# imjaegyun/super_resolution

Measured on AMD Instinct MI355X. Metric: SR output megapixels/sec, HAT-S x4, 1280x720 LR in, higher is better.
Workload: dtype bf16; 1 GPU; HAT-S x4, one 3x720x1280 LR frame per GPU, full-frame forward; upscale=4, parallelism=dp1

## Files before the change

include/hat_mi355x.h:

```cpp
#ifndef HAT_MI355X_H
#define HAT_MI355X_H

#include <stdint.h>

#ifdef __cplusplus
extern "C" {
#endif

#define HAT_ABI_VERSION 2

enum { HAT_F32 = 0, HAT_BF16 = 1 };
enum { HAT_EINVAL = -1, HAT_ELDS = -2, HAT_EUNSUPPORTED = -3 };

enum { HAT_ACT_NONE = 0, HAT_ACT_GELU = 1 , HAT_ACT_LRELU = 2 ,
       HAT_ACT_LRELU02 = 3  };
enum { HAT_X_NHWC_T = 0, HAT_X_NHWC_F32 = 1, HAT_X_NCHW_F32_MEAN = 2 };
enum { HAT_O_NHWC_T = 0, HAT_O_NHWC_F32 = 1, HAT_O_PIXSHUF_T = 2, HAT_O_NCHW_F32 = 3 };

typedef struct HatConvDesc {
    const void* x;
    const void* x0;
    const void* w;
    const float* bias;
    void* out;
    const float* r1;
    const void* r2;
    const float* r2scale;
    float* colsum;
    int32_t B, H, W;
    int32_t Cin, ldx, x_mode;
    int32_t c_split, ldx0;
    int32_t ksize, Kpad;
    int32_t nt, n_slices;
    int64_t w_bstride;
    int32_t n_store;
    int32_t ldo, out_mode, act;
    int32_t ldr1, ldr2, r2scale_bstride;
    int32_t ps_r;
    float in_scale, out_scale;
    float mean[4];
    int32_t dtype;
    int32_t ld_ln, ln_ones;
    const float* ln_g;
    const float* ln_b;
    void* ln_out;
    float* gap_out;
    void* n16_out;
    int32_t gap_c;
    int32_t reserved0;
} HatConvDesc;

int hat_conv_occupancy(const HatConvDesc* d, int32_t* wgs_per_cu);
int hat_conv_tiles(const HatConvDesc* d, int32_t* tiles_out);
int hat_conv_plan(const HatConvDesc* d, int32_t* waves, int32_t* rows_per_wave, int32_t* tiles, int64_t* lds_bytes);
int hat_conv(const HatConvDesc* d, void* stream);

int hat_linear(const HatConvDesc* d, void* stream);

int hat_conv3x3_small_groups(const HatConvDesc* d, int32_t* groups_out);
int hat_conv3x3_small(const HatConvDesc* d, void* stream);

typedef struct HatCabFoldDesc {
    const void* c1;
    const float* c1_colsum;
    const float* w2;
    const float* b2;
    const float* wk;
    const float* bias_in;
    float* scale;
    void* wf;
    float* bias_out;
    float* tmp;
    int32_t B, H, W, C, mid, ld1, tiles, ldcs, k, ld_scale, dtype;
    float conv_scale;
    const float* stats;
    const float* w2f;
} HatCabFoldDesc;
int hat_cab_fold(const HatCabFoldDesc* d, void* stream);

typedef struct HatAggrCabDesc {
    HatConvDesc lin;
    const void* c1;
    const void* wf;
    const float* bias_b;
} HatAggrCabDesc;
int hat_aggr_cab(const HatAggrCabDesc* d, void* stream);

int hat_layernorm_blocks(void);
int hat_layernorm(const float* x, void* y, const float* gamma, const float* beta, float* gap_partial,
                  int32_t B, int64_t npix, int32_t C, int32_t ldy, int32_t out_f32, int32_t gap_c,
                  int32_t dtype, void* stream);

int hat_add_f32(const float* a, const float* c, float* out, int32_t B, int64_t n, int64_t c_bstride, void* stream);

int hat_esc_weights(const float* gap_partial, int32_t nblk, int64_t npix, const float* w1, const float* b1,
                    const float* w2, const float* b2, const float* plk_packed, void* w_out, int32_t B,
                    int32_t pdim, int32_t ksize, int32_t Kpad, int32_t dtype, void* stream);

int hat_esc_conv13(const void* x, int32_t ldx, const void* wp, int32_t Kpad, void* y16, int32_t B, int32_t H, int32_t W,
                   int32_t dtype, void* stream);
// ... 5 lines not shown
                    int32_t W, int32_t hid, int32_t ldu, int32_t ldo, int32_t dtype, void* stream);

typedef struct HatMlpDesc {
    const void* x;
    const void* w1f;
    const float* b1;
    const void* w2f;
    const float* b2;
    const float* r1;
    void* out;
    int32_t B, H, W, C, hidden;
    int32_t ldx, ldr1, ldo;
    int32_t out_f32, dtype;
} HatMlpDesc;
int hat_ocab_mlp(const HatMlpDesc* d, void* stream);
int hat_ocab_qkv(const HatMlpDesc* d, void* stream);

int hat_ocab_keybias(const void* sal, int32_t ldsal, const void* kv, int32_t ldkv, float* kb, int32_t B, int32_t H, int32_t W,
                     int32_t C, int32_t ws, int32_t wse, int32_t pad, int32_t k_keep, int32_t dtype, void* stream);
int hat_ocab_attention_kb(const void* q, const void* kv, const float* bias_rot, const float* kb, void* out, int32_t B, int32_t H,
                          int32_t W, int32_t C, int32_t heads, int32_t ws, int32_t wse, int32_t pad, int32_t ldq, int32_t ldkv,
                          int32_t ldo, int32_t dtype, void* stream);

int hat_sgfn_gate(const void* u, const float* wdw, const float* bdw, void* out, int32_t B, int32_t H, int32_t W,
                  int32_t half, int32_t ldu, int32_t ldo, int32_t dtype, void* stream);

int hat_ocab_attention(const void* q, const void* kv, const float* bias_rot, void* out, int32_t B, int32_t H,
                       int32_t W, int32_t C, int32_t heads, int32_t ws, int32_t wse, int32_t ldq,
                       int32_t ldkv, int32_t ldo, int32_t dtype, void* stream);
int hat_ocab_attention_log2(const void* q, const void* kv, const float* bias_rot, void* out, int32_t B, int32_t H, int32_t W,
                            int32_t C, int32_t heads, int32_t ws, int32_t wse, int32_t ldq, int32_t ldkv, int32_t ldo,
                            int32_t dtype, void* stream);

int hat_cab_squeeze_units(int32_t H, int32_t W, int32_t* rows_per_band, int32_t* units);
int hat_cab_squeeze(const void* x, const void* wpk, const float* bias, void* out, float* colsum, int32_t B, int32_t H,
                    int32_t W, int32_t C, int32_t ldx, int32_t dtype, void* stream);

int hat_conv3x3_to_planes(const void* x, const void* wpk, const float* bias, float* out, int32_t B, int32_t H, int32_t W,
                          int32_t C, int32_t ldx, int32_t n_out, float out_scale, const float* mean4, int32_t dtype,
                          void* stream);

int hat_u8_to_planes(const uint8_t* src, int64_t src_pitch, int64_t src_bstride, float* dst, int32_t B, int32_t h, int32_t w,
                     int32_t Hp, int32_t Wp, int32_t bgr, void* stream);
int hat_planes_to_u8(const float* src, int32_t B, int32_t Hs, int32_t Ws, uint8_t* dst, int64_t dst_pitch, int64_t dst_bstride,
                     int32_t h_out, int32_t w_out, int32_t bgr, void* stream);
int hat_conv3x3_to_u8(const void* x, const void* wpk, const float* bias, uint8_t* dst, int64_t dst_pitch, int64_t dst_bstride,
                      int32_t B, int32_t H, int32_t W, int32_t C, int32_t ldx, int32_t h_out, int32_t w_out, float out_scale,
                      const float* mean4, int32_t bgr, int32_t dtype, void* stream);

int hat_yuv420_to_planes(const uint8_t* y, int64_t y_pitch, int64_t y_bstride, const uint8_t* cb, const uint8_t* cr, int64_t c_pitch,
                         int32_t c_step, int64_t c_bstride, float* dst, int32_t B, int32_t h, int32_t w, int32_t Hp, int32_t Wp,
                         const float* to_rgb12, void* stream);
int hat_planes_to_yuv420(const float* src, int32_t B, int32_t Hs, int32_t Ws, uint8_t* y, int64_t y_pitch, int64_t y_bstride,
                         uint8_t* cb, uint8_t* cr, int64_t c_pitch, int32_t c_step, int64_t c_bstride, int32_t h_out, int32_t w_out,
                         const float* from_rgb12, void* stream);
int hat_conv3x3_to_yuv420(const void* x, const void* wpk, const float* bias, uint8_t* y, int64_t y_pitch, int64_t y_bstride, uint8_t* cb,
                          uint8_t* cr, int64_t c_pitch, int32_t c_step, int64_t c_bstride, int32_t B, int32_t H, int32_t W, int32_t C,
                          int32_t ldx, int32_t h_out, int32_t w_out, float out_scale, const float* mean4, const float* from_rgb12,
                          int32_t dtype, void* stream);

int hat_yuv420p16_to_planes(const uint16_t* y, int64_t y_pitch, int64_t y_bstride, const uint16_t* cb, const uint16_t* cr, int64_t c_pitch,
                            int32_t c_step, int64_t c_bstride, float* dst, int32_t B, int32_t h, int32_t w, int32_t Hp, int32_t Wp,
                            const float* to_rgb12, int32_t depth, int32_t msb, void* stream);
int hat_planes_to_yuv420p16(const float* src, int32_t B, int32_t Hs, int32_t Ws, uint16_t* y, int64_t y_pitch, int64_t y_bstride,
                            uint16_t* cb, uint16_t* cr, int64_t c_pitch, int32_t c_step, int64_t c_bstride, int32_t h_out, int32_t w_out,
                            const float* from_rgb12, int32_t depth, int32_t msb, void* stream);
int hat_conv3x3_to_yuv420p16(const void* x, const void* wpk, const float* bias, uint16_t* y, int64_t y_pitch, int64_t y_bstride, uint16_t* cb,
                             uint16_t* cr, int64_t c_pitch, int32_t c_step, int64_t c_bstride, int32_t B, int32_t H, int32_t W, int32_t C,
                             int32_t ldx, int32_t h_out, int32_t w_out, float out_scale, const float* mean4, const float* from_rgb12,
                             int32_t dtype, int32_t depth, int32_t msb, void* stream);

typedef struct {
    void* y; int64_t y_pitch, y_bstride; void* cb; void* cr; int64_t c_pitch; int32_t c_step; int64_t c_bstride;
    int32_t sub_x, sub_y, depth, msb;
} HatYuvSurface;
int hat_yuv_to_planes(const HatYuvSurface* src, float* dst, int32_t B, int32_t h, int32_t w, int32_t Hp, int32_t Wp, const float* to_rgb12,
                      void* stream);
int hat_planes_to_yuv(const float* src, int32_t B, int32_t Hs, int32_t Ws, const HatYuvSurface* dst, int32_t h_out, int32_t w_out,
                      const float* from_rgb12, void* stream);
int hat_conv3x3_to_yuv(const void* x, const void* wpk, const float* bias, const HatYuvSurface* dst, int32_t B, int32_t H, int32_t W, int32_t C,
                       int32_t ldx, int32_t h_out, int32_t w_out, float out_scale, const float* mean4, const float* from_rgb12,
                       int32_t dtype, void* stream);

#define HAT_SITING_CENTER 0
#define HAT_SITING_LEFT 1
#define HAT_SITING_TOPLEFT 2
int hat_yuv_to_planes_sited(const HatYuvSurface* src, int32_t siting, float* dst, int32_t B, int32_t h, int32_t w, int32_t Hp, int32_t Wp,
                            const float* to_rgb12, void* stream);
int hat_planes_to_yuv_sited(const float* src, int32_t B, int32_t Hs, int32_t Ws, const HatYuvSurface* dst, int32_t siting, int32_t h_out,
                            int32_t w_out, const float* from_rgb12, void* stream);

int hat_imresize_rows(const void* src, int32_t src_u8, int64_t src_pitch, int64_t src_bstride, int32_t bgr, float* mid, int32_t B,
                      int32_t h, int32_t w, int32_t oh, const float* w_h, const int32_t* src_h, int32_t P_h, int64_t n_table,
                      void* stream);
int hat_imresize_cols_to_planes(const float* mid, int32_t B, int32_t oh, int32_t w, int32_t ow, const float* w_w, const int32_t* src_w,
                                int32_t P_w, int64_t n_table, float* dst, int32_t Hp, int32_t Wp, void* stream);
int hat_imresize_cols_to_u8(const float* mid, int32_t B, int32_t oh, int32_t w, int32_t ow, const float* w_w, const int32_t* src_w,
                            int32_t P_w, int64_t n_table, uint8_t* dst, int64_t dst_pitch, int64_t dst_bstride, int32_t bgr,
                            void* stream);


enum { HAT_METRICS_Y = 1, HAT_METRICS_BGR = 2, HAT_METRICS_PSNR = 4, HAT_METRICS_SSIM = 8 };
int hat_u8_metrics_workspace_bytes(int32_t B, int32_t h, int32_t w, int32_t crop_border, int32_t flags, int64_t* bytes);
int hat_u8_metrics(const uint8_t* a, int64_t a_pitch, int64_t a_bstride, const uint8_t* b, int64_t b_pitch, int64_t b_bstride,
                   int32_t B, int32_t h, int32_t w, int32_t crop_border, int32_t flags, double* sums, void* workspace, void* stream);

int hat_pil_resize_u8(const uint8_t* src, int64_t src_pitch, int32_t h, int32_t w, uint8_t* mid, uint8_t* dst, int64_t dst_pitch, int32_t oh,
                      int32_t ow, const int32_t* coef_w, const int32_t* bounds_w, int32_t K_w, const int32_t* coef_h,
                      const int32_t* bounds_h, int32_t K_h, void* stream);
int hat_arb_psnr_workspace_bytes(int32_t h, int32_t w, int32_t shave, int64_t* bytes);
int hat_arb_psnr(const float* pred, int32_t ph, int32_t pw, const uint8_t* gt, int64_t gt_pitch, int32_t h, int32_t w, int32_t gray,
                 int32_t shave, double* sums, void* workspace, void* stream);

int hat_window_attention(const void* q, const void* kv, const float* bias_flip, void* out, int32_t B, int32_t H,
                         int32_t W, int32_t C, int32_t heads, int32_t ws, int32_t shift, int32_t ldq, int32_t ldkv,
                         int32_t ldo, int32_t dtype, void* stream);

typedef struct HatFfnDesc {
    const float* t_in;
    float* t_out;
    const float* ln_g;
    const float* ln_b;
    const void* w1f;
    const float* b1;
    const void* dww;
    const float* dwb;
    const void* w2f;
    const float* b2;
    const float* ln1_g;
    const float* ln1_b;
    void* n_out;
    float* gap_out;
    int32_t B, H, W, C;
    int32_t chunks;
    int32_t ldn, gap_c;
    int32_t dtype;
    int32_t ldm_in;
    const void* m_in;
    void* n16_out;
} HatFfnDesc;

int hat_ffn_tiles(const HatFfnDesc* d, int32_t* tiles_out);
int hat_ffn(const HatFfnDesc* d, void* stream);

int hat_ffn2(const HatFfnDesc* d, void* stream);

typedef struct HatHabTailDesc {
    HatFfnDesc ffn;
    const void* n;
    const void* y16;
    const void* c1;
    const void* w_aggr;
    const void* wf;
    const float* bias_b;
    int32_t ldn_in;
    int32_t ldr2;
    const void* r2;
    const float* r2scale;
    int32_t r2scale_bstride;
    int32_t reserved1;
} HatHabTailDesc;
int hat_hab_tail(const HatHabTailDesc* d, void* stream);

int hat_hab_tail3(const HatHabTailDesc* d, void* stream);

typedef struct hat_plan hat_plan;
// ... 144 lines not shown
```

super_resolution_amd/_lib.py:

```python
from __future__ import annotations

import ctypes as C
import os
import threading

_HERE = os.path.dirname(os.path.abspath(__file__))
LIB_PATH = os.environ.get("HAT_MI355X_LIB") or os.path.join(_HERE, "libhat_mi355x.so")

ABI_VERSION = 2
HAT_F32, HAT_BF16 = 0, 1
ACT_NONE, ACT_GELU, ACT_LRELU, ACT_LRELU02 = 0, 1, 2, 3
X_NHWC_T, X_NHWC_F32, X_NCHW_F32_MEAN = 0, 1, 2
O_NHWC_T, O_NHWC_F32, O_PIXSHUF_T, O_NCHW_F32 = 0, 1, 2, 3
METRICS_Y, METRICS_BGR, METRICS_PSNR, METRICS_SSIM = 1, 2, 4, 8

_ERRORS = {-1: "HAT_EINVAL (bad argument)", -2: "HAT_ELDS (tile does not fit in 160 KiB LDS)",
           -3: "HAT_EUNSUPPORTED (shape not instantiated)"}


class HatConvDesc(C.Structure):
    _fields_ = [
        ("x", C.c_void_p), ("x0", C.c_void_p), ("w", C.c_void_p), ("bias", C.c_void_p),
        ("out", C.c_void_p), ("r1", C.c_void_p), ("r2", C.c_void_p), ("r2scale", C.c_void_p), ("colsum", C.c_void_p),
        ("B", C.c_int32), ("H", C.c_int32), ("W", C.c_int32),
        ("Cin", C.c_int32), ("ldx", C.c_int32), ("x_mode", C.c_int32),
        ("c_split", C.c_int32), ("ldx0", C.c_int32),
        ("ksize", C.c_int32), ("Kpad", C.c_int32),
        ("nt", C.c_int32), ("n_slices", C.c_int32),
        ("w_bstride", C.c_int64),
        ("n_store", C.c_int32),
        ("ldo", C.c_int32), ("out_mode", C.c_int32), ("act", C.c_int32),
        ("ldr1", C.c_int32), ("ldr2", C.c_int32), ("r2scale_bstride", C.c_int32),
        ("ps_r", C.c_int32),
        ("in_scale", C.c_float), ("out_scale", C.c_float),
        ("mean", C.c_float * 4),
        ("dtype", C.c_int32),
        ("ld_ln", C.c_int32), ("ln_ones", C.c_int32),
        ("ln_g", C.c_void_p), ("ln_b", C.c_void_p), ("ln_out", C.c_void_p),
        ("gap_out", C.c_void_p), ("n16_out", C.c_void_p), ("gap_c", C.c_int32), ("reserved0", C.c_int32),
    ]


class HatMlpDesc(C.Structure):
    _fields_ = [
        ("x", C.c_void_p), ("w1f", C.c_void_p), ("b1", C.c_void_p), ("w2f", C.c_void_p), ("b2", C.c_void_p),
        ("r1", C.c_void_p), ("out", C.c_void_p),
        ("B", C.c_int32), ("H", C.c_int32), ("W", C.c_int32), ("C", C.c_int32), ("hidden", C.c_int32),
        ("ldx", C.c_int32), ("ldr1", C.c_int32), ("ldo", C.c_int32),
        ("out_f32", C.c_int32), ("dtype", C.c_int32),
    ]


class HatFfnDesc(C.Structure):
    _fields_ = [
        ("t_in", C.c_void_p), ("t_out", C.c_void_p), ("ln_g", C.c_void_p), ("ln_b", C.c_void_p),
        ("w1f", C.c_void_p), ("b1", C.c_void_p), ("dww", C.c_void_p), ("dwb", C.c_void_p),
        ("w2f", C.c_void_p), ("b2", C.c_void_p), ("ln1_g", C.c_void_p), ("ln1_b", C.c_void_p),
        ("n_out", C.c_void_p), ("gap_out", C.c_void_p),
        ("B", C.c_int32), ("H", C.c_int32), ("W", C.c_int32), ("C", C.c_int32),
        ("chunks", C.c_int32), ("ldn", C.c_int32), ("gap_c", C.c_int32), ("dtype", C.c_int32),
        ("ldm_in", C.c_int32), ("m_in", C.c_void_p), ("n16_out", C.c_void_p),
    ]


class HatHabTailDesc(C.Structure):
    _fields_ = [("ffn", HatFfnDesc), ("n", C.c_void_p), ("y16", C.c_void_p), ("c1", C.c_void_p), ("w_aggr", C.c_void_p),
                ("wf", C.c_void_p), ("bias_b", C.c_void_p), ("ldn_in", C.c_int32), ("ldr2", C.c_int32), ("r2", C.c_void_p),
                ("r2scale", C.c_void_p), ("r2scale_bstride", C.c_int32), ("reserved1", C.c_int32)]


class HatCabFoldDesc(C.Structure):
    _fields_ = [
        ("c1", C.c_void_p), ("c1_colsum", C.c_void_p), ("w2", C.c_void_p), ("b2", C.c_void_p), ("wk", C.c_void_p),
        ("bias_in", C.c_void_p), ("scale", C.c_void_p), ("wf", C.c_void_p), ("bias_out", C.c_void_p), ("tmp", C.c_void_p),
        ("B", C.c_int32), ("H", C.c_int32), ("W", C.c_int32), ("C", C.c_int32), ("mid", C.c_int32), ("ld1", C.c_int32),
        ("tiles", C.c_int32), ("ldcs", C.c_int32), ("k", C.c_int32), ("ld_scale", C.c_int32), ("dtype", C.c_int32),
        ("conv_scale", C.c_float), ("stats", C.c_void_p), ("w2f", C.c_void_p),
    ]


class HatAggrCabDesc(C.Structure):
    _fields_ = [("lin", HatConvDesc), ("c1", C.c_void_p), ("wf", C.c_void_p), ("bias_b", C.c_void_p)]


class HatYuvSurface(C.Structure):
    _fields_ = [("y", C.c_void_p), ("y_pitch", C.c_int64), ("y_bstride", C.c_int64), ("cb", C.c_void_p), ("cr", C.c_void_p),
                ("c_pitch", C.c_int64), ("c_step", C.c_int32), ("c_bstride", C.c_int64),
                ("sub_x", C.c_int32), ("sub_y", C.c_int32), ("depth", C.c_int32), ("msb", C.c_int32)]


class HatNafHalfDesc(C.Structure):
    _fields_ = [("r_in", C.c_void_p), ("gprev", C.c_void_p), ("wf", C.c_void_p), ("bf", C.c_void_p), ("r_out", C.c_void_p),
                ("w1", C.c_void_p), ("b1", C.c_void_p), ("dww", C.c_void_p), ("dwb", C.c_void_p), ("g_out", C.c_void_p),
                ("partials", C.c_void_p), ("wf_bstride", C.c_int64), ("bf_bstride", C.c_int32),
                ("B", C.c_int32), ("H", C.c_int32), ("W", C.c_int32), ("C", C.c_int32), ("ldr", C.c_int32), ("ldg", C.c_int32),
                ("ldo", C.c_int32), ("dtype", C.c_int32), ("reserved0", C.c_int32)]
# ... 13 lines not shown
                ("ldo", C.c_int32), ("out_f32", C.c_int32), ("dtype", C.c_int32), ("reserved0", C.c_int32)]


_YUV_BLOCK = [C.c_void_p, C.c_int64, C.c_int64, C.c_void_p, C.c_void_p, C.c_int64, C.c_int32, C.c_int64]

SIGNATURES = {
    "hat_abi_version": (C.c_int, []),
    "hat_target_arch": (C.c_char_p, []),
    "hat_conv_tiles": (C.c_int, [C.POINTER(HatConvDesc), C.POINTER(C.c_int32)]),
    "hat_ocab_mlp": (C.c_int, [C.POINTER(HatMlpDesc), C.c_void_p]),
    "hat_ocab_qkv": (C.c_int, [C.POINTER(HatMlpDesc), C.c_void_p]),
    "hat_conv_occupancy": (C.c_int, [C.POINTER(HatConvDesc), C.POINTER(C.c_int32)]),
    "hat_conv_plan": (C.c_int, [C.POINTER(HatConvDesc), C.POINTER(C.c_int32), C.POINTER(C.c_int32), C.POINTER(C.c_int32),
                                C.POINTER(C.c_int64)]),
    "hat_conv": (C.c_int, [C.POINTER(HatConvDesc), C.c_void_p]),
    "hat_linear": (C.c_int, [C.POINTER(HatConvDesc), C.c_void_p]),
    "hat_conv3x3_small_groups": (C.c_int, [C.POINTER(HatConvDesc), C.POINTER(C.c_int32)]),
    "hat_conv3x3_small": (C.c_int, [C.POINTER(HatConvDesc), C.c_void_p]),
    "hat_cab_fold": (C.c_int, [C.POINTER(HatCabFoldDesc), C.c_void_p]),
    "hat_aggr_cab": (C.c_int, [C.POINTER(HatAggrCabDesc), C.c_void_p]),
    "hat_ffn_tiles": (C.c_int, [C.POINTER(HatFfnDesc), C.POINTER(C.c_int32)]),
    "hat_ffn": (C.c_int, [C.POINTER(HatFfnDesc), C.c_void_p]),
    "hat_ffn2": (C.c_int, [C.POINTER(HatFfnDesc), C.c_void_p]),
    "hat_hab_tail": (C.c_int, [C.POINTER(HatHabTailDesc), C.c_void_p]),
    "hat_hab_tail3": (C.c_int, [C.POINTER(HatHabTailDesc), C.c_void_p]),
    "hat_plan_load": (C.c_int, [C.c_char_p, C.POINTER(C.c_void_p)]),
    "hat_plan_info": (C.c_int, [C.c_void_p, C.POINTER(C.c_int32), C.POINTER(C.c_int64), C.POINTER(C.c_int64)]),
    "hat_plan_forward": (C.c_int, [C.c_void_p, C.c_void_p, C.c_void_p, C.c_void_p]),
    "hat_plan_free": (None, [C.c_void_p]),
    "hat_layernorm_blocks": (C.c_int, []),
    "hat_layernorm": (C.c_int, [C.c_void_p, C.c_void_p, C.c_void_p, C.c_void_p, C.c_void_p, C.c_int32, C.c_int64,
                                C.c_int32, C.c_int32, C.c_int32, C.c_int32, C.c_int32, C.c_void_p]),
    "hat_rect_sum": (C.c_int, [C.c_void_p, C.c_int32, C.c_int32, C.c_int32, C.c_int32, C.c_int32, C.c_int32, C.c_int32, C.c_int32,
                               C.c_int64, C.c_int32, C.c_void_p, C.c_int32, C.c_void_p, C.c_void_p, C.c_void_p]),
    "hat_add_f32": (C.c_int, [C.c_void_p, C.c_void_p, C.c_void_p, C.c_int32, C.c_int64, C.c_int64, C.c_void_p]),
    "hat_esc_weights": (C.c_int, [C.c_void_p, C.c_int32, C.c_int64, C.c_void_p, C.c_void_p, C.c_void_p, C.c_void_p,
                                  C.c_void_p, C.c_void_p, C.c_int32, C.c_int32, C.c_int32, C.c_int32, C.c_int32, C.c_void_p]),
    "hat_esc_conv13": (C.c_int, [C.c_void_p, C.c_int32, C.c_void_p, C.c_int32, C.c_void_p, C.c_int32, C.c_int32, C.c_int32, C.c_int32, C.c_void_p]),
    "hat_eca_scale": (C.c_int, [C.c_void_p, C.c_int32, C.c_int32, C.c_int64, C.c_void_p, C.c_int32, C.c_float,
                                C.c_void_p, C.c_void_p, C.c_int32, C.c_int32, C.c_void_p]),
    "hat_dwconv_gate": (C.c_int, [C.c_void_p, C.c_void_p, C.c_void_p, C.c_void_p, C.c_int32, C.c_int32, C.c_int32,
                                  C.c_int32, C.c_int32, C.c_int32, C.c_int32, C.c_void_p]),
    "hat_ocab_keybias": (C.c_int, [C.c_void_p, C.c_int32, C.c_void_p, C.c_int32, C.c_void_p] + [C.c_int32] * 9 + [C.c_void_p]),
    "hat_ocab_attention_kb": (C.c_int, [C.c_void_p] * 5 + [C.c_int32] * 12 + [C.c_void_p]),
    "hat_sgfn_gate": (C.c_int, [C.c_void_p, C.c_void_p, C.c_void_p, C.c_void_p, C.c_int32, C.c_int32, C.c_int32,
                                C.c_int32, C.c_int32, C.c_int32, C.c_int32, C.c_void_p]),
    "hat_ocab_attention": (C.c_int, [C.c_void_p, C.c_void_p, C.c_void_p, C.c_void_p, C.c_int32, C.c_int32, C.c_int32,
                                     C.c_int32, C.c_int32, C.c_int32, C.c_int32, C.c_int32, C.c_int32, C.c_int32,
                                     C.c_int32, C.c_void_p]),
    "hat_ocab_attention_log2": (C.c_int, [C.c_void_p, C.c_void_p, C.c_void_p, C.c_void_p, C.c_int32, C.c_int32, C.c_int32,
                                     C.c_int32, C.c_int32, C.c_int32, C.c_int32, C.c_int32, C.c_int32, C.c_int32,
                                     C.c_int32, C.c_void_p]),
    "hat_cab_squeeze_units": (C.c_int, [C.c_int32, C.c_int32, C.c_void_p, C.c_void_p]),
    "hat_cab_squeeze": (C.c_int, [C.c_void_p, C.c_void_p, C.c_void_p, C.c_void_p, C.c_void_p, C.c_int32, C.c_int32, C.c_int32,
                                  C.c_int32, C.c_int32, C.c_int32, C.c_void_p]),
    "hat_conv3x3_to_planes": (C.c_int, [C.c_void_p, C.c_void_p, C.c_void_p, C.c_void_p, C.c_int32, C.c_int32, C.c_int32, C.c_int32,
                                        C.c_int32, C.c_int32, C.c_float, C.c_void_p, C.c_int32, C.c_void_p]),
    "hat_u8_to_planes": (C.c_int, [C.c_void_p, C.c_int64, C.c_int64, C.c_void_p, C.c_int32, C.c_int32, C.c_int32, C.c_int32, C.c_int32,
                                   C.c_int32, C.c_void_p]),
    "hat_planes_to_u8": (C.c_int, [C.c_void_p, C.c_int32, C.c_int32, C.c_int32, C.c_void_p, C.c_int64, C.c_int64, C.c_int32, C.c_int32,
                                   C.c_int32, C.c_void_p]),
    "hat_conv3x3_to_u8": (C.c_int, [C.c_void_p, C.c_void_p, C.c_void_p, C.c_void_p, C.c_int64, C.c_int64, C.c_int32, C.c_int32, C.c_int32,
                                    C.c_int32, C.c_int32, C.c_int32, C.c_int32, C.c_float, C.c_void_p, C.c_int32, C.c_int32, C.c_void_p]),
    "hat_plan_forward_u8": (C.c_int, [C.c_void_p, C.c_void_p, C.c_int64, C.c_int32, C.c_int32, C.c_void_p, C.c_int64, C.c_int32,
                                      C.c_void_p]),
    "hat_yuv420_to_planes": (C.c_int, _YUV_BLOCK + [C.c_void_p, C.c_int32, C.c_int32, C.c_int32, C.c_int32, C.c_int32, C.c_void_p, C.c_void_p]),
    "hat_planes_to_yuv420": (C.c_int, [C.c_void_p, C.c_int32, C.c_int32, C.c_int32] + _YUV_BLOCK + [C.c_int32, C.c_int32, C.c_void_p, C.c_void_p]),
    "hat_conv3x3_to_yuv420": (C.c_int, [C.c_void_p, C.c_void_p, C.c_void_p] + _YUV_BLOCK + [C.c_int32] * 7 + [C.c_float, C.c_void_p, C.c_void_p,
                                                                                                      C.c_int32, C.c_void_p]),
    "hat_plan_forward_yuv420": (C.c_int, [C.c_void_p] + _YUV_BLOCK + [C.c_int32, C.c_int32] + _YUV_BLOCK + [C.c_void_p, C.c_void_p, C.c_void_p]),
    "hat_yuv420p16_to_planes": (C.c_int, _YUV_BLOCK + [C.c_void_p, C.c_int32, C.c_int32, C.c_int32, C.c_int32, C.c_int32, C.c_void_p, C.c_int32,
                                                       C.c_int32, C.c_void_p]),
    "hat_planes_to_yuv420p16": (C.c_int, [C.c_void_p, C.c_int32, C.c_int32, C.c_int32] + _YUV_BLOCK + [C.c_int32, C.c_int32, C.c_void_p, C.c_int32,
                                                                                                     C.c_int32, C.c_void_p]),
    "hat_conv3x3_to_yuv420p16": (C.c_int, [C.c_void_p, C.c_void_p, C.c_void_p] + _YUV_BLOCK + [C.c_int32] * 7 + [C.c_float, C.c_void_p, C.c_void_p,
                                                                                                         C.c_int32, C.c_int32, C.c_int32, C.c_void_p]),
    "hat_plan_forward_yuv420_deep": (C.c_int, [C.c_void_p] + _YUV_BLOCK + [C.c_int32] * 4 + _YUV_BLOCK + [C.c_int32, C.c_int32, C.c_void_p, C.c_void_p,
                                                                                                     C.c_void_p]),
    "hat_yuv_to_planes": (C.c_int, [C.POINTER(HatYuvSurface), C.c_void_p] + [C.c_int32] * 5 + [C.c_void_p, C.c_void_p]),
    "hat_planes_to_yuv": (C.c_int, [C.c_void_p, C.c_int32, C.c_int32, C.c_int32, C.POINTER(HatYuvSurface), C.c_int32, C.c_int32, C.c_void_p,
                                    C.c_void_p]),
    "hat_conv3x3_to_yuv": (C.c_int, [C.c_void_p, C.c_void_p, C.c_void_p, C.POINTER(HatYuvSurface)] + [C.c_int32] * 7 + [C.c_float, C.c_void_p,
                                                                                                        C.c_void_p, C.c_int32, C.c_void_p]),
    "hat_plan_forward_yuv": (C.c_int, [C.c_void_p, C.POINTER(HatYuvSurface), C.POINTER(HatYuvSurface), C.c_int32, C.c_int32, C.c_void_p,
                                       C.c_void_p, C.c_void_p]),
    "hat_yuv_to_planes_sited": (C.c_int, [C.POINTER(HatYuvSurface), C.c_int32, C.c_void_p] + [C.c_int32] * 5 + [C.c_void_p, C.c_void_p]),
    "hat_planes_to_yuv_sited": (C.c_int, [C.c_void_p, C.c_int32, C.c_int32, C.c_int32, C.POINTER(HatYuvSurface), C.c_int32, C.c_int32, C.c_int32,
                                          C.c_void_p, C.c_void_p]),
    "hat_plan_forward_yuv_sited": (C.c_int, [C.c_void_p, C.POINTER(HatYuvSurface), C.c_int32, C.POINTER(HatYuvSurface), C.c_int32, C.c_int32,
                                             C.c_int32, C.c_void_p, C.c_void_p, C.c_void_p]),
    "hat_imresize_rows": (C.c_int, [C.c_void_p, C.c_int32, C.c_int64, C.c_int64, C.c_int32, C.c_void_p, C.c_int32, C.c_int32, C.c_int32,
                                    C.c_int32, C.c_void_p, C.c_void_p, C.c_int32, C.c_int64, C.c_void_p]),
    "hat_imresize_cols_to_planes": (C.c_int, [C.c_void_p, C.c_int32, C.c_int32, C.c_int32, C.c_int32, C.c_void_p, C.c_void_p, C.c_int32,
                                              C.c_int64, C.c_void_p, C.c_int32, C.c_int32, C.c_void_p]),
    "hat_imresize_cols_to_u8": (C.c_int, [C.c_void_p, C.c_int32, C.c_int32, C.c_int32, C.c_int32, C.c_void_p, C.c_void_p, C.c_int32,
                                          C.c_int64, C.c_void_p, C.c_int64, C.c_int64, C.c_int32, C.c_void_p]),
    "hat_u8_metrics_workspace_bytes": (C.c_int, [C.c_int32, C.c_int32, C.c_int32, C.c_int32, C.c_int32, C.POINTER(C.c_int64)]),
    "hat_u8_metrics": (C.c_int, [C.c_void_p, C.c_int64, C.c_int64, C.c_void_p, C.c_int64, C.c_int64, C.c_int32, C.c_int32, C.c_int32,
                                 C.c_int32, C.c_int32, C.c_void_p, C.c_void_p, C.c_void_p]),
    "hat_pil_resize_u8": (C.c_int, [C.c_void_p, C.c_int64, C.c_int32, C.c_int32, C.c_void_p, C.c_void_p, C.c_int64, C.c_int32, C.c_int32,
                                    C.c_void_p, C.c_void_p, C.c_int32, C.c_void_p, C.c_void_p, C.c_int32, C.c_void_p]),
    "hat_arb_psnr_workspace_bytes": (C.c_int, [C.c_int32, C.c_int32, C.c_int32, C.POINTER(C.c_int64)]),
    "hat_arb_psnr": (C.c_int, [C.c_void_p, C.c_int32, C.c_int32, C.c_void_p, C.c_int64, C.c_int32, C.c_int32, C.c_int32, C.c_int32,
                               C.c_void_p, C.c_void_p, C.c_void_p]),
    "hat_dihedral_f32": (C.c_int, [C.c_void_p, C.c_void_p, C.c_int32, C.c_int32, C.c_int32, C.c_int32, C.c_int32, C.c_float, C.c_int32,
                                   C.c_void_p]),
    "hat_window_attention": (C.c_int, [C.c_void_p, C.c_void_p, C.c_void_p, C.c_void_p, C.c_int32, C.c_int32, C.c_int32,
                                       C.c_int32, C.c_int32, C.c_int32, C.c_int32, C.c_int32, C.c_int32, C.c_int32,
                                       C.c_int32, C.c_void_p]),
    "hat_niqe_workspace_bytes": (C.c_int, [C.c_int32, C.c_int32, C.c_int32, C.c_int32, C.POINTER(C.c_int32), C.POINTER(C.c_int32),
                                           C.POINTER(C.c_int64)]),
    "hat_niqe_y_u8": (C.c_int, [C.c_void_p, C.c_int64, C.c_int64, C.c_int32, C.c_int32, C.c_int32, C.c_int32, C.c_int32, C.c_void_p,
                                C.c_void_p, C.c_void_p]),
    "hat_imresize_plane_rows": (C.c_int, [C.c_void_p, C.c_void_p, C.c_int32, C.c_int32, C.c_int32, C.c_int32, C.c_void_p, C.c_void_p,
                                          C.c_int32, C.c_int64, C.c_void_p]),
    "hat_imresize_plane_cols": (C.c_int, [C.c_void_p, C.c_int32, C.c_int32, C.c_int32, C.c_int32, C.c_void_p, C.c_void_p, C.c_int32,
                                          C.c_int64, C.c_float, C.c_void_p, C.c_void_p]),
    "hat_niqe_block_stats": (C.c_int, [C.c_void_p, C.c_int32, C.c_int32, C.c_int32, C.c_int32, C.POINTER(C.c_double), C.c_void_p,
                                       C.c_void_p]),
    "hat_naf_half_tiles": (C.c_int, [C.c_int32, C.c_int32]),
    "hat_naf_half": (C.c_int, [C.POINTER(HatNafHalfDesc), C.c_void_p]),
    "hat_naf_fold": (C.c_int, [C.POINTER(HatNafFoldDesc), C.c_void_p]),
    "hat_esc_convffn_tiles": (C.c_int, [C.c_int32, C.c_int32]),
    "hat_esc_convffn": (C.c_int, [C.POINTER(HatEscConvFfnDesc), C.c_void_p]),
    "hat_window_attention_r": (C.c_int, [C.c_void_p] * 4 + [C.c_int32] * 10 + [C.c_void_p]),
    "hat_esc_layernorm": (C.c_int, [C.c_void_p] * 4 + [C.c_float, C.c_int64, C.c_int32, C.c_int32, C.c_int32, C.c_void_p]),
    "hat_esc_shuffle_add": (C.c_int, [C.c_void_p] * 3 + [C.c_int32] * 5 + [C.c_void_p]),
    "hat_escreal_skip": (C.c_int, [C.c_void_p] * 7 + [C.c_int32] * 6 + [C.c_void_p]),
    "hat_dysample": (C.c_int, [C.c_void_p] * 4 + [C.c_int32] * 5 + [C.c_void_p]),
    "hat_unshuffle_pad": (C.c_int, [C.c_void_p] * 2 + [C.c_int32] * 5 + [C.c_void_p]),
    "hat_escrealm_skip": (C.c_int, [C.c_void_p] * 9 + [C.c_int32] * 8 + [C.c_void_p]),
    "hat_shuffle_planes": (C.c_int, [C.c_void_p] * 2 + [C.c_int32] * 5 + [C.c_void_p]),
    "hat_escfp_convffn": (C.c_int, [C.POINTER(HatEscConvFfnDesc), C.c_void_p]),
    "hat_escfp_layernorm": (C.c_int, [C.c_void_p] * 4 + [C.c_float, C.c_int64, C.c_int32, C.c_int32, C.c_int32, C.c_void_p]),
    "hat_escfp_weights": (C.c_int, [C.c_void_p, C.c_int32, C.c_int64] + [C.c_void_p] * 7 + [C.c_int32] * 3 + [C.c_void_p]),
    "hat_escfp_shuffle_bicubic": (C.c_int, [C.c_void_p] * 4 + [C.c_int32] * 5 + [C.c_void_p]),
    "hat_lte_query": (C.c_int, [C.c_void_p, C.c_void_p, C.c_int32, C.c_int32, C.c_void_p, C.c_int32, C.c_int32] + [C.c_void_p] * 11
                      + [C.c_int64, C.c_int32, C.c_int32] + [C.c_float] * 4 + [C.c_void_p, C.c_int32, C.c_void_p]),
    "hat_lte_query_u8": (C.c_int, [C.c_void_p, C.c_void_p, C.c_int32, C.c_int32, C.c_void_p, C.c_int32, C.c_int32] + [C.c_void_p] * 9
                         + [C.c_int32, C.c_int32] + [C.c_float] * 4 + [C.c_void_p, C.c_int64, C.c_int32, C.c_int32, C.c_void_p]),
    "hat_lte_query_yuv": (C.c_int, [C.c_void_p, C.c_void_p, C.c_int32, C.c_int32, C.c_void_p, C.c_int32, C.c_int32] + [C.c_void_p] * 9
                          + [C.c_int32, C.c_int32] + [C.c_float] * 4 + [C.POINTER(HatYuvSurface), C.c_void_p, C.c_int32, C.c_void_p]),
    "hat_shuffle_to_u8": (C.c_int, [C.c_void_p, C.c_int32, C.c_void_p] + [C.c_int32] * 4 + [C.c_void_p, C.c_int64, C.c_int64] + [C.c_int32] * 3
                          + [C.c_void_p]),
    "hat_shuffle_to_yuv": (C.c_int, [C.c_void_p, C.c_int32, C.c_void_p] + [C.c_int32] * 4 + [C.POINTER(HatYuvSurface), C.c_int32, C.c_int32,
                                                                                              C.c_void_p, C.c_void_p]),
}

_lib = None
_lock = threading.Lock()


def load():
    global _lib
    if _lib is not None:
        return _lib
    with _lock:
        if _lib is not None:
            return _lib
        if not os.path.exists(LIB_PATH):
            raise RuntimeError(
                f"{LIB_PATH} not found: the HIP kernels are not built. Run `python -m super_resolution_amd.build` "
                "(needs hipcc). There is no CPU fallback for the HAT forward pass.")
        import torch
        lib = C.CDLL(LIB_PATH)
        for name, (res, args) in SIGNATURES.items():
# ... 17 lines not shown
```

super_resolution_amd/build.py:

```python
from __future__ import annotations

import os
import subprocess
import sys
from concurrent.futures import ThreadPoolExecutor

HERE = os.path.dirname(os.path.abspath(__file__))
CSRC = os.path.join(HERE, "csrc")
LIB = os.path.join(HERE, "libhat_mi355x.so")
SOURCES = ["hat_conv.hip", "hat_conv64r.hip", "hat_attn.hip", "hat_misc.hip", "hat_ffn.hip", "hat_ffn2.hip", "hat_tail3.hip", "hat_tail3l.hip", "hat_pw.hip", "hat_mlp.hip", "hat_cabsq.hip", "hat_esc13.hip", "hat_u8.hip", "hat_yuv.hip", "hat_resize.hip", "hat_pil_resize.hip", "hat_metrics.hip", "hat_dihedral.hip", "hat_niqe.hip", "hat_naf.hip", "hat_esc.hip", "hat_escreal.hip", "hat_escrealm.hip", "hat_escfp.hip", "hat_lte.hip", "hat_esc_sink.hip", "hat_plan.cpp"]
HEADERS = [os.path.join(CSRC, "hat_common.h"), os.path.join(CSRC, "hat_yuv_check.h"), os.path.join(CSRC, "hat_yuv_sample.h"), os.path.join(CSRC, "hat_frame_sink.h"), os.path.join(CSRC, "hat_esc_ffn.h"), os.path.join(CSRC, "hat_plan_parse.h"), os.path.join(os.path.dirname(HERE), "include", "hat_mi355x.h")]
FLAGS = ["-O3", "--offload-arch=gfx950", "-fPIC", "-std=c++17", "-Wall", "-Wno-unused-function"]


def _hipcc() -> str:
    for c in (os.environ.get("HIPCC"), "/opt/rocm/bin/hipcc", "hipcc"):
        if c and (os.path.isabs(c) and os.path.exists(c) or not os.path.isabs(c)):
            return c
    raise RuntimeError("hipcc not found")


def _stale(target: str, deps) -> bool:
    if not os.path.exists(target):
        return True
    t = os.path.getmtime(target)
    return any(os.path.getmtime(d) > t for d in deps)


def build(force: bool = False, verbose: bool = True) -> str:
    hipcc = _hipcc()
    objs, jobs = [], []
    for src in SOURCES:
        s = os.path.join(CSRC, src)
        o = os.path.join(CSRC, os.path.splitext(src)[0] + ".o")
        objs.append(o)
        if force or _stale(o, [s] + HEADERS):
            jobs.append([hipcc, *FLAGS, "-c", s, "-o", o])

    def run(cmd):
        if verbose:
            print(" ".join(cmd), flush=True)
        r = subprocess.run(cmd, capture_output=True, text=True)
        if r.returncode != 0:
            raise RuntimeError(f"hipcc failed:\n{' '.join(cmd)}\n{r.stdout}\n{r.stderr}")
        if verbose and r.stderr.strip():
            print(r.stderr, file=sys.stderr)

    with ThreadPoolExecutor(max_workers=4) as ex:
        list(ex.map(run, jobs))
    if force or jobs or _stale(LIB, objs):
        run([hipcc, "--offload-arch=gfx950", "-shared", "-fPIC", "-o", LIB, *objs])
    return LIB


if __name__ == "__main__":
    print(build(force="--force" in sys.argv))
```

super_resolution_amd/csrc/hat_conv.hip:

```cpp
#include <type_traits>

#include "hat_common.h"

bool hat_conv64r_can_launch(const HatConvDesc& d);
int hat_conv64r_launch(const HatConvDesc& d, hipStream_t s);

#ifndef HAT_CONV_PIPE
#define HAT_CONV_PIPE 1
#endif

namespace {

struct TileCfg { int waves, pt; };

__host__ inline size_t conv_lds_bytes(const HatConvDesc& d, int waves, int pt, int es, int kc) {
    const int hl = d.ksize / 2;
    const int cin_p = (d.Cin + 7) & ~7;
    const size_t xs = (size_t)(waves * pt + 2 * hl) * (16 + 2 * hl) * lds_row_elems(cin_p, es) * es;
    const size_t ws = (size_t)d.nt * 16 * lds_row_elems(kc, es) * es;
    const size_t koff = ((size_t)(d.Kpad / 32) * 16 + 15) & ~(size_t)15;
    return xs + ws + koff;
}

__host__ inline bool conv_pick(const HatConvDesc& d, TileCfg* out, size_t* lds) {
    const int es = d.dtype == HAT_BF16 ? 2 : 4;
    const int kc = (d.dtype == HAT_BF16 ? 64 : 32) * (d.nt == 1 ? 3 : (d.nt <= 4 ? 2 : 1));
    const TileCfg cands[3] = {{8, 2}, {4, 2}, {4, 1}};
    const size_t wbytes = (size_t)d.nt * 16 * d.ksize * d.ksize * ((d.Cin + 7) & ~7) * es;
    for (int pass = (wbytes <= 180000 ? 0 : 1); pass < 2; ++pass) {
        const size_t limit = pass == 0 ? HAT_LDS_MAX / 2 : HAT_LDS_MAX;
        for (int i = 0; i < 3; ++i) {
            const int rows = cands[i].waves * cands[i].pt;
            if (i < 2 && d.H * 2 <= rows) continue;
            if (pass == 0 && i == 2) continue;
            const size_t b = conv_lds_bytes(d, cands[i].waves, cands[i].pt, es, kc);
            if (b <= limit) { *out = cands[i]; *lds = b; return true; }
        }
    }
    return false;
}

template <typename T, int WAVES, int PT, int NT, int TH = 0>
__global__ __launch_bounds__(WAVES * 64) void conv_kernel(const HatConvDesc d) {
    using M = MT<T>;
    constexpr int NTHR = WAVES * 64;
    constexpr int TROWS = WAVES * PT;
    constexpr int KC = M::KC * (NT == 1 ? 3 : (NT <= 4 ? 2 : 1));
    constexpr int KS = KC / 32;
    constexpr int PPR = KC * (int)sizeof(T) / 16;
    constexpr int VEC = M::VEC;
    constexpr int WPIECES = NT * 16 * PPR;
    constexpr int WPT = (WPIECES + NTHR - 1) / NTHR;

    extern __shared__ __attribute__((aligned(16))) char smem[];
#ifdef HAT_CONV_STAMPS
    const long long st0 = (long long)__builtin_amdgcn_s_memtime();
#endif
    const int tid = threadIdx.x;
    const int lane = tid & 63, wave = tid >> 6, g = lane >> 4, c16 = lane & 15;
    if (d.reserved0 > 0) {
        const unsigned lin = (blockIdx.z * gridDim.y + blockIdx.y) * gridDim.x + blockIdx.x;
        if (lin < 256u) {
            const int n = (int)((lin >> 3) & 3u) * d.reserved0;
            for (int i = 0; i < n; ++i) __builtin_amdgcn_s_sleep(127);
        }
    }
    const int ks_ = d.ksize;
    const int hl = ks_ >> 1, TWH = 16 + 2 * hl, THH = TROWS + 2 * hl;
    const int Cin = d.Cin, Cin_p = (Cin + 7) & ~7;
    const int ldxs = lds_row_elems(Cin_p, sizeof(T));
    const int ldws = lds_row_elems(KC, sizeof(T));
    T* Xs = reinterpret_cast<T*>(smem);
    T* Ws = Xs + (size_t)THH * TWH * ldxs;
    int* koff = reinterpret_cast<int*>(Ws + NT * 16 * ldws);
    float* cs = reinterpret_cast<float*>(Ws);

    const int b = blockIdx.z;
    const int x0 = blockIdx.x * 16, y0 = blockIdx.y * TROWS;
    const int H = d.H, W = d.W;
    const int ntaps = ks_ * ks_;

    for (int i = tid; i < (d.Kpad / 32) * 4; i += NTHR) {
        const int k = 32 * (i >> 2) + 8 * (i & 3);
        int tp = k / Cin_p;
        const int cc = k - tp * Cin_p;
        tp = tp < ntaps ? tp : ntaps - 1;
        koff[i] = ((tp / ks_) * TWH + (tp % ks_)) * ldxs + cc;
    }
// ... 427 lines not shown
    if (!d.x || !d.w || !d.bias || !d.out) return HAT_EINVAL;
    if (d.reserved0 & ~3) return HAT_EINVAL;
    if (d.reserved0) {
        if (d.dtype != HAT_BF16 || d.nt != 9 || d.n_slices != 1 || d.n_store != 144 || d.colsum || d.ksize == 1) return HAT_EINVAL;
        if ((d.reserved0 & 1) && (!d.r1 || reinterpret_cast<uintptr_t>(d.r1) % 8)) return HAT_EINVAL;
        if ((d.reserved0 & 2) && (d.out_mode != HAT_O_NHWC_F32 || d.ldo % 8 || reinterpret_cast<uintptr_t>(d.out) % 16)) return HAT_EINVAL;
    }
    if (d.B < 1 || d.H < 1 || d.W < 1 || d.Cin < 1) return HAT_EINVAL;
    if (d.act < HAT_ACT_NONE || d.act > HAT_ACT_LRELU02) return HAT_EINVAL;
    if (d.ksize < 1 || (d.ksize & 1) == 0 || d.ksize > 17) return HAT_EINVAL;
    if (d.dtype != HAT_F32 && d.dtype != HAT_BF16) return HAT_EINVAL;
    const int kc = (d.dtype == HAT_BF16 ? 64 : 32) * (d.nt == 1 ? 3 : (d.nt <= 4 ? 2 : 1)), vec = d.dtype == HAT_BF16 ? 8 : 4;
    const int cin_p = (d.Cin + 7) & ~7;
    if (d.Kpad % kc || d.Kpad < d.ksize * d.ksize * cin_p) return HAT_EINVAL;
    if (d.n_slices < 1 || d.n_store < 1 || d.n_store > d.n_slices * d.nt * 16) return HAT_EINVAL;
    if (d.x_mode == HAT_X_NHWC_T) {
        if (d.ldx % vec || d.ldx < cin_p) return HAT_EINVAL;
        if (d.x0 && (d.ldx0 % vec || d.c_split % vec || d.c_split > d.Cin)) return HAT_EINVAL;
    } else if (d.x_mode == HAT_X_NHWC_F32) {
        if (d.ldx % 4 || d.Cin % 4 || d.x0) return HAT_EINVAL;
    } else if (d.x_mode == HAT_X_NCHW_F32_MEAN) {
        if (d.Cin > 4 || d.x0) return HAT_EINVAL;
    } else {
        return HAT_EINVAL;
    }
    if (d.out_mode == HAT_O_NCHW_F32) {
        if (d.n_store > 4 || d.r1 || d.r2) return HAT_EINVAL;
    } else {
        if (d.n_store % 4 || d.ldo % 4) return HAT_EINVAL;
        if (d.out_mode == HAT_O_PIXSHUF_T) {
            if (d.ps_r < 2 || d.n_store % (d.ps_r * d.ps_r) || (d.n_store / (d.ps_r * d.ps_r)) % 4 || d.r1 || d.r2) return HAT_EINVAL;
        } else if (d.out_mode != HAT_O_NHWC_T && d.out_mode != HAT_O_NHWC_F32) {
            return HAT_EINVAL;
        }
    }
    if (d.r1 && d.ldr1 % 4) return HAT_EINVAL;
    if (d.r2 && (d.ldr2 % 4 || !d.r2scale)) return HAT_EINVAL;
    if (d.ln_out) {
        if (!d.ln_g || !d.ln_b || d.ln_ones || d.n_slices != 1 || d.n_store != d.nt * 16 || d.ld_ln % 4 || d.ld_ln < d.n_store) return HAT_EINVAL;
        if (d.out_mode != HAT_O_NHWC_T && d.out_mode != HAT_O_NHWC_F32) return HAT_EINVAL;
        if (d.colsum || d.gap_c < 0 || d.gap_c > 16 || d.gap_c % 4) return HAT_EINVAL;
    } else if (d.gap_out || d.n16_out) {
#ifndef HAT_CONV_STAMPS
        return HAT_EINVAL;
#endif
    }
    return 0;
}

}

extern "C" int hat_conv_tiles(const HatConvDesc* d, int32_t* tiles_out) {
    if (!d || !tiles_out) return HAT_EINVAL;
    TileCfg tc; size_t lds;
    if (!conv_pick(*d, &tc, &lds)) return HAT_ELDS;
    *tiles_out = ((d->W + 15) / 16) * ((d->H + tc.waves * tc.pt - 1) / (tc.waves * tc.pt));
    return 0;
}

extern "C" int hat_conv_plan(const HatConvDesc* d, int32_t* waves, int32_t* rows_per_wave, int32_t* tiles, int64_t* lds_bytes) {
    if (!d || !waves || !rows_per_wave || !tiles || !lds_bytes) return HAT_EINVAL;
    TileCfg tc; size_t lds;
    if (!conv_pick(*d, &tc, &lds)) return HAT_ELDS;
    *waves = tc.waves; *rows_per_wave = tc.pt; *lds_bytes = (int64_t)lds;
    *tiles = ((d->W + 15) / 16) * ((d->H + tc.waves * tc.pt - 1) / (tc.waves * tc.pt));
    return 0;
}

extern "C" int hat_conv_occupancy(const HatConvDesc* dp, int32_t* wgs_per_cu) {
    if (!dp || !wgs_per_cu) return HAT_EINVAL;
    TileCfg tc; size_t lds;
    if (!conv_pick(*dp, &tc, &lds)) return HAT_ELDS;
    int v = 0;
    g_occ_query = &v;
    const int rc = dp->dtype == HAT_BF16 ? dispatch_tile<bf16_t>(*dp, tc, lds, nullptr) : dispatch_tile<float>(*dp, tc, lds, nullptr);
    g_occ_query = nullptr;
    *wgs_per_cu = v;
    return rc;
}

extern "C" int hat_conv(const HatConvDesc* dp, void* stream) {
    if (!dp) return HAT_EINVAL;
    const HatConvDesc& d = *dp;
    int rc = conv_validate(d);
    if (rc) return rc;
    TileCfg tc; size_t lds;
    hipStream_t s = reinterpret_cast<hipStream_t>(stream);
    if (hat_conv64r_can_launch(d)) return hat_conv64r_launch(d, s);
    if (!conv_pick(d, &tc, &lds)) return HAT_ELDS;
    if (d.dtype == HAT_BF16) return dispatch_tile<bf16_t>(d, tc, lds, s);
    return dispatch_tile<float>(d, tc, lds, s);
}
```

super_resolution_amd/csrc/hat_plan.cpp:

```cpp
#include <hip/hip_runtime.h>
#include <stdint.h>
#include <stdio.h>
#include <string.h>

#include <string>
#include <utility>
#include <vector>

#include "../../include/hat_mi355x.h"
#include "hat_plan_parse.h"
#include "hat_yuv_check.h"

using namespace hat_plan_host;

struct hat_plan {
    int32_t dims[8];
    std::vector<Buf> bufs;
    std::vector<Call> calls;
    int device = -1;
    mutable float* stage_in = nullptr;
    mutable float* stage_out = nullptr;
};

namespace {

struct Resolved {
    const hat_plan* p;
    const Call* c;
    const void* x;
    void* y;
    void* stream;
    std::vector<std::vector<unsigned char>> tmp;
    void* ptr(uint32_t buf, uint64_t off) const {
        if (buf == NULL_BUF) return nullptr;
        const Buf& b = p->bufs[buf];
        char* base = b.kind == BUF_INPUT ? (char*)const_cast<void*>(x) : (b.kind == BUF_OUTPUT ? (char*)y : (char*)b.dev);
        return base + off;
    }
    int32_t I(size_t k) const { return (int32_t)c->args[k].i; }
    int64_t L(size_t k) const { return c->args[k].i; }
    float F(size_t k) const { return (float)c->args[k].f; }
    void* P(size_t k) {
        const Arg& a = c->args[k];
        if (a.tag == ARG_PTR) return ptr(a.buf, a.off);
        if (a.tag == ARG_STREAM) return stream;
        if (a.tag == ARG_STRUCT || a.tag == ARG_HOST) {
            tmp.emplace_back(a.blob);
            for (const Fix& fx : a.fix) {
                void* v = ptr(fx.buf, fx.off);
                memcpy(tmp.back().data() + fx.field_off, &v, sizeof(void*));
            }
            return tmp.back().data();
        }
        return nullptr;
    }
};

template <class T> T arg_as(Resolved& r, size_t k) {
    if constexpr (std::is_same_v<T, int32_t>) return r.I(k);
    else if constexpr (std::is_same_v<T, int64_t>) return r.L(k);
    else if constexpr (std::is_same_v<T, float>) return r.F(k);
    else return (T)r.P(k);
}
template <class... A, size_t... K> int replay(int (*fn)(A...), Resolved& r, std::index_sequence<K...>) { return fn(arg_as<A>(r, K)...); }
template <class... A> int replay(int (*fn)(A...), Resolved& r) {
    return r.c->args.size() == sizeof...(A) ? replay(fn, r, std::index_sequence_for<A...>{}) : HAT_EINVAL;
}

int dispatch(Resolved& r) {
    switch (r.c->fn) {
#define HAT_PLAN_CASE(f) case FN_##f: return replay(&f, r);
        HAT_PLAN_FUNCTIONS(HAT_PLAN_CASE)
#undef HAT_PLAN_CASE
        default: return HAT_EUNSUPPORTED;
    }
}

}

extern "C" void hat_plan_free(hat_plan* p) {
    if (!p) return;
    for (Buf& b : p->bufs)
        if (b.dev) (void)hipFree(b.dev);
    if (p->stage_in) (void)hipFree(p->stage_in);
    if (p->stage_out) (void)hipFree(p->stage_out);
// ... 8 lines not shown
    try {
        return plan_load_impl(path, out);
    } catch (...) {
        return HAT_EINVAL;
    }
}

namespace {
struct PlanGuard {
    hat_plan* p;
    ~PlanGuard() { if (p) hat_plan_free(p); }
};
}

static int plan_load_impl(const char* path, hat_plan** out) {
    FILE* f = fopen(path, "rb");
    if (!f) return HAT_EINVAL;
    struct FileGuard { FILE* f; ~FileGuard() { fclose(f); } } fguard{f};
    hat_plan* p = new hat_plan();
    PlanGuard guard{p};
    {
        Parsed parsed;
        if (const int rc = hat_plan_parse(f, &parsed)) return rc;
        memcpy(p->dims, parsed.dims, sizeof(p->dims));
        p->bufs = std::move(parsed.bufs);
        p->calls = std::move(parsed.calls);
    }
    if (hipGetDevice(&p->device) != hipSuccess) return HAT_EINVAL;
    std::vector<unsigned char> host;
    for (Buf& b : p->bufs) {
        if (b.kind != BUF_CONST && b.kind != BUF_SCRATCH) continue;
        hipError_t e = hipMalloc(&b.dev, b.nbytes ? b.nbytes : 16);
        if (e != hipSuccess) { b.dev = nullptr; return (int)e; }
        if (b.kind == BUF_CONST) {
            host.resize(b.nbytes);
            if (fseeko(f, (off_t)b.file_off, SEEK_SET) != 0 || (b.nbytes && fread(host.data(), 1, b.nbytes, f) != b.nbytes)) return HAT_EINVAL;
            e = hipMemcpy(b.dev, host.data(), b.nbytes, hipMemcpyHostToDevice);
        } else {
            e = hipMemset(b.dev, 0, b.nbytes ? b.nbytes : 16);
        }
        if (e != hipSuccess) return (int)e;
    }
    if (const hipError_t e = hipDeviceSynchronize()) return (int)e;
    guard.p = nullptr;
    *out = p;
    return 0;
}

extern "C" int hat_plan_info(const hat_plan* p, int32_t* dims8, int64_t* n_calls, int64_t* device_bytes) {
    if (!p) return HAT_EINVAL;
    if (dims8) memcpy(dims8, p->dims, sizeof(p->dims));
    if (n_calls) *n_calls = (int64_t)p->calls.size();
    if (device_bytes) {
        int64_t s = 0;
        for (const Buf& b : p->bufs)
            if (b.dev) s += (int64_t)b.nbytes;
        *device_bytes = s;
    }
    return 0;
}

extern "C" int hat_plan_forward(const hat_plan* p, const float* x, float* y, void* stream) {
    if (!p || !x || !y) return HAT_EINVAL;
    int dev = -1;
    if (hipGetDevice(&dev) != hipSuccess || dev != p->device) return HAT_EINVAL;
    for (const Call& c : p->calls) {
        Resolved r{p, &c, x, y, stream, {}};
        const int rc = dispatch(r);
        if (rc) return rc;
    }
    return 0;
}

namespace {
bool addresses_output(const hat_plan* p, const Call& c) {
    for (const Arg& a : c.args) {
        if (a.tag == ARG_PTR && a.buf != NULL_BUF && p->bufs[a.buf].kind == BUF_OUTPUT) return true;
        for (const Fix& fx : a.fix)
            if (fx.buf != NULL_BUF && p->bufs[fx.buf].kind == BUF_OUTPUT) return true;
    }
    return false;
}

bool ends_in_planes(const hat_plan* p) {
    if (p->calls.empty()) return false;
    const Call& c = p->calls.back();
    if (c.fn != FN_hat_conv3x3_to_planes || c.args.size() != 14 || c.args[3].tag != ARG_PTR || c.args[3].buf >= p->bufs.size()) return false;
    if (p->bufs[c.args[3].buf].kind != BUF_OUTPUT || c.args[3].off != 0 || c.args[9].i != 3) return false;
    for (size_t k = 0; k + 1 < p->calls.size(); ++k)
        if (addresses_output(p, p->calls[k])) return false;
    return true;
}

template <typename Source, typename Fused, typename Planes>
int forward_frames(const hat_plan* p, void* stream, Source source, Fused fused_sink, Planes planes_sink, bool may_fuse = true) {
    const int32_t B = p->dims[0], H = p->dims[2], W = p->dims[3], s = p->dims[4];
    int dev = -1;
    if (hipGetDevice(&dev) != hipSuccess || dev != p->device) return HAT_EINVAL;
    const bool fused = may_fuse && ends_in_planes(p);
    if (!p->stage_in) {
        const hipError_t e = hipMalloc((void**)&p->stage_in, (size_t)B * 3 * H * W * sizeof(float));
        if (e != hipSuccess) { p->stage_in = nullptr; return (int)e; }
    }
    if (!fused && !p->stage_out) {
        const hipError_t e = hipMalloc((void**)&p->stage_out, (size_t)B * 3 * s * H * s * W * sizeof(float));
        if (e != hipSuccess) { p->stage_out = nullptr; return (int)e; }
    }
    int rc = source(p->stage_in);
    if (rc) return rc;
    const size_t n = p->calls.size() - (fused ? 1 : 0);
    for (size_t k = 0; k < n; ++k) {
        Resolved r{p, &p->calls[k], p->stage_in, p->stage_out, stream, {}};
        rc = dispatch(r);
        if (rc) return rc;
    }
    if (!fused) return planes_sink(p->stage_out, s * H, s * W);
    Resolved r{p, &p->calls.back(), p->stage_in, nullptr, stream, {}};
    return fused_sink(r);
}

int frame_fits(const hat_plan* p, int32_t h, int32_t w) {
    const int32_t H = p->dims[2], W = p->dims[3];
    if (p->dims[1] != 3 || p->dims[5] != 3) return HAT_EUNSUPPORTED;
    return h > H || w > W || H - h >= h || W - w >= w ? HAT_EINVAL : 0;
}

int forward_yuv(const hat_plan* p, const HatYuvSurface* src, const HatYuvSurface* dst, int32_t h, int32_t w, const float* to_rgb12,
                const float* from_rgb12, void* stream, bool planes420, int32_t src_siting = HAT_SITING_CENTER,
                int32_t dst_siting = HAT_SITING_CENTER) {
    if (!hat_yuv_surface_ok(src, 1, h, w)) return HAT_EINVAL;
    if (const int rc = frame_fits(p, h, w)) return rc;
    const int32_t B = p->dims[0], H = p->dims[2], W = p->dims[3], s = p->dims[4], ho = s * h, wo = s * w;
    if (!hat_yuv_surface_ok(src, B, h, w) || !hat_yuv_surface_ok(dst, B, (int64_t)s * h, (int64_t)s * w)) return HAT_EINVAL;
    const bool sited_out = hat_siting_of(dst, dst_siting) != HAT_SITING_CENTER;
    return forward_frames(
        p, stream,
        [&](float* in) {
            if (hat_siting_of(src, src_siting) == HAT_SITING_CENTER) return hat_yuv_to_planes(src, in, B, h, w, H, W, to_rgb12, stream);
            return hat_yuv_to_planes_sited(src, src_siting, in, B, h, w, H, W, to_rgb12, stream);
        },
        [&](Resolved& r) {
            return hat_conv3x3_to_yuv(r.P(0), r.P(1), (const float*)r.P(2), dst, r.I(4), r.I(5), r.I(6), r.I(7), r.I(8), ho, wo, r.F(10),
                                      (const float*)r.P(11), from_rgb12, r.I(12), stream);
        },
        [&](const float* out, int32_t Hs, int32_t Ws) {
            const HatYuvSurface& d = *dst;
            if (sited_out) return hat_planes_to_yuv_sited(out, B, Hs, Ws, dst, dst_siting, ho, wo, from_rgb12, stream);
            if (!planes420) return hat_planes_to_yuv(out, B, Hs, Ws, dst, ho, wo, from_rgb12, stream);
            if (d.depth == 8)
                return hat_planes_to_yuv420(out, B, Hs, Ws, (uint8_t*)d.y, d.y_pitch, d.y_bstride, (uint8_t*)d.cb, (uint8_t*)d.cr, d.c_pitch, d.c_step,
                                            d.c_bstride, ho, wo, from_rgb12, stream);
            return hat_planes_to_yuv420p16(out, B, Hs, Ws, (uint16_t*)d.y, d.y_pitch, d.y_bstride, (uint16_t*)d.cb, (uint16_t*)d.cr, d.c_pitch, d.c_step,
                                           d.c_bstride, ho, wo, from_rgb12, d.depth, d.msb, stream);
        },
        !sited_out);
}
}

extern "C" int hat_plan_forward_u8(const hat_plan* p, const uint8_t* src, int64_t src_pitch, int32_t h, int32_t w, uint8_t* dst,
                                   int64_t dst_pitch, int32_t flags, void* stream) {
    if (!p || !src || !dst || h < 1 || w < 1 || src_pitch < 3 * (int64_t)w) return HAT_EINVAL;
    if (const int rc = frame_fits(p, h, w)) return rc;
    const int32_t B = p->dims[0], H = p->dims[2], W = p->dims[3], s = p->dims[4];
    if (dst_pitch < 3 * (int64_t)s * w) return HAT_EINVAL;
    const int bgr = flags & 1, ho = s * h, wo = s * w;
    return forward_frames(
        p, stream, [&](float* in) { return hat_u8_to_planes(src, src_pitch, src_pitch * h, in, B, h, w, H, W, bgr, stream); },
        [&](Resolved& r) {
            return hat_conv3x3_to_u8(r.P(0), r.P(1), (const float*)r.P(2), dst, dst_pitch, dst_pitch * ho, r.I(4), r.I(5), r.I(6), r.I(7), r.I(8),
                                     ho, wo, r.F(10), (const float*)r.P(11), bgr, r.I(12), stream);
        },
        [&](const float* out, int32_t Hs, int32_t Ws) { return hat_planes_to_u8(out, B, Hs, Ws, dst, dst_pitch, dst_pitch * ho, ho, wo, bgr, stream); });
}

extern "C" int hat_plan_forward_yuv420(const hat_plan* p, const uint8_t* sy, int64_t sy_pitch, int64_t sy_bstride, const uint8_t* scb,
                                       const uint8_t* scr, int64_t sc_pitch, int32_t sc_step, int64_t sc_bstride, int32_t h, int32_t w,
                                       uint8_t* dy, int64_t dy_pitch, int64_t dy_bstride, uint8_t* dcb, uint8_t* dcr, int64_t dc_pitch,
                                       int32_t dc_step, int64_t dc_bstride, const float* to_rgb12, const float* from_rgb12, void* stream) {
    if (!p || !sy || !scb || !scr || !dy || !dcb || !dcr || !to_rgb12 || !from_rgb12 || h < 2 || w < 2 || (h & 1) || (w & 1)) return HAT_EINVAL;
    if ((sc_step != 1 && sc_step != 2) || (dc_step != 1 && dc_step != 2) || sy_pitch < w || sc_pitch < (int64_t)sc_step * (w / 2)) return HAT_EINVAL;
    const HatYuvSurface src = hat_yuv420_surface(sy, sy_pitch, sy_bstride, scb, scr, sc_pitch, sc_step, sc_bstride, 8, 0);
    const HatYuvSurface dst = hat_yuv420_surface(dy, dy_pitch, dy_bstride, dcb, dcr, dc_pitch, dc_step, dc_bstride, 8, 0);
    return forward_yuv(p, &src, &dst, h, w, to_rgb12, from_rgb12, stream, true);
}

extern "C" int hat_plan_forward_yuv420_deep(const hat_plan* p, const void* sy, int64_t sy_pitch, int64_t sy_bstride, const void* scb,
                                            const void* scr, int64_t sc_pitch, int32_t sc_step, int64_t sc_bstride, int32_t src_depth,
                                            int32_t src_msb, int32_t h, int32_t w, void* dy, int64_t dy_pitch, int64_t dy_bstride, void* dcb,
                                            void* dcr, int64_t dc_pitch, int32_t dc_step, int64_t dc_bstride, int32_t dst_depth, int32_t dst_msb,
                                            const float* to_rgb12, const float* from_rgb12, void* stream) {
    if (!p || !sy || !scb || !scr || !dy || !dcb || !dcr || !to_rgb12 || !from_rgb12 || h < 2 || w < 2 || (h & 1) || (w & 1)) return HAT_EINVAL;
    if ((src_depth != 8 && !hat_yuv_depth_ok(src_depth, 0)) || (dst_depth != 8 && !hat_yuv_depth_ok(dst_depth, 0))) return HAT_EINVAL;
    if ((src_msb != 0 && src_msb != 1) || (dst_msb != 0 && dst_msb != 1)) return HAT_EINVAL;
    const int32_t db = dst_depth == 8 ? 1 : 2;
    if ((db == 2 && (((uintptr_t)dy | (uintptr_t)dcb | (uintptr_t)dcr) & 1)) || (dc_step != db && dc_step != 2 * db)) return HAT_EINVAL;
    const HatYuvSurface src = hat_yuv420_surface(sy, sy_pitch, sy_bstride, scb, scr, sc_pitch, sc_step, sc_bstride, src_depth, src_msb);
    const HatYuvSurface dst = hat_yuv420_surface(dy, dy_pitch, dy_bstride, dcb, dcr, dc_pitch, dc_step, dc_bstride, dst_depth, dst_msb);
    return forward_yuv(p, &src, &dst, h, w, to_rgb12, from_rgb12, stream, true);
}

extern "C" int hat_plan_forward_yuv(const hat_plan* p, const HatYuvSurface* src, const HatYuvSurface* dst, int32_t h, int32_t w,
                                    const float* to_rgb12, const float* from_rgb12, void* stream) {
    if (!p || !src || !dst || !to_rgb12 || !from_rgb12 || h < 1 || w < 1) return HAT_EINVAL;
    return forward_yuv(p, src, dst, h, w, to_rgb12, from_rgb12, stream, false);
}

extern "C" int hat_plan_forward_yuv_sited(const hat_plan* p, const HatYuvSurface* src, int32_t src_siting, const HatYuvSurface* dst,
                                          int32_t dst_siting, int32_t h, int32_t w, const float* to_rgb12, const float* from_rgb12,
                                          void* stream) {
    if (!p || !src || !dst || !to_rgb12 || !from_rgb12 || h < 1 || w < 1 || !hat_siting_ok(src_siting) || !hat_siting_ok(dst_siting))
        return HAT_EINVAL;
    return forward_yuv(p, src, dst, h, w, to_rgb12, from_rgb12, stream, false, src_siting, dst_siting);
}
```

super_resolution_amd/engine.py:

```python
from __future__ import annotations

import dataclasses
import math
import os
from typing import Dict

import torch

from . import ops
from .engine_base import EngineBase
from .frame_boundary import FrameBoundary
from .ops import (ACT_GELU, ACT_LRELU, ACT_NONE, O_NCHW_F32, O_NHWC_F32, O_NHWC_T, O_PIXSHUF_T, X_NCHW_F32_MEAN, X_NHWC_F32, X_NHWC_T)
from .packing import _ESC

RGB_MEAN = (0.4488, 0.4371, 0.4040)


def _r8(x: int) -> int:
    return (x + 7) // 8 * 8


def _r4(x: int) -> int:
    return (x + 3) // 4 * 4


@dataclasses.dataclass(frozen=True)
class Options:
    no_n16: bool = False
    no_t16: bool = False
    no_fused_ffn: bool = False
    ffn_v1: bool = False
    no_hab_tail: bool = False
    no_cab_fold: bool = False
    no_cab_sweep: bool = False
    no_esc13: bool = False
    esc_side: bool = False
    one_stream: bool = False
    no_attn_log2: bool = False
    no_ocab_mlp: bool = False
    no_ocab_qkv: bool = False
    no_bf16_conv_in: bool = False
    no_conv_ln: bool = False

    @classmethod
    def from_env(cls, env=None) -> "Options":
        env = os.environ if env is None else env
        get = lambda name: env.get("HAT_" + name.upper(), "")
        any_value = ("no_cab_fold", "no_cab_sweep", "no_ocab_mlp", "no_ocab_qkv", "no_bf16_conv_in", "no_conv_ln")
        return cls(**{k.name: (get(k.name) != "" if k.name in any_value else get(k.name) == "1") for k in dataclasses.fields(cls)})


class _Packed:

    def __getitem__(self, key):
        try:
            return getattr(self, key)
        except AttributeError:
            raise KeyError(key) from None


class _Hab(_Packed):
    fold = ffn = ffn3 = fc1 = fc2 = bias256 = None
    tail = "aggr"
    next_ln = None
    out16 = False


class _Ocab(_Packed):
    qkvf = mlpf = esc = fh0 = fh2 = None


class _Naf(_Packed):

    def __init__(self, c, head, blocks, tail):
        self.c, self.head, self.blocks, self.tail = c, head, blocks, tail


class _Group(_Packed):
    to_conv = ocab16 = out16 = False
    conv_ln = None

    def __init__(self, heads, habs, ocab, conv):
        self.heads, self.habs, self.ocab, self.conv = heads, habs, ocab, conv


class _Fwd:

    def __init__(self, eng, w, B, H, W, band, one_stream):
        self.B, self.H, self.W, self.N = B, H, W, H * W
        self.C, self.dt, self.ldc = eng.C, eng.dtype, _r8(eng.C)
        self.geo = dict(B=B, H=H, W=W, dtype=eng.dtype)
        self.w, self.band, self.one_stream = w, band, one_stream
        self.t = self.gin = w["tA"]
        self.have_n = self.have_n16 = False
        self.nblk = ops.layernorm_blocks()

    def ln(self, src, dst, gb, out_f32=False, gap_c=0):
        ops.layernorm(src, dst, gb[0], gb[1], B=self.B, npix=self.N, C_=self.C, ldy=(self.C if out_f32 else self.ldc),
                      out_f32=out_f32, dtype=self.dt, gap=(self.w["gap"] if gap_c else None), gap_c=gap_c)

    def pooled(self, src, ld, C_, dst, off=0, r0=None, r1=None, c0=0, c1=None):
        bd, w = self.band, self.w
        ops.rect_sum(src, dst, w["rs_tmp"], w["rs_cnt"], B=self.B, W=self.W, ld=ld, C_=C_, r0=(bd.lo if r0 is None else r0),
                     r1=(bd.lo + bd.own if r1 is None else r1), c0=c0, c1=c1, out_off=off)

    def gstat(self, esc):
        gs = 32 if esc.pdim > 16 else 16
        return tuple(self.w[k].view(-1)[:self.B * gs].view(self.B, gs) for k in ("gstat_l", "gstat_g"))


class HATEngine(FrameBoundary, EngineBase):
    def __init__(self, cfg: dict, state_dict: Dict[str, torch.Tensor], device, dtype: str = "bf16"):
        if cfg.get("upsampler") != "pixelshuffle":
            raise NotImplementedError("only upsampler='pixelshuffle' is on the hot path (all shipped test YAMLs)")
        if cfg.get("resi_connection", "1conv") not in ("1conv", "identity"):
            raise ValueError(f"Unknown resi_connection: {cfg.get('resi_connection')}")
        self.cfg = cfg
        self.opt = Options.from_env()
        self.identity = cfg.get("resi_connection", "1conv") == "identity"
        if torch.device(device).type != "cuda":
            raise RuntimeError("HATEngine needs a GPU device: there is no CPU path")
        super().__init__(device, dtype, int(os.environ.get("HAT_WS_CACHE", "12")))
        self.C = cfg["embed_dim"]
        self.ws = cfg["window_size"]
        self.wse = self.ws + int(cfg["overlap_ratio"] * self.ws)
        self.scale = cfg["upscale"]
        self.fp16_fallbacks = 0
        self.u8_fused_calls = self.u8_planes_calls = 0
        self.yuv_fused_calls = self.yuv_planes_calls = 0
        self.use_n16 = not self.opt.no_n16
        self.t16 = not self.opt.no_t16 and self.dtype == ops.HAT_BF16 and self.C == 144
        self._s1 = None
        ops._lib.load()
        self.hatx = cfg.get("variant", "hat") == "hatx"
        self.topk = float(cfg.get("kv_topk_ratio", 1.0)) if self.hatx else 1.0
        self.focus = bool(cfg.get("use_focus_bias", False)) if self.hatx else False
        self.fuse_ffn = not self.hatx and ops.ffn_supported(self.C) and not self.opt.no_fused_ffn
        self._pack(state_dict)
        self._resolve()

    def _lin(self, sd, wkey, bkey, scale=1.0):
        w = sd[wkey]
        b = sd.get(bkey) if bkey else None
        o, i = w.shape[0], w.reshape(w.shape[0], -1).shape[1]

        pack = lambda wm, bias: ops.pack_pointwise(wm, bias, self.dtype, self.dev, scale=scale)
        w2 = w.reshape(o, -1)
        if w2.shape[1] == i and i > 512 and i % 16 == 0 and not ops.linear_supported(o, i, self.dtype):
            h1, h2 = pack(w2[:, :i // 2].contiguous(), b), pack(w2[:, i // 2:].contiguous(), None)
            h1.ksplit = h2
            return h1
        return pack(w, b)

    def _c3(self, sd, wkey, bkey):
        w = sd[wkey]
        if w.shape[0] > 16 and ops.conv3x3_small_supported(w.shape[0], w.shape[1], self.dtype):
            return ops.pack_linear_weight(w, sd[bkey], self.dtype, self.dev)
        return ops.pack_conv_weight(w, sd[bkey], self.dtype, self.dev)

    def _esc(self, sd, core, plk_key, pdim, ksize):
        esc = _ESC(sd, core, plk_key, pdim, ksize, self.C, self.dtype, self.dev)
        esc.aggr = self._lin(sd, *esc.aggr_keys)
        esc.conv13 = ops.esc_conv13_supported(pdim, ksize, self.dtype) and not self.opt.no_esc13
        return esc

    def _run_lin(self, pw, x, out, **kw):
        h2 = getattr(pw, "ksplit", None)
        if h2 is not None:
            if kw.get("out_mode") != O_NHWC_F32 or kw.get("act", ACT_NONE) != ACT_NONE:
                raise NotImplementedError("a K-split linear accumulates through its fp32 output")
            (ops.linear if pw.frag else ops.conv)(pw, x, out, **kw)
            (ops.linear if h2.frag else ops.conv)(h2, x.reshape(-1)[pw.cin:], out, **dict(kw, r1=out, ldr1=kw["ldo"]))
            return
        (ops.linear if pw.frag else ops.conv)(pw, x, out, **kw)

    def _pack(self, sd):
        cfg, dev = self.cfg, self.dev
        f32 = dict(dtype=torch.float32, device=dev)
        P = lambda w, b=None, **kw: ops.pack_conv_weight(sd[w], None if b is None else sd[b], self.dtype, dev, **kw)
        vec = lambda k: sd[k].detach().to(**f32).contiguous()
        self.naf = self._pack_naf(sd) if cfg.get("naf") else None
        self.conv_first = P("conv_first.weight", "conv_first.bias")
        self.pe_norm = (vec("patch_embed.norm.weight"), vec("patch_embed.norm.bias")) if cfg.get("patch_norm", True) else None
        self.ape = vec("absolute_pos_embed").reshape(-1) if cfg.get("ape", False) else None
        self.layers = []
        for g, (depth, heads) in enumerate(zip(cfg["depths"], cfg["num_heads"])):
            habs = [self._pack_hab(sd, f"layers.{g}.residual_group.blocks.{i}") for i in range(depth)]
            ocab = self._pack_ocab(sd, f"layers.{g}.residual_group.overlap_attn", heads)
            self.layers.append(_Group(heads, habs, ocab, None if self.identity else P(f"layers.{g}.conv.weight", f"layers.{g}.conv.bias")))
        self.norm = (vec("norm.weight"), vec("norm.bias"))
        self.conv_after_body = None if self.identity else P("conv_after_body.weight", "conv_after_body.bias")
        self.conv_before_up = P("conv_before_upsample.0.weight", "conv_before_upsample.0.bias")
        self.ups = []
        s = self.scale
        if s & (s - 1) == 0:
            for i in range(int(math.log2(s))):
                self.ups.append((self._pack_ps(sd, f"upsample.{2 * i}", 2), 2))
        elif s == 3:
            self.ups.append((self._pack_ps(sd, "upsample.0", 3), 3))
        else:
            raise ValueError(f"scale {s} is not supported. Supported scales: 2^n and 3.")
        self.conv_last = P("conv_last.weight", "conv_last.bias")
        wl = sd["conv_last.weight"]
        self.conv_last_sweep = None
        if ops.conv3x3_to_planes_supported(wl.shape[0], wl.shape[1], 16, self.dtype) and not self.opt.no_cab_sweep:
            self.conv_last_sweep = ops.pack_cab_squeeze(wl, sd["conv_last.bias"], dev) + (wl.shape[0],)

    def _pack_naf(self, sd):
        c, nb = int(self.cfg["naf"]["width"]), int(self.cfg["naf"]["blocks"])
        if c not in ops.NAF_WIDTHS:
            raise ValueError(f"naf_width {c} is not supported: hat_naf_half is built for {' and '.join(map(str, ops.NAF_WIDTHS))} channels")
        if self.cfg["in_chans"] != 3:
            raise ValueError(f"the NAF stem's head and tail convs are packed for in_chans 3, got {self.cfg['in_chans']}")
        P = lambda k: ops.pack_conv_weight(sd[f"naf.{k}.weight"], sd[f"naf.{k}.bias"], self.dtype, self.dev)
        return _Naf(c, P("head"), [ops.pack_naf_block(sd, f"naf.body.{i}", self.dtype, self.dev) for i in range(nb)], P("tail"))

    def _pack_hab(self, sd, p):
        cfg, dt, dev, C, opt = self.cfg, self.dtype, self.dev, self.C, self.opt
        f32 = dict(dtype=torch.float32, device=dev)
        vec = lambda k: sd[k].detach().to(**f32).contiguous()
        hb = _Hab()
        hb.n1 = (vec(p + ".norm1.weight"), vec(p + ".norm1.bias"))
        hb.n2 = (vec(p + ".norm2.weight"), vec(p + ".norm2.bias"))
        hb.esc = self._esc(sd, p + ".esc_attn.core", p + ".esc_attn.plk_filter", cfg["esc_pdim"], cfg["esc_kernel"])
        hb.cab0 = self._c3(sd, p + ".conv_block.cab.0.weight", p + ".conv_block.cab.0.bias")
        hb.cab2 = self._c3(sd, p + ".conv_block.cab.2.weight", p + ".conv_block.cab.2.bias")
        hb.eca_w = vec(p + ".conv_block.cab.3.conv.weight").reshape(-1)
        w2raw = sd[p + ".conv_block.cab.2.weight"]
        if hb.esc.aggr.frag and not hb.cab0.frag and ops.aggr_cab_supported(C, w2raw.shape[1], dt) and not opt.no_cab_fold:
            hb.fold = {"w2": w2raw.detach().to(**f32).contiguous(), "b2": vec(p + ".conv_block.cab.2.bias"),
                       "ba": vec(hb.esc.aggr_keys[1]), "w2f": ops.pack_cab_w2f(w2raw, dev)}
            if ops.cab_squeeze_supported(C, w2raw.shape[1], 16, dt) and not opt.no_cab_sweep:
                hb.fold["sq"] = ops.pack_cab_squeeze(sd[p + ".conv_block.cab.0.weight"], sd[p + ".conv_block.cab.0.bias"], dev)
        if not self.fuse_ffn:
            hb.fc1 = self._lin(sd, p + ".mlp.fc1.weight", p + ".mlp.fc1.bias")
            hb.fc2 = self._lin(sd, p + ".mlp.fc2.weight", p + ".mlp.fc2.bias")
        hid2 = sd[p + ".mlp.dw.weight"].shape[0]
        hb.dw_w = sd[p + ".mlp.dw.weight"].detach().to(**f32).reshape(hid2, 9).t().contiguous()
        hb.dw_b = vec(p + ".mlp.dw.bias")
        hb.tail144_ok = hb.tail180_ok = False
        if not self.fuse_ffn:
            return hb
        fw = [sd[p + k] for k in (".mlp.fc1.weight", ".mlp.fc1.bias", ".mlp.dw.weight", ".mlp.dw.bias", ".mlp.fc2.weight", ".mlp.fc2.bias")]
        fp16_ok = ops.ffn_fp16_range_bound(fw[0], fw[1], fw[2], fw[3], *hb.n2) < ops.FP16_SAFE
        if not fp16_ok:
            self.fp16_fallbacks += 1
        if ops.ffn2_supported(C, hid2 // 2, dt) and not opt.ffn_v1 and fp16_ok:
            hb.ffn = ops.pack_ffn2(*fw, dev)
        else:
            hb.ffn = ops.pack_ffn(*fw, dt, dev)
        hb.tail144_ok = (hb.fold is not None and hb.esc.pdim == 16 and ops.hab_tail_supported(hb.ffn, hb.esc.aggr, w2raw.shape[1], dt)
                         and not opt.no_hab_tail)
        if hb.tail144_ok:
            hb.ffn3 = ops.pack_ffn3(*fw, *hb.n2, dev)
        if (hb.fold is None and C == 180 and fp16_ok and ops.tail3_supported(C, hid2 // 2, dt) and hb.esc.pdim == 16
                and hb.esc.aggr.frag and not opt.no_hab_tail):
            f3 = ops.pack_ffn3(*fw, *hb.n2, dev)
            if ops.hab_tail_supported(f3, hb.esc.aggr, w2raw.shape[1], dt):
                hb.ffn3, hb.tail180_ok = f3, True
                hb.bias256 = torch.zeros(256, **f32)
                hb.bias256[:C] = vec(hb.esc.aggr_keys[1])
        return hb

    def _pack_ocab(self, sd, p, heads):
        cfg, dt, dev, C = self.cfg, self.dtype, self.dev, self.C
        vec = lambda k: sd[k].detach().to(dtype=torch.float32, device=dev).contiguous()
        ws, wse = self.ws, self.wse
        M = ws + wse - 1
        shift = (ws - wse + 1 - (ws - 1)) * (M + 1)
        rot = (torch.arange(M * M) + shift) % (M * M)
        d = C // heads
        qscale = cfg.get("qk_scale") or d ** -0.5
        qlog2 = (ops.ocab_attention_log2_supported(C, heads, ws, wse, dt) and not (self.focus or self.topk < 1.0)
                 and not self.opt.no_attn_log2 and d % 2 == 0 and _r8(C) == C)
        if qlog2:
            qscale = qscale * ops.LOG2E
        table = sd[p + ".relative_position_bias_table"].detach().to(torch.float32).cpu()
        oc = _Ocab()
        oc.n1 = (vec(p + ".norm1.weight"), vec(p + ".norm1.bias"))
        oc.n2 = (vec(p + ".norm2.weight"), vec(p + ".norm2.bias"))
        oc.q = self._lin(sd, p + ".q_proj.weight", p + ".q_proj.bias", scale=qscale)
        oc.kv = self._lin(sd, p + ".kv_proj.weight", p + ".kv_proj.bias")
        oc.proj = self._lin(sd, p + ".proj.weight", p + ".proj.bias")
        oc.mlp0 = self._lin(sd, p + ".mlp.0.weight", p + ".mlp.0.bias")
        oc.mlp2 = self._lin(sd, p + ".mlp.2.weight", p + ".mlp.2.bias")
        if ops.ocab_mlp_supported(C, sd[p + ".mlp.0.weight"].shape[0], dt) and _r8(C) == C and not self.opt.no_ocab_mlp:
            oc.mlpf = ops.pack_ocab_mlp(sd[p + ".mlp.0.weight"], sd[p + ".mlp.0.bias"], sd[p + ".mlp.2.weight"], sd[p + ".mlp.2.bias"], dev)
        oc.bias_rot = table[rot].t().contiguous().to(dev)
        oc.qlog2 = qlog2
# ... 37 lines not shown
                else:
                    nxt, gap_c = (self.norm, 0) if self.conv_after_body is not None else (None, 0)
                G.conv_ln = (nxt, gap_c) if nxt is not None and gap_c in (0, 4, 8, 12, 16) else None
        self._resolve_stream16()
        self.u8_fused = self.conv_last_sweep is not None and self.conv_last_sweep[2] == 3
        hab0 = layers[0].habs[0] if layers and layers[0].habs else None
        self._hab0 = hab0
        self._yw = max([16] + [e.npad for e in escs])
        self._kpad = max([hab0.esc.kpad if hab0 else 0] + [G.ocab.esc.kpad for G in layers if G.ocab.esc is not None])

    def _resolve_stream16(self):
        if not self.t16:
            return
        layers = self.layers
        tail16 = lambda hb: hb.tail == "fused144" and hb.ffn3.C == 144
        conv16 = lambda G: bool(G.conv is not None and not G.conv.frag and G.conv.ksize > 1 and G.conv.nt == 9
                                and G.conv.n_slices == 1 and G.conv.nout == 144)
        for G in layers:
            oc = G.ocab
            G.ocab16 = bool(G.habs and tail16(G.habs[-1]) and G.to_conv and oc.mlpf is not None and oc.proj.frag
                            and oc.proj.nt == 9 and getattr(oc.proj, "ksplit", None) is None and oc.esc is None)
            for i, hb in enumerate(G.habs):
                hb.out16 = tail16(hb) and (G.ocab16 if i + 1 == len(G.habs) else tail16(G.habs[i + 1]))
        for gi, G in enumerate(layers):
            if not conv16(G) or G.conv_ln is None:
                continue
            if gi + 1 < len(layers):
                nG = layers[gi + 1]
                G.out16 = bool(nG.habs and tail16(nG.habs[0]) and conv16(nG))
            else:
                G.out16 = self.conv_after_body is not None

    def _alloc_workspace(self, B, H, W, tag):
        C, dev, T, hab0, yw = self.C, self.dev, self.tdt, self._hab0, self._yw
        N = H * W
        mid = hab0.cab0.nout if hab0 is not None else 8
        hid2 = 2 * int(C * self.cfg["mlp_ratio"])
        z = lambda *shape, dtype=T: torch.zeros(*shape, dtype=dtype, device=dev)
        f = torch.float32
        w = {
            "f0": z(B, N, C, dtype=f), "tA": z(B, N, C, dtype=f), "tB": z(B, N, C, dtype=f), "tC": z(B, N, C, dtype=f),
            "hA": (z(B, N, C, dtype=torch.float16) if self.t16 else None),
            "hB": (z(B, N, C, dtype=torch.float16) if self.t16 else None), "hC": (z(B, N, C, dtype=torch.float16) if self.t16 else None),
            "n": z(B, N, _r8(C)), "n2b": z(B, N, _r8(C)), "c1": z(B, N, _r8(mid)), "c2": z(B, N, _r8(C)), "m2": z(B, N, ops.ffn_m_ld(C)),
            "y16": z(B, N, yw), "n16": z(B, N, 16), "u": z(B, N, _r8(max(hid2, 2 * C))), "g": z(B, N, _r8(max(hid2 // 2, 2 * C))),
            "q": z(B, N, _r8(C)), "kv": z(B, N, _r8(2 * C)), "ao": z(B, N, _r8(C)),
            "fb": z(B, N, 64),
            "gap": z(B, max(ops.layernorm_blocks(), -(-H // 4) * -(-W // 16)), yw, dtype=f),
            "scale": z(B, 256, dtype=f), "eca_tmp": z(B, 32, 256, dtype=f),
        }
        if any(G.ocab.qkvf is not None for G in self.layers):
            w["qkv"] = z(B, N, 432)
        w["weff"] = z(B, yw, max(self._kpad, 64))
        if any(G.ocab.esc is not None for G in self.layers):
            w["yesc"] = z(B, N, _r8(C))
        if self.focus:
            w["fh"], w["sal"] = z(B, N, _r8(C // 4)), z(B, N, 8, dtype=f)
        if self.focus or self.topk < 1.0:
            w["kb"] = z(B, (H // self.ws) * (W // self.ws), -(-(self.wse * self.wse) // 16) * 16, dtype=f)
        if hab0 is not None:
            cab2 = hab0.cab2
            tiles = ops.conv3x3_small_groups(cab2, B, H, W, self.dtype) if cab2.frag else ops.conv_tiles(cab2, H, W, self.dtype)
            w["tiles"] = tiles
            w["colsum"] = z(B, tiles, cab2.npad, dtype=f)
        if hab0 is not None and hab0.fold is not None:
            cab0 = hab0.cab0
            w["sweep"] = "sq" in hab0.fold and W % 16 == 0 and cab0.npad == 16
            w["tiles1"] = ops.cab_squeeze_units(H, W) if w["sweep"] else ops.conv_tiles(cab0, H, W, self.dtype)
            w["colsum1"] = z(B, w["tiles1"], cab0.npad, dtype=f)
            w["wf"] = z(B, hab0.esc.aggr.nt * 3 * 512)
            w["bias_b"] = z(B, hab0.esc.aggr.npad, dtype=f)
        if tag is not None:
            w["gstat_l"], w["gstat_g"] = z(B, yw, dtype=f), z(B, yw, dtype=f)
            w["cstat_l"], w["cstat_g"] = z(B, 72, dtype=f), z(B, 72, dtype=f)
            w["estat_l"], w["estat_g"] = z(B, 256, dtype=f), z(B, 256, dtype=f)
            w["rs_tmp"], w["rs_cnt"] = z(B, 64, 256, dtype=f), torch.zeros(B, dtype=torch.int32, device=dev)
        if self.naf is not None:
            c = self.naf.c
            w["naf_sA"], w["naf_sB"], w["naf_gA"], w["naf_gB"] = z(B, N, c, dtype=f), z(B, N, c, dtype=f), z(B, N, c), z(B, N, c)
            w["naf_part"], w["naf_wf"], w["naf_bf"] = z(B, ops.naf_tiles(H, W), c, dtype=f), z(B, c * c), z(B, c, dtype=f)
            w["x_naf"] = z(B, self.cfg["in_chans"], H, W, dtype=f)
        h, wd = H, W
        w["ups"] = []
        for _, r in self.ups:
            h, wd = h * r, wd * r
            w["ups"].append(z(B, h * wd, 64))
        return w

    def _esc_w(self, esc: _ESC, w, B, H, W, nblk, gap=None):
        ops.esc_weights(w["gap"] if gap is None else gap, nblk, H * W, esc.w1, esc.b1, esc.w2, esc.b2, esc.plk, w["weff"], B=B,
                        pdim=esc.pdim, ksize=esc.ksize, kpad=esc.kpad, dtype=self.dtype)

    def _esc_conv(self, esc: _ESC, w, n, B, H, W, n16=None):
        if esc.conv13:
            src, ldx = (n16, 16) if n16 is not None else (n, _r8(self.C))
            ops.esc_conv13(src, w["weff"], w["y16"], B=B, H=H, W=W, ldx=ldx, kpad=esc.kpad, dtype=self.dtype)
            return
        pw = ops.PackedConv(w["weff"], esc.zero_bias, esc.ksize, esc.pdim, esc.kpad, 1, esc.npad // 16, esc.pdim,
                            w_bstride=esc.npad * esc.kpad)
        ops.conv(pw, n, w["y16"], B=B, H=H, W=W, dtype=self.dtype, ldx=_r8(self.C), ldo=w["y16"].shape[2], n_store=_r4(esc.pdim))

    def _esc_lk(self, esc: _ESC, w, n, B, H, W, nblk):
        self._esc_w(esc, w, B, H, W, nblk)
        self._esc_conv(esc, w, n, B, H, W)

    @staticmethod
    def _hab_halo(esc: _ESC) -> int:
        return max(3, esc.ksize // 2 + 1)

    def _ocab_halo(self, oc: _Ocab) -> int:
        pad = (self.wse - self.ws + 1) // 2
        return pad + (oc.esc.ksize // 2 if oc.esc is not None else 0)

    def band_halo(self) -> int:
        d = 8
        for G in self.layers:
            d = max([d, self._ocab_halo(G.ocab)] + [self._hab_halo(hb.esc) for hb in G.habs])
        return d

    def _side_stream(self, f: _Fwd):
        if f.band is not None or f.one_stream:
            return torch.cuda.current_stream(self.dev)
        if self._s1 is None:
            self._s1 = torch.cuda.Stream(device=self.dev)
        return self._s1

    def _check_input(self, x):
        if x.dim() != 4 or x.shape[1] != self.cfg["in_chans"]:
            raise RuntimeError(f"expected (B,{self.cfg['in_chans']},H,W), got {tuple(x.shape)}")
        if x.shape[2] % self.ws or x.shape[3] % self.ws:
            raise RuntimeError(f"input size ({x.shape[2]},{x.shape[3]}) is not a multiple of window_size {self.ws}")

    def ocab_only(self, t: torch.Tensor, group: int, H: int, W: int) -> torch.Tensor:
        x = torch.zeros(t.shape[0], self.cfg["in_chans"], H, W, device=self.dev)
        with self._lock, torch.cuda.device(self.dev):
            return self._forward(x, only_ocab=(t.to(self.dev, torch.float32).contiguous(), group))

    def _forward(self, x: torch.Tensor, only_ocab=None, one_stream=None, sink=None) -> torch.Tensor:
        gen = self._forward_gen(x, only_ocab=only_ocab, one_stream=one_stream, sink=sink)
        try:
            req = next(gen)
        except StopIteration as done:
            return done.value
        raise RuntimeError(f"the unsharded forward must not reach an exchange point (got {req[0]!r})")

    def _forward_gen(self, x: torch.Tensor, only_ocab=None, band=None, one_stream=None, sink=None):
        self._check_input(x)
        if band is not None and self.naf is not None:
            raise NotImplementedError("a row band of a HybridHATNAF frame is not implemented: the stem's SCA pool needs one more "
                                      "reduce exchange and two more halo rows per NAF block")
        B, _, H, W = x.shape
        x = x.to(torch.float32).contiguous()
        w = dict(self._workspace(B, H, W, tag=(None if band is None else ("band", band.idx, band.n))))
        if band is not None and band.e1 - band.e0 != H:
            raise RuntimeError(f"band {band.idx} holds frame rows [{band.e0}, {band.e1}) but the input has {H} rows")
        f = _Fwd(self, w, B, H, W, band, self.opt.one_stream if one_stream is None else one_stream)
        if only_ocab is not None:
            t_in, gidx = only_ocab
            w["tB"].copy_(t_in.reshape(B, H * W, self.C))
            f.t = w["tB"]
            return (yield from self._ocab(f, self.layers[gidx], as_conv_input=False)).clone()
        if sink is None:
            y = torch.empty(B, self.cfg["in_chans"], H * self.scale, W * self.scale, dtype=torch.float32, device=self.dev)
        elif band is not None:
            raise RuntimeError(sink.band_refusal)
        else:
            y = sink.out
        if self.naf is not None:
            x = self._naf_stem(f, x)
        self._head(f, x)
# ... 244 lines not shown
            with torch.cuda.stream(s1):
                self._run_lin(oc.q, w["n"], w["q"], **geo, ldx=ldc, ldo=ldc)
            self._run_lin(oc.kv, kv_src, w["kv"], **geo, ldx=ldc, ldo=w["kv"].shape[2])
            s0.wait_stream(s1)
        self._ocab_attention(f, G, kv_src, qbuf, kvbuf, ldq, ldkv)
        tout = w["tB"] if t is w["tA"] else t
        if oc.proj.frag:
            self._run_lin(oc.proj, w["ao"], tout, **geo, ldx=ldc, ldo=C, out_mode=O_NHWC_F32, r1=t, ldr1=C,
                          ln=oc.n2, ln_out=w["n"], ld_ln=ldc)
        else:
            self._run_lin(oc.proj, w["ao"], tout, **geo, ldx=ldc, ldo=C, out_mode=O_NHWC_F32, r1=t, ldr1=C)
            f.ln(tout, w["n"], oc.n2)
        if oc.mlpf is not None:
            dst = w["ao"] if as_conv_input else tout
            ops.ocab_mlp(oc.mlpf, w["n"], tout, dst, B=f.B, H=f.H, W=f.W, ldx=ldc, ldr1=C, ldo=(ldc if as_conv_input else C),
                         out_f32=not as_conv_input, dtype=f.dt)
            return dst
        self._run_lin(oc.mlp0, w["n"], w["g"], **geo, ldx=ldc, ldo=w["g"].shape[2], act=ACT_GELU)
        if as_conv_input:
            self._run_lin(oc.mlp2, w["g"], w["ao"], **geo, ldx=w["g"].shape[2], ldo=ldc, out_mode=O_NHWC_T, r1=tout, ldr1=C)
            return w["ao"]
        self._run_lin(oc.mlp2, w["g"], tout, **geo, ldx=w["g"].shape[2], ldo=C, out_mode=O_NHWC_F32, r1=tout, ldr1=C)
        return tout

    def _ocab_attention(self, f: _Fwd, G: _Group, kv_src, qbuf, kvbuf, ldq, ldkv):
        w, oc, C, ldc, ws, wse = f.w, G.ocab, self.C, f.ldc, self.ws, self.wse
        if not (self.focus or self.topk < 1.0):
            ops.ocab_attention(qbuf, kvbuf, oc.bias_rot, w["ao"], B=f.B, H=f.H, W=f.W, C_=C, heads=G.heads, ws=ws, wse=wse,
                               ldq=ldq, ldkv=ldkv, ldo=ldc, dtype=f.dt, q_log2=oc.qlog2)
            return
        nk, pad = wse * wse, (wse - ws + 1) // 2
        if self.focus:
            ops.conv(oc.fh0, kv_src, w["fh"], **f.geo, ldx=ldc, ldo=w["fh"].shape[2], act=ACT_GELU, n_store=_r4(C // 4))
            ops.conv(oc.fh2, w["fh"], w["sal"], **f.geo, ldx=w["fh"].shape[2], ldo=8, n_store=4, out_mode=O_NHWC_F32)
        k_keep = max(1, int(self.topk * nk)) if self.topk < 1.0 else nk
        ops.ocab_keybias(w["sal"] if self.focus else None, kvbuf, w["kb"], B=f.B, H=f.H, W=f.W, C_=C, ws=ws, wse=wse, pad=pad,
                         k_keep=k_keep, ldsal=(-8 if f.dt == ops.HAT_BF16 else 8), ldkv=ldkv, dtype=f.dt)
        ops.ocab_attention_kb(qbuf, kvbuf, oc.bias_rot, w["kb"], w["ao"], B=f.B, H=f.H, W=f.W, C_=C, heads=G.heads, ws=ws,
                              wse=wse, pad=pad, ldq=ldq, ldkv=ldkv, ldo=ldc, dtype=f.dt)

    def _group_end(self, f: _Fwd, G: _Group, tout):
        w, tA, C = f.w, f.w["tA"], self.C
        if f.band is not None and G.conv is not None:
            yield ("halo", [(tout, 1)])
        if G.conv is None:
            ops.add_f32(tout, tA, tA, B=f.B, n=f.N * C)
            f.t = f.gin = tA
            f.have_n = f.have_n16 = False
            return
        lnkw = {}
        if G.conv_ln is not None:
            nxt, gap_c = G.conv_ln
            lnkw = dict(ln=nxt, ln_out=w["n"], ld_ln=f.ldc, gap_out=w["gap"], gap_c=gap_c, n16_out=(w["n16"] if self.use_n16 and gap_c else None))
            f.nblk = ops.conv_tiles(G.conv, f.H, f.W, f.dt)
        f.have_n = G.conv_ln is not None
        f.have_n16 = bool(f.have_n and self.use_n16 and G.conv_ln[1])
        gout = w["hA"] if G.out16 else tA
        if G.to_conv:
            ops.conv(G.conv, tout, gout, **f.geo, ldx=f.ldc, ldo=C, x_mode=X_NHWC_T, out_mode=O_NHWC_F32, r1=f.gin, ldr1=C, **lnkw)
        else:
            ops.conv(G.conv, tout, gout, **f.geo, ldx=C, ldo=C, x_mode=X_NHWC_F32, out_mode=O_NHWC_F32, r1=f.gin, ldr1=C, **lnkw)
        f.t = f.gin = gout

    def _body_end(self, f: _Fwd):
        w, tA, C, ldc = f.w, f.w["tA"], self.C, f.ldc
        if f.gin is not tA and not (f.have_n and self.conv_after_body is not None):
            raise RuntimeError("the FP16 residual stream reached a reader that takes fp32 only")
        if self.conv_after_body is None:
            if f.band is not None:
                yield ("halo", [(tA, 8)])
            f.ln(tA, w["tB"], self.norm, out_f32=True)
            ops.add_f32(w["tB"], w["f0"], w["tB"], B=f.B, n=f.N * C)
            ops.conv(self.conv_before_up, w["tB"], w["fb"], **f.geo, ldx=C, ldo=64, x_mode=X_NHWC_F32, act=ACT_LRELU)
            return
        if f.band is not None:
            yield ("halo", [((w["n"] if f.have_n else tA), 8)])
        if not f.have_n:
            f.ln(tA, w["n"], self.norm)
        ops.conv(self.conv_after_body, w["n"], w["c2"], **f.geo, ldx=ldc, ldo=ldc, r1=w["f0"], ldr1=C)
        ops.conv(self.conv_before_up, w["c2"], w["fb"], **f.geo, ldx=ldc, ldo=64, act=ACT_LRELU)

    def _upsample(self, f: _Fwd, y, sink=None):
        src, h, wd, dt = f.w["fb"], f.H, f.W, f.dt
        for (pw, rr), dst in zip(self.ups, f.w["ups"]):
            ops.conv(pw, src, dst, B=f.B, H=h, W=wd, dtype=dt, ldx=64, ldo=64, out_mode=O_PIXSHUF_T, ps_r=rr)
            src, h, wd = dst, h * rr, wd * rr
        r = float(self.cfg.get("img_range", 1.0))
        if sink is not None:
            if self.u8_fused and wd % 16 == 0 and sink.fusable:
                wpk, b8, _ = self.conv_last_sweep
                sink.fused(src, wpk, b8, B=f.B, H=h, W=wd, C_=64, ldx=64, out_scale=1.0 / r, mean=self._mean(), dtype=dt)
                return
            y = torch.empty(f.B, 3, h, wd, dtype=torch.float32, device=self.dev)
        if self.conv_last_sweep is not None and wd % 16 == 0:
            wpk, b8, nout = self.conv_last_sweep
            ops.conv3x3_to_planes(src, wpk, b8, y, B=f.B, H=h, W=wd, C_=64, ldx=64, n_out=nout, out_scale=1.0 / r, mean=self._mean(),
                                  dtype=dt)
        else:
            ops.conv(self.conv_last, src, y, B=f.B, H=h, W=wd, dtype=dt, ldx=64, ldo=0, out_mode=O_NCHW_F32,
                     out_scale=1.0 / r, mean=self._mean())
        if sink is not None:
            sink.from_planes(y)
```

super_resolution_amd/frame_boundary.py:

```python
from __future__ import annotations

from typing import Optional

import torch

from . import ops


class _Sink:
    kind = band_refusal = None
    fusable = True

    def __init__(self, eng, out, size):
        self.eng, self.out, self.size = eng, out, size

    def _count(self, how):
        name = f"{self.kind}_{how}_calls"
        setattr(self.eng, name, getattr(self.eng, name) + 1)


class _U8Sink(_Sink):
    kind, band_refusal = "u8", "a row band hands its rows over as fp32: the 8-bit output is the unsharded forward's"

    def __init__(self, eng, out, bgr):
        super().__init__(eng, out, tuple(out.shape[1:3]))
        self.bgr = bool(bgr)

    def fused(self, src, wpk, b8, **conv):
        ops.conv3x3_to_u8(src, wpk, b8, self.out, h_out=self.size[0], w_out=self.size[1], bgr=self.bgr, **conv)
        self._count("fused")

    def shuffled(self, rows, base, **geo):
        ops.shuffle_to_u8(rows, base, self.out, bgr=self.bgr, **geo)
        self._count("fused")

    def from_planes(self, y):
        ops.planes_to_u8(y, self.out, bgr=self.bgr)
        self._count("planes")


class _YuvSink(_Sink):
    kind, band_refusal = "yuv", "the 4:2:0 output is the unsharded forward's, and it is one target of three"

    def __init__(self, eng, out, views, from_rgb, *, sub, depth, msb, siting="center"):
        super().__init__(eng, out, tuple(views[0].shape[1:3]))
        self.views, self.from_rgb, self.surface = views, from_rgb, dict(sub=sub, depth=depth, msb=msb)
        self.siting = ops._siting(sub, siting)[0]
        self.fusable = self.siting == "center"

    def fused(self, src, wpk, b8, **conv):
        ops.conv3x3_to_yuv(src, wpk, b8, *self.views, from_rgb=self.from_rgb, **self.surface, **conv)
        self._count("fused")

    def shuffled(self, rows, base, **geo):
        ops.shuffle_to_yuv(rows, base, *self.views, self.from_rgb, **self.surface, **geo)
        self._count("fused")

    def from_planes(self, y):
        ops.planes_to_yuv(y, *self.views, self.from_rgb, siting=self.siting, **self.surface)
        self._count("planes")


class FrameBoundary:

    def _pad_multiple(self) -> int:
        return self.ws

    def _out_factor(self) -> int:
        return self.scale

    def forward_ensemble(self, x: torch.Tensor, n: int = 8, *, one_stream: Optional[bool] = None) -> torch.Tensor:
        n = ops.ensemble_members(n)
        if not x.is_cuda:
            raise RuntimeError("HAT forward needs a device tensor: the HIP path is the only path")
        if x.device != self.dev:
            raise RuntimeError(f"input is on {x.device} but this engine's weights and workspace live on {self.dev}")
        with self._lock, torch.cuda.device(self.dev):
            if n == 1:
                return self._forward(x, one_stream=one_stream)
            self._check_input(x)
            s = self._out_factor()
            acc = torch.empty(x.shape[0], x.shape[1], x.shape[2] * s, x.shape[3] * s, dtype=torch.float32, device=self.dev)
            return self._ensemble(x, n, acc, one_stream=one_stream)

    def _ws_buffer(self, ws, key, shape):
        t = ws.get(key)
        if t is None or tuple(t.shape) != tuple(shape):
            t = ws[key] = torch.zeros(shape, dtype=torch.float32, device=self.dev)
            ws["bytes"] += t.numel() * 4
        return t

    def _ens_acc(self, ws, B, Hp, Wp):
        return self._ws_buffer(ws, "ens_acc", (B, 3, Hp * self._out_factor(), Wp * self._out_factor()))

    def _ensemble(self, x, n, acc, one_stream=None):
        x = x.to(torch.float32).contiguous()
        B, C_, H, W = x.shape
        for i in range(n):
            if i == 0:
                xi = x
            else:
                Hi, Wi = (W, H) if i & 4 else (H, W)
                xi = self._ws_buffer(self._workspace(B, Hi, Wi), "ens_x", (B, C_, Hi, Wi))
                ops.dihedral(x, xi, op=i)
            y = self._forward(xi, one_stream=one_stream)
            if not y.is_contiguous():
                Hi, Wi = xi.shape[2:]
                y = self._ws_buffer(self._workspace(B, Hi, Wi), "ens_y", tuple(y.shape)).copy_(y)
            ops.dihedral(y, acc, op=i, inverse=True, alpha=1.0 / n, accumulate=i > 0)
        return acc

    def _check_u8(self):
        if self.cfg["in_chans"] != 3:
            raise RuntimeError(f"8-bit frames are three-channel images: in_chans={self.cfg['in_chans']} has no uint8 path "
                               f"(use forward() and convert the planes yourself)")

    def _u8_out(self, out, shape):
        if out is None:
            return torch.empty(shape, dtype=torch.uint8, device=self.dev)
        if out.dtype != torch.uint8 or tuple(out.shape) != tuple(shape) or out.device != self.dev or out.stride(3) != 1 or out.stride(2) != 3:
            raise RuntimeError(f"out must be a {tuple(shape)} uint8 tensor on {self.dev} with interleaved pixels, got "
                               f"{tuple(out.shape)} {out.dtype} on {out.device}")
        return out

    def _to_sink(self, x, sink, ensemble, one_stream=None):
        if ensemble > 1:
            B, _, Hp, Wp = x.shape
            sink.from_planes(self._ensemble(x, ensemble, self._ens_acc(self._workspace(B, Hp, Wp), B, Hp, Wp), one_stream=one_stream))
            return sink.out
        return self._forward(x, one_stream=one_stream, sink=sink)

    def _frame_forward(self, B, h, w, fill, make_sink, ensemble, what=None, of="frame"):
        m = self._pad_multiple()
        Hp, Wp = -(-h // m) * m, -(-w // m) * m
# ... 118 lines not shown
```

super_resolution_amd/ops.py:

```python
from __future__ import annotations

import collections
import ctypes as C
from typing import Optional

import torch

from . import _lib
from ._lib import (ACT_GELU, ACT_LRELU, ACT_LRELU02, ACT_NONE, HAT_BF16, HAT_F32, O_NCHW_F32, O_NHWC_F32, O_NHWC_T, O_PIXSHUF_T,
                   X_NCHW_F32_MEAN, X_NHWC_F32, X_NHWC_T, HatAggrCabDesc, HatCabFoldDesc, HatConvDesc, HatFfnDesc, HatHabTailDesc, HatMlpDesc, HatNafFoldDesc,
                   HatNafHalfDesc, HatEscConvFfnDesc)
from .packing import (ESC_HID_PAD, FP16_SAFE, KC, NAF_WIDTHS, TORCH_DTYPE, PackedConv, PackedEscFfn, PackedFFN, PackedMlp, PackedNafBlock, choose_nt,
                      esc_geo_ensemble, pack_esc_convffn, PackedEscRealSkip, ESCFP_HID_PAD, PackedEscFpLk, bicubic_phase_table, escfp_rank1_fold,
                      pack_escfp_convffn, pack_escfp_lk, dysample_fold, pack_escreal_skip, pack_nearest_conv,
                      LTE_HIDDEN, PackedLte, pack_lte,
                      UNI_UPSAMPLERS, PackedEscRealMSkip, conv_nearest_fold, pack_conv_nearest, pack_escrealm_skip, pack_pixshuf_conv, pixshuf_perm,
                      choose_nt_linear, naf_ffn_fold, naf_frags, pack_naf_block,
                      ffn_fp16_range_bound, pack_cab_squeeze, pack_cab_w2f, pack_conv_weight, pack_ffn, pack_ffn2, pack_ffn3,
                      pack_linear_weight, pack_ocab_mlp, pack_ocab_qkv, pack_pointwise)

DTYPE_CODE = {"f32": HAT_F32, "fp32": HAT_F32, "float32": HAT_F32, "bf16": HAT_BF16, "bfloat16": HAT_BF16}


def _ptr(t: Optional[torch.Tensor]) -> Optional[int]:
    if t is None:
        return None
    if not t.is_cuda:
        raise RuntimeError("HAT HIP ops need device tensors (no CPU path exists)")
    if not t.is_contiguous():
        raise RuntimeError("HAT HIP ops need contiguous tensors")
    return t.data_ptr()


def _stream() -> int:
    return torch.cuda.current_stream().cuda_stream


_prof = None


class profile:

    def __enter__(self):
        global _prof
        _prof = []
        return _prof

    def __exit__(self, *exc):
        global _prof
        _prof = None
        return False


def profiling() -> bool:
    return _prof is not None


def _timed(name, flops, fn, tag="", nbytes=0.0):
    if _prof is None:
        return fn()
    s, e = torch.cuda.Event(enable_timing=True), torch.cuda.Event(enable_timing=True)
    s.record()
    r = fn()
    e.record()
    _prof.append((name, float(flops), s, e, tag, float(nbytes)))
    return r


_TNAME = {HAT_F32: "float", HAT_BF16: "__bf16"}


def _mean4(mean):
    return (C.c_float * 4)(*[float(mean[i]) if i < len(mean) else 0.0 for i in range(4)])


def _stream16(r1, out, out_mode: int) -> int:
    h = 1 if r1 is not None and r1.dtype == torch.float16 else 0
    if out_mode == O_NHWC_F32 and out.dtype == torch.float16:
        h |= 2
    return h


def conv(pw: PackedConv, x: torch.Tensor, out: torch.Tensor, *, B: int, H: int, W: int, dtype: int, ldx: int, ldo: int,
         x_mode: int = X_NHWC_T, out_mode: int = O_NHWC_T, act: int = ACT_NONE, n_store: Optional[int] = None,
         x0: Optional[torch.Tensor] = None, c_split: int = 0, ldx0: int = 0,
         r1: Optional[torch.Tensor] = None, ldr1: int = 0, r2: Optional[torch.Tensor] = None, ldr2: int = 0,
         r2scale: Optional[torch.Tensor] = None, r2scale_bstride: int = 0, colsum: Optional[torch.Tensor] = None,
         ps_r: int = 0, in_scale: float = 1.0, out_scale: float = 1.0, mean=(0.0, 0.0, 0.0, 0.0), cin: Optional[int] = None,
         ln=None, ln_out: Optional[torch.Tensor] = None, ld_ln: int = 0, gap_out: Optional[torch.Tensor] = None, gap_c: int = 0,
         n16_out: Optional[torch.Tensor] = None):
    lib = _lib.load()
    d = HatConvDesc()
    if ln is not None:
        d.ln_g, d.ln_b, d.ln_out, d.ld_ln = _ptr(ln[0]), _ptr(ln[1]), _ptr(ln_out), ld_ln
    if gap_out is not None and gap_c:
        d.gap_out, d.gap_c = _ptr(gap_out), gap_c
    d.n16_out = _ptr(n16_out)
    d.x, d.x0, d.w, d.bias, d.out = _ptr(x), _ptr(x0), _ptr(pw.w), _ptr(pw.bias), _ptr(out)
    d.r1, d.r2, d.r2scale, d.colsum = _ptr(r1), _ptr(r2), _ptr(r2scale), _ptr(colsum)
    d.B, d.H, d.W = B, H, W
    d.Cin, d.ldx, d.x_mode = (pw.cin if cin is None else cin), ldx, x_mode
# ... 355 lines not shown
def _lte_grid_args(what: str, pl: PackedLte, coef, freq, inp, H: int, W: int, ldc: int, ldf: int, grid, cell_yx, out_affine):
    gh, gw = int(grid[0]), int(grid[1])
    if coef.dtype != torch.float32 or freq.dtype != torch.float32 or inp.dtype != torch.float32:
        raise ValueError(f"{what} expects fp32 coef / freq rows and fp32 input planes")
    if coef.numel() < (H * W - 1) * ldc + LTE_HIDDEN or freq.numel() < (H * W - 1) * ldf + LTE_HIDDEN or inp.numel() != 3 * H * W:
        raise ValueError(f"{what}: coef / freq / inp do not hold a {H}x{W} map")
    Q, hd = gh * gw, float(LTE_HIDDEN)
    flops = Q * (4.0 * (2.0 * hd * hd * 3 + 2.0 * hd * 3 + 5.0 * hd) + 30.0)
    nbytes = 4.0 * (min(4 * Q, H * W) * 2 * hd + 3 * H * W) + 3 * hd * hd * (2 if pl.w[0].element_size() == 2 else 4)
    args = (_ptr(coef), _ptr(freq), ldc, ldf, _ptr(inp), H, W, _ptr(pl.phase), _ptr(pl.w[0]), _ptr(pl.b[0]), _ptr(pl.w[1]), _ptr(pl.b[1]),
            _ptr(pl.w[2]), _ptr(pl.b[2]), _ptr(pl.w4), _ptr(pl.b4), gh, gw, float(cell_yx[0]), float(cell_yx[1]), float(out_affine[0]),
            float(out_affine[1]))
    return args, flops, nbytes


def lte_query_u8(pl: PackedLte, coef, freq, inp, out, *, H: int, W: int, ldc: int, ldf: int, dtype: int, grid, cell_yx=(0.0, 0.0),
                 out_affine=(1.0, 0.0), bgr: bool = False):
    lib = _lib.load()
    gh, gw = int(grid[0]), int(grid[1])
    o = out[0] if out.dim() == 4 and out.shape[0] == 1 else out
    if o.dtype != torch.uint8 or not o.is_cuda or tuple(o.shape) != (gh, gw, 3) or o.stride(2) != 1 or o.stride(1) != 3:
        raise RuntimeError(f"lte_query_u8 needs a ({gh},{gw},3) uint8 device destination with interleaved pixels, got {tuple(out.shape)} {out.dtype}")
    args, flops, nbytes = _lte_grid_args("lte_query_u8", pl, coef, freq, inp, H, W, ldc, ldf, grid, cell_yx, out_affine)
    _timed(f"lte_query_kernel<{_TNAME[dtype]}, u8>", flops, lambda: _lib.check(
        lib.hat_lte_query_u8(*args, o.data_ptr(), o.stride(0), int(bool(bgr)), dtype, _stream()), "hat_lte_query_u8"),
        tag=f"lte grid {gh}x{gw} on {H}x{W} -> u8", nbytes=nbytes + 3.0 * gh * gw)


def lte_query_yuv(pl: PackedLte, coef, freq, inp, y, cb, cr, from_rgb, *, H: int, W: int, ldc: int, ldf: int, dtype: int, grid,
                  cell_yx=(0.0, 0.0), out_affine=(1.0, 0.0), sub, depth: int = 8, msb=False):
    lib = _lib.load()
    gh, gw = int(grid[0]), int(grid[1])
    surf = yuv_surface(y, cb, cr, sub=sub, depth=depth, msb=msb, what="lte_query_yuv")
    if tuple(y.shape) != (1, gh, gw):
        raise RuntimeError(f"lte_query_yuv: a {gh}x{gw} grid needs a (1,{gh},{gw}) Y view, got {tuple(y.shape)}")
    args, flops, nbytes = _lte_grid_args("lte_query_yuv", pl, coef, freq, inp, H, W, ldc, ldf, grid, cell_yx, out_affine)
    m, name = _f12(from_rgb), _sub_name(sub, depth)
    _timed(f"lte_query_kernel<{_TNAME[dtype]}, {name}>", flops, lambda: _lib.check(
        lib.hat_lte_query_yuv(*args, C.byref(surf), m, dtype, _stream()), "hat_lte_query_yuv"),
        tag=f"lte grid {gh}x{gw} on {H}x{W} -> {name}", nbytes=nbytes + 3.0 * gh * gw)


LOG2E = 1.4426950408889634


def ocab_attention_log2_supported(C_: int, heads: int, ws: int, wse: int, dtype: int) -> bool:
    return dtype == HAT_BF16 and C_ % heads == 0 and C_ // heads == 24 and ws == 16 and wse == 24 and C_ % 8 == 0


def ocab_attention(q, kv, bias_rot, out, *, B: int, H: int, W: int, C_: int, heads: int, ws: int, wse: int, ldq: int,
                   ldkv: int, ldo: int, dtype: int, q_log2: bool = False):
    lib = _lib.load()
    fn, nm = (lib.hat_ocab_attention_log2, "hat_ocab_attention_log2") if q_log2 else (lib.hat_ocab_attention, "hat_ocab_attention")
    _timed(f"ocab_attn_kernel<{_TNAME[dtype]}>", 2.0 * 2 * wse * wse * C_ * B * H * W, lambda: _lib.check(
        fn(_ptr(q), _ptr(kv), _ptr(bias_rot), _ptr(out), B, H, W, C_, heads, ws, wse, ldq, ldkv, ldo, dtype, _stream()), nm))


def cab_squeeze_supported(C_: int, mid: int, W: int, dtype: int) -> bool:
    return dtype == HAT_BF16 and 128 < C_ <= 160 and C_ % 8 == 0 and mid <= 8 and W % 16 == 0


def conv3x3_to_planes_supported(nout: int, cin: int, W: int, dtype: int) -> bool:
    return dtype == HAT_BF16 and cin == 64 and nout <= 8 and W % 16 == 0


def conv3x3_to_planes(x, wpk, bias8, out, *, B: int, H: int, W: int, C_: int, ldx: int, n_out: int, out_scale: float, mean,
                      dtype: int):
    lib = _lib.load()
    m4 = _mean4(mean)
    _timed("cab_squeeze_kernel<2, planes>", 2.0 * B * H * W * 9 * C_ * n_out, lambda: _lib.check(
        lib.hat_conv3x3_to_planes(_ptr(x), _ptr(wpk), _ptr(bias8), _ptr(out), B, H, W, C_, ldx, n_out, out_scale, m4, dtype,
                                  _stream()), "hat_conv3x3_to_planes"), tag=f"k3 {C_}->{n_out} {H}x{W} row sweep planes")


def conv3x3_to_u8(x, wpk, bias8, out, *, B: int, H: int, W: int, C_: int, ldx: int, h_out: int, w_out: int, out_scale: float, mean,
                  bgr: bool, dtype: int):
    lib = _lib.load()
    m4 = _mean4(mean)
    if out.dtype != torch.uint8 or not out.is_cuda or tuple(out.shape) != (B, h_out, w_out, 3) or out.stride(-1) != 1 or out.stride(-2) != 3:
        raise RuntimeError("conv3x3_to_u8 needs a (B,h_out,w_out,3) uint8 device destination with interleaved pixels")
    _timed("cab_squeeze_kernel<2, u8>", 2.0 * B * H * W * 9 * C_ * 3, lambda: _lib.check(
        lib.hat_conv3x3_to_u8(_ptr(x), _ptr(wpk), _ptr(bias8), out.data_ptr(), out.stride(1), out.stride(0), B, H, W, C_, ldx, h_out, w_out,
                              out_scale, m4, int(bgr), dtype, _stream()), "hat_conv3x3_to_u8"), tag=f"k3 {C_}->3 {H}x{W} row sweep u8")


def u8_to_planes(src, dst, *, bgr: bool = False):
    lib = _lib.load()
    B, h, w, c = src.shape
    if c != 3 or src.dtype != torch.uint8 or src.stride(-1) != 1 or src.stride(-2) != 3 or dst.dtype != torch.float32:
        raise RuntimeError("u8_to_planes needs (B,h,w,3) uint8 with interleaved pixels and an fp32 destination")
    if not src.is_cuda:
        raise RuntimeError("HAT HIP ops need device tensors (no CPU path exists)")
    if dst.dim() != 4 or dst.shape[0] != B or dst.shape[1] != 3 or dst.shape[2] < h or dst.shape[3] < w or dst.device != src.device:
        raise RuntimeError(f"u8_to_planes needs a (B,3,Hp>=h,Wp>=w) destination on {src.device}, got {tuple(dst.shape)} on {dst.device} "
                           f"for frames {tuple(src.shape)}")
    _timed("u8_to_planes_kernel", 0.0, lambda: _lib.check(
        lib.hat_u8_to_planes(src.data_ptr(), src.stride(1), src.stride(0), _ptr(dst), B, h, w, dst.shape[2], dst.shape[3], int(bgr),
                             _stream()), "hat_u8_to_planes"), tag=f"u8 {h}x{w} -> planes {dst.shape[2]}x{dst.shape[3]}")


def planes_to_u8(src, dst, *, bgr: bool = False):
    lib = _lib.load()
    B, c, Hs, Ws = src.shape
    if c != 3 or src.dtype != torch.float32 or dst.dtype != torch.uint8 or dst.shape[0] != B or dst.shape[3] != 3 or dst.stride(-1) != 1 \
            or dst.stride(-2) != 3 or not dst.is_cuda:
        raise RuntimeError("planes_to_u8 needs (B,3,Hs,Ws) fp32 planes and a (B,h,w,3) uint8 device destination with interleaved pixels")
    _timed("planes_to_u8_kernel", 0.0, lambda: _lib.check(
        lib.hat_planes_to_u8(_ptr(src), B, Hs, Ws, dst.data_ptr(), dst.stride(1), dst.stride(0), dst.shape[1], dst.shape[2], int(bgr),
                             _stream()), "hat_planes_to_u8"), tag=f"planes {Hs}x{Ws} -> u8 {dst.shape[1]}x{dst.shape[2]}")


ENSEMBLE_SIZES = (1, 2, 4, 8)


def ensemble_members(n) -> int:
    if isinstance(n, bool) or not isinstance(n, int) or n not in ENSEMBLE_SIZES:
        raise ValueError(f"the self-ensemble runs the first 1, 2, 4 or 8 of the eight flips / transposes, got {n!r}")
    return n


def dihedral(src, dst, *, op: int, inverse: bool = False, alpha: float = 1.0, accumulate: bool = False):
    lib = _lib.load()
    if src.dtype != torch.float32 or dst.dtype != torch.float32 or src.dim() < 2 or src.device != dst.device:
        raise RuntimeError(f"dihedral needs fp32 planes on one device, got {src.dtype} on {src.device} and {dst.dtype} on {dst.device}")
    if not 0 <= int(op) <= 7:
        raise RuntimeError(f"dihedral: op is one of the eight members 0..7, got {op}")
    H, W = src.shape[-2:]
    want = tuple(src.shape[:-2]) + ((W, H) if op & 4 else (H, W))
    if tuple(dst.shape) != want:
        raise RuntimeError(f"dihedral: member {op} of {tuple(src.shape)} planes needs a {want} destination, got {tuple(dst.shape)}")
    planes = src.numel() // (H * W)
    _timed("dihedral_transpose_kernel" if op & 4 else "dihedral_flip_kernel", 0.0, lambda: _lib.check(
        lib.hat_dihedral_f32(_ptr(src), _ptr(dst), planes, H, W, int(op), int(bool(inverse)), float(alpha), int(bool(accumulate)), _stream()),
        "hat_dihedral_f32"), tag=f"dihedral op {op}{' inv' if inverse else ''} {planes}x{H}x{W}", nbytes=4.0 * src.numel() * (3 if accumulate else 2))


resize_calls = 0
_RESIZE_TABLES_KEPT = 32
_resize_tables = collections.OrderedDict()
_resize_mid = {}


def _resize_workspace(dev, B: int, oh: int, w: int):
    key, n = (str(dev), _stream()), B * 3 * oh * w
    buf = _resize_mid.get(key)
    if buf is None or buf.numel() < n:
        _resize_mid.pop(key, None)
        buf = _resize_mid[key] = torch.empty(n, dtype=torch.float32, device=dev)
    return buf[:n].view(B, 3, oh, w)


def _resize_axis(dev, in_len: int, scale: float, antialiasing: bool) -> dict:
    import numpy as np

    from . import resize as _rz
    out_len = _rz.out_length(in_len, scale)
    key = (str(dev), int(in_len), out_len, float(scale), bool(antialiasing))
    t = _resize_tables.get(key)
    if t is not None:
        _resize_tables.move_to_end(key)
    else:
        try:
            w, s, _, _ = _rz.tables(in_len, out_len, scale, antialiasing)
        except ValueError as e:
            raise RuntimeError(str(e)) from e
        t = {"w": torch.from_numpy(w).to(dev).contiguous(), "src": torch.from_numpy(_rz.mirror(s, in_len).astype(np.int32)).to(dev).contiguous(),
# ... 262 lines not shown
        st, o_cb, o_cr = (frame.stride(0), 2 * cw, 2), off + (kind == "semi_vu"), off + (kind == "semi")
    return frame[:, :h], frame.as_strided((B, ch, cw), st, o_cb), frame.as_strided((B, ch, cw), st, o_cr)


def yuv_surface(y, cb, cr, *, sub, depth: int = 8, msb=False, what: str = "yuv_surface"):
    if y.dim() != 3 or y.dtype not in (torch.uint8, torch.uint16):
        raise TypeError(f"{what} needs uint8 (or uint16) (B,h,w) views, got {y.dtype} {tuple(y.shape)}")
    if (y.dtype == torch.uint8) != (depth == 8) or depth not in (8, 10, 12, 16):
        raise TypeError(f"{what}: depth {depth} does not go with {y.dtype} views (uint8 holds 8-bit samples, uint16 10, 12 or 16 bits)")
    if (cb is None) != (cr is None) or (cb is None) != (sub is None):
        raise RuntimeError(f"{what}: a grey surface has neither Cb nor Cr nor a subsampling; every other one has all three")
    if not y.is_cuda or y.stride(2) != 1:
        raise RuntimeError("HAT HIP ops need device tensors with unit-step rows (no CPU path exists)")
    n, (B, h, w) = y.element_size(), y.shape
    s = _lib.HatYuvSurface(y=y.data_ptr(), y_pitch=n * y.stride(1), y_bstride=n * y.stride(0), depth=int(depth), msb=int(bool(msb)))
    if cb is not None:
        sx, sy = int(sub[0]), int(sub[1])
        if (sx, sy) not in ((1, 1), (1, 0), (0, 0)) or (sx and w % 2) or (sy and h % 2):
            raise RuntimeError(f"{what}: a {h}x{w} frame has no chroma subsampling {(sx, sy)} (w even where sub_x = 1, h where sub_y = 1)")
        if cb.dtype != y.dtype or cr.dtype != y.dtype or not (cb.is_cuda and cr.is_cuda) or tuple(cb.shape) != (B, h >> sy, w >> sx) \
                or tuple(cr.shape) != tuple(cb.shape) or cb.stride() != cr.stride() or cb.stride(2) not in (1, 2):
            raise RuntimeError(f"{what} needs Cb, Cr ({B},{h >> sy},{w >> sx}) views of Y's dtype and one pitch with a step of 1 or 2 samples")
        s.cb, s.cr, s.c_pitch, s.c_step, s.c_bstride, s.sub_x, s.sub_y = cb.data_ptr(), cr.data_ptr(), n * cb.stride(1), n * cb.stride(2), \
            n * cb.stride(0), sx, sy
    return s


def _sub_name(sub, depth):
    return ("gray" if sub is None else {(1, 1): "yuv420", (1, 0): "yuv422", (0, 0): "yuv444"}[tuple(sub)]) + ("" if depth == 8 else f"p{depth}")


def _siting(sub, siting):
    from . import yuv as _yuv
    eff = _yuv.effective_siting(sub, siting)
    return eff, _yuv.SITINGS.index(eff)


def yuv_to_planes(y, cb, cr, dst, to_rgb, *, sub, depth: int = 8, msb=False, siting: str = "center"):
    lib = _lib.load()
    eff, code = _siting(sub, siting)
    surf = yuv_surface(y, cb, cr, sub=sub, depth=depth, msb=msb, what="yuv_to_planes")
    B, h, w = y.shape
    _planes_dst("yuv_to_planes", dst, y, contiguous=True)
    m, name = _f12(to_rgb), _sub_name(sub, depth)
    if code:
        _timed(f"yuv_to_planes_sited_kernel<{name}, {eff}>", 0.0, lambda: _lib.check(
            lib.hat_yuv_to_planes_sited(C.byref(surf), code, _ptr(dst), B, h, w, dst.shape[2], dst.shape[3], m, _stream()),
            "hat_yuv_to_planes_sited"), tag=f"{name} {eff} {h}x{w} -> planes {dst.shape[2]}x{dst.shape[3]}")
        return
    _timed(f"yuv_to_planes_kernel<{name}>", 0.0, lambda: _lib.check(
        lib.hat_yuv_to_planes(C.byref(surf), _ptr(dst), B, h, w, dst.shape[2], dst.shape[3], m, _stream()), "hat_yuv_to_planes"),
        tag=f"{name} {h}x{w} -> planes {dst.shape[2]}x{dst.shape[3]}")


def planes_to_yuv(src, y, cb, cr, from_rgb, *, sub, depth: int = 8, msb=False, siting: str = "center"):
    lib = _lib.load()
    eff, code = _siting(sub, siting)
    surf = yuv_surface(y, cb, cr, sub=sub, depth=depth, msb=msb, what="planes_to_yuv")
    B, h, w = y.shape
    _planes_src("planes_to_yuv", src, y, contiguous=True)
    m, name = _f12(from_rgb), _sub_name(sub, depth)
    if code:
        _timed(f"planes_to_yuv_sited_kernel<{name}, {eff}>", 0.0, lambda: _lib.check(
            lib.hat_planes_to_yuv_sited(_ptr(src), B, src.shape[2], src.shape[3], C.byref(surf), code, h, w, m, _stream()),
            "hat_planes_to_yuv_sited"), tag=f"planes {src.shape[2]}x{src.shape[3]} -> {name} {eff} {h}x{w}")
        return
    _timed(f"planes_to_yuv_kernel<{name}>", 0.0, lambda: _lib.check(
        lib.hat_planes_to_yuv(_ptr(src), B, src.shape[2], src.shape[3], C.byref(surf), h, w, m, _stream()), "hat_planes_to_yuv"),
        tag=f"planes {src.shape[2]}x{src.shape[3]} -> {name} {h}x{w}")


def conv3x3_to_yuv(x, wpk, bias8, y, cb, cr, *, sub, B: int, H: int, W: int, C_: int, ldx: int, out_scale: float, mean, from_rgb, dtype: int,
                   depth: int = 8, msb=False):
    lib = _lib.load()
    surf = yuv_surface(y, cb, cr, sub=sub, depth=depth, msb=msb, what="conv3x3_to_yuv")
    if y.shape[0] != B:
        raise RuntimeError(f"conv3x3_to_yuv: destination batch {y.shape[0]} != {B}")
    m4, m, name = _mean4(mean), _f12(from_rgb), _sub_name(sub, depth)
    _timed(f"cab_squeeze_kernel<2, {name}>", 2.0 * B * H * W * 9 * C_ * 3, lambda: _lib.check(
        lib.hat_conv3x3_to_yuv(_ptr(x), _ptr(wpk), _ptr(bias8), C.byref(surf), B, H, W, C_, ldx, y.shape[1], y.shape[2], out_scale, m4, m, dtype,
                               _stream()), "hat_conv3x3_to_yuv"), tag=f"k3 {C_}->3 {H}x{W} row sweep {name}")


def u8_metrics_flags(*, y_channel: bool, bgr: bool, psnr: bool, ssim: bool) -> int:
    return (_lib.METRICS_Y if y_channel else 0) | (_lib.METRICS_BGR if bgr else 0) | (_lib.METRICS_PSNR if psnr else 0) \
        | (_lib.METRICS_SSIM if ssim else 0)


def u8_metrics_workspace_bytes(B: int, h: int, w: int, *, crop_border: int, y_channel: bool, bgr: bool = False, psnr: bool = True,
                               ssim: bool = True) -> int:
    lib = _lib.load()
    n = C.c_int64(0)
    _lib.check(lib.hat_u8_metrics_workspace_bytes(B, h, w, crop_border, u8_metrics_flags(y_channel=y_channel, bgr=bgr, psnr=psnr, ssim=ssim),
                                                  C.byref(n)), "hat_u8_metrics_workspace_bytes")
    return n.value


def u8_metrics(a, b, sums, workspace, *, crop_border: int, y_channel: bool, bgr: bool = False, psnr: bool = True, ssim: bool = True):
    lib = _lib.load()
    for t in (a, b):
        if t.dim() != 4 or t.shape[3] != 3 or t.dtype != torch.uint8 or t.stride(-1) != 1 or t.stride(-2) != 3:
            raise RuntimeError("u8_metrics needs (B,h,w,3) uint8 frames with interleaved pixels")
        if not t.is_cuda:
            raise RuntimeError("HAT HIP ops need device tensors (no CPU path exists)")
    if a.shape != b.shape or a.device != b.device:
        raise RuntimeError(f"u8_metrics needs two frames of one shape on one device, got {tuple(a.shape)} on {a.device} and "
                           f"{tuple(b.shape)} on {b.device}")
    B, h, w, _ = a.shape
    if sums.dtype != torch.float64 or tuple(sums.shape) != (B, 4) or sums.device != a.device or workspace.device != a.device:
        raise RuntimeError(f"u8_metrics needs a (B,4) float64 destination and a workspace on {a.device}")
    need = u8_metrics_workspace_bytes(B, h, w, crop_border=crop_border, y_channel=y_channel, bgr=bgr, psnr=psnr, ssim=ssim)
    if workspace.dtype != torch.uint8 or workspace.numel() < need or workspace.data_ptr() % 8:
        raise RuntimeError(f"u8_metrics needs an 8-byte aligned uint8 workspace of at least {need} bytes")
    flags = u8_metrics_flags(y_channel=y_channel, bgr=bgr, psnr=psnr, ssim=ssim)
    nch = 1 if y_channel else 3
    hc, wc = h - 2 * crop_border, w - 2 * crop_border
    flops = 2.0 * B * nch * (hc - 10) * (wc - 10) * 5 * 22 if ssim else 0.0
    _timed(f"u8_metrics_kernel<{'y' if y_channel else 'rgb'}>", flops, lambda: _lib.check(
        lib.hat_u8_metrics(a.data_ptr(), a.stride(1), a.stride(0), b.data_ptr(), b.stride(1), b.stride(0), B, h, w, crop_border, flags,
                           _ptr(sums), _ptr(workspace), _stream()), "hat_u8_metrics"),
        tag=f"u8 metrics {h}x{w} crop {crop_border}{' psnr' if psnr else ''}{' ssim' if ssim else ''}", nbytes=2.0 * B * h * w * 3)


_niqe_buffers = {}


def niqe_workspace(B: int, h: int, w: int, *, crop_border: int):
    lib = _lib.load()
    H, W, n = C.c_int32(0), C.c_int32(0), C.c_int64(0)
    _lib.check(lib.hat_niqe_workspace_bytes(B, h, w, crop_border, C.byref(H), C.byref(W), C.byref(n)), "hat_niqe_workspace_bytes")
    return H.value, W.value, n.value


def _niqe_buffers_for(dev, B, h, w, crop_border):
    import numpy as np

    from . import niqe as _nq
    key = (str(dev), B, h, w, crop_border)
    buf = _niqe_buffers.get(key)
    if buf is None:
        H, W, nbytes = niqe_workspace(B, h, w, crop_border=crop_border)
        ws = torch.empty(nbytes // 4, dtype=torch.float32, device=dev)
        px, views, o = B * H * W, [], 0
        for shape in ((B, H, W), (B, H, W), (B, H // 2, W), (B, H // 2, W // 2)):
            n = shape[0] * shape[1] * shape[2]
            views.append(ws[o:o + n].view(shape))
            o += n
        assert o * 4 == nbytes and px == views[0].numel()
        win = np.ascontiguousarray(_nq.gaussian_window(), dtype=np.float64)
        buf = _niqe_buffers[key] = {"plane": views[0], "unit": views[1], "mid": views[2], "half": views[3], "window": win,
                                    "stats96": torch.zeros(B, H // 96, W // 96, 25, dtype=torch.float64, device=dev),
                                    "stats48": torch.zeros(B, H // 96, W // 96, 25, dtype=torch.float64, device=dev)}
    return buf


def niqe_stats(frame_u8, *, crop_border: int, bgr: bool = False):
    lib = _lib.load()
    f = frame_u8
    if not isinstance(f, torch.Tensor) or not f.is_cuda:
        raise RuntimeError("niqe_stats needs a uint8 device tensor (no CPU path exists: niqe.stats_of is the host definition)")
    if f.dim() == 3:
        f = f.unsqueeze(0)
    if f.dim() != 4 or f.shape[3] != 3 or f.dtype != torch.uint8 or f.stride(3) != 1 or f.stride(2) != 3:
        raise RuntimeError(f"niqe_stats needs (B,h,w,3) uint8 frames with interleaved pixels, got {tuple(frame_u8.shape)} {frame_u8.dtype}")
    B, h, w, _ = f.shape
    crop_border = int(crop_border)
# ... 243 lines not shown
```

super_resolution_amd/packing.py:

```python
from __future__ import annotations

from typing import Optional

import torch

from ._lib import HAT_BF16, HAT_F32

TORCH_DTYPE = {HAT_F32: torch.float32, HAT_BF16: torch.bfloat16}
KC = {HAT_F32: 32, HAT_BF16: 64}


class PackedConv:
    __slots__ = ("w", "bias", "ksize", "cin", "kpad", "nt", "n_slices", "nout", "w_bstride", "frag", "ksplit")

    def __init__(self, w, bias, ksize, cin, kpad, nt, n_slices, nout, w_bstride=0, frag=False):
        self.w, self.bias, self.ksize, self.cin, self.kpad = w, bias, ksize, cin, kpad
        self.nt, self.n_slices, self.nout, self.w_bstride = nt, n_slices, nout, w_bstride
        self.frag = frag
        self.ksplit = None

    @property
    def npad(self):
        return self.nt * 16 * self.n_slices

# ... 423 lines not shown
    wf, bf = escreal_skip_fold(w0, _f32(sd[p + ".0.bias"]), dw, _f32(sd[p + ".1.bias"]))
    f = PackedEscRealSkip()
    f.w1 = frags(_pad(wf.permute(0, 2, 3, 1).reshape(128, 147), 128, 160)).to(TORCH_DTYPE[dtype]).contiguous().to(device)
    f.b1 = bf.contiguous().to(device)
    f.w3 = frags(w3.reshape(64, 128)).to(TORCH_DTYPE[dtype]).contiguous().to(device)
    f.b3 = _f32(sd[p + ".3.bias"]).contiguous().to(device)
    return f


def pack_nearest_conv(weight, bias, dtype: int, device) -> PackedConv:
    wf, bf = nearest_conv_fold(_f32(weight), _f32(bias))
    o = weight.shape[0]
    n = torch.arange(4 * o)
    return pack_conv_weight(wf, bf, dtype, device, out_perm=(n % o) * 4 + n // o)


UNI_UPSAMPLERS = ("conv", "pixelshuffledirect", "pixelshuffle", "nearest+conv", "dysample")


class PackedEscRealMSkip:
    __slots__ = ("cin", "w0", "b0", "dw", "bdw", "w3", "b3")


def pack_escrealm_skip(sd, p: str, dtype: int, device) -> PackedEscRealMSkip:
    w0, dw, w3 = _f32(sd[p + ".1.weight"]), _f32(sd[p + ".2.weight"]), _f32(sd[p + ".4.weight"])
    cin = w0.shape[1]
    if cin not in (12, 48) or tuple(w0.shape) != (128, cin, 1, 1) or tuple(dw.shape) != (128, 1, 7, 7) or tuple(w3.shape) != (64, 128, 1, 1):
        raise ValueError(f"skip branch {tuple(w0.shape)} / {tuple(dw.shape)} / {tuple(w3.shape)} is not supported: hat_escrealm_skip is "
                         "built for 12 or 48 -> 128 (1x1), depthwise 7x7, 128 -> 64 (1x1)")
    f = PackedEscRealMSkip()
    f.cin = cin
    f.w0, f.b0 = w0.reshape(128, cin).contiguous().to(device), _f32(sd[p + ".1.bias"]).contiguous().to(device)
    f.dw, f.bdw = dw.reshape(128, 49).contiguous().to(device), _f32(sd[p + ".2.bias"]).contiguous().to(device)
    f.w3 = frags(w3.reshape(64, 128)).to(TORCH_DTYPE[dtype]).contiguous().to(device)
    f.b3 = _f32(sd[p + ".4.bias"]).contiguous().to(device)
    return f


def pixshuf_perm(o: int, r: int) -> torch.Tensor:
    n = torch.arange(o)
    cps = o // (r * r)
    return (n % cps) * (r * r) + n // cps


def conv_nearest_fold(w, b, r: int):
    return w.repeat_interleave(r * r, 0), b.repeat_interleave(r * r)


def pack_conv_nearest(weight, bias, r: int, dtype: int, device) -> PackedConv:
    if r not in (2, 3):
        raise ValueError(f"nearest x{r} is not supported: the fold is built for 2 and 3")
    wf, bf = conv_nearest_fold(_f32(weight), _f32(bias), r)
    return pack_conv_weight(wf, bf, dtype, device, out_perm=pixshuf_perm(wf.shape[0], r))


def pack_pixshuf_conv(weight, bias, r: int, dtype: int, device) -> PackedConv:
    return pack_conv_weight(weight, bias, dtype, device, out_perm=pixshuf_perm(weight.shape[0], r))


LTE_HIDDEN = 256


class PackedLte:
    __slots__ = ("taps", "phase", "w", "b", "w4", "b4")


def pack_lte(sd, dtype: int, device) -> PackedLte:
    hd = LTE_HIDDEN
    if tuple(sd["coef.weight"].shape[:1]) != (hd,) or tuple(sd["freq.weight"].shape[:1]) != (hd,) or tuple(sd["phase.weight"].shape) != (hd // 2, 2):
        raise ValueError(f"ESC-LTE with hidden_dim={sd['coef.weight'].shape[0]} is not supported: hat_lte_query is built for hidden_dim {hd}")
    shapes = [tuple(sd[f"imnet.layers.{i}.weight"].shape) for i in (0, 2, 4, 6) if f"imnet.layers.{i}.weight" in sd]
    if shapes != [(hd, hd)] * 3 + [(3, hd)] or "imnet.layers.8.weight" in sd:
        raise ValueError(f"ESC-LTE with an imnet of layer shapes {shapes} is not supported: hat_lte_query is built for hidden_list "
                         f"({hd}, {hd}, {hd}) and out_dim 3")
    p = PackedLte()
    p.taps = pack_conv_weight(torch.cat([_f32(sd["coef.weight"]), _f32(sd["freq.weight"])]),
                              torch.cat([_f32(sd["coef.bias"]), _f32(sd["freq.bias"])]), dtype, device)
    p.phase = _f32(sd["phase.weight"]).contiguous().to(device)
    p.w = [frags(_f32(sd[f"imnet.layers.{i}.weight"])).to(TORCH_DTYPE[dtype]).contiguous().to(device) for i in (0, 2, 4)]
    p.b = [_f32(sd[f"imnet.layers.{i}.bias"]).contiguous().to(device) for i in (0, 2, 4)]
    p.w4 = _f32(sd["imnet.layers.6.weight"]).contiguous().to(device)
    p.b4 = _f32(sd["imnet.layers.6.bias"]).contiguous().to(device)
    return p
```

Before: 340.5 MP/s.

## Fold the final PixelShuffle(2) conv pair into one 5x5 sub-pixel kernel

Adds a new upfold kernel that algebraically composes the last upsample conv, PixelShuffle(2) and the 3x3 conv_last into a single 5x5 64->2x2x3 convolution, with border-variant weights so zero padding at the image edges stays exact. It writes planes, u8 or YUV output directly from the low-resolution feature map. This removes the 64-channel high-resolution intermediate and its extra conv pass. The plan executor recognises the new folded ending and routes it to the fused sinks. Precomposed weights in bf16 may change rounding slightly, and the code is restricted to 64->3 channels with W a multiple of 16.

```diff
diff --git a/include/hat_mi355x.h b/include/hat_mi355x.h
--- a/include/hat_mi355x.h
+++ b/include/hat_mi355x.h
@@ -15,7 +15,8 @@
 enum { HAT_ACT_NONE = 0, HAT_ACT_GELU = 1 , HAT_ACT_LRELU = 2 ,
        HAT_ACT_LRELU02 = 3  };
 enum { HAT_X_NHWC_T = 0, HAT_X_NHWC_F32 = 1, HAT_X_NCHW_F32_MEAN = 2 };
-enum { HAT_O_NHWC_T = 0, HAT_O_NHWC_F32 = 1, HAT_O_PIXSHUF_T = 2, HAT_O_NCHW_F32 = 3 };
+enum { HAT_O_NHWC_T = 0, HAT_O_NHWC_F32 = 1, HAT_O_PIXSHUF_T = 2, HAT_O_NCHW_F32 = 3,
+       HAT_O_FOLD2_NCHW_F32 = 4  };
 
 typedef struct HatConvDesc {
     const void* x;
@@ -187,6 +188,15 @@
                        int32_t ldx, int32_t h_out, int32_t w_out, float out_scale, const float* mean4, const float* from_rgb12,
                        int32_t dtype, void* stream);
 
+int hat_upfold_to_planes(const void* x, const void* wpk, const float* bias, float* out, int32_t B, int32_t H, int32_t W, int32_t ldx,
+                         float out_scale, float mean_r, float mean_g, float mean_b, int32_t dtype, void* stream);
+int hat_upfold_to_u8(const void* x, const void* wpk, const float* bias, uint8_t* dst, int64_t dst_pitch, int64_t dst_bstride, int32_t B,
+                     int32_t H, int32_t W, int32_t ldx, int32_t h_out, int32_t w_out, float out_scale, float mean_r, float mean_g,
+                     float mean_b, int32_t bgr, int32_t dtype, void* stream);
+int hat_upfold_to_yuv(const void* x, const void* wpk, const float* bias, const HatYuvSurface* dst, int32_t B, int32_t H, int32_t W,
+                      int32_t ldx, int32_t h_out, int32_t w_out, float out_scale, float mean_r, float mean_g, float mean_b,
+                      const float* from_rgb12, int32_t dtype, void* stream);
+
 #define HAT_SITING_CENTER 0
 #define HAT_SITING_LEFT 1
 #define HAT_SITING_TOPLEFT 2
diff --git a/super_resolution_amd/_lib.py b/super_resolution_amd/_lib.py
--- a/super_resolution_amd/_lib.py
+++ b/super_resolution_amd/_lib.py
@@ -11,7 +11,7 @@
 HAT_F32, HAT_BF16 = 0, 1
 ACT_NONE, ACT_GELU, ACT_LRELU, ACT_LRELU02 = 0, 1, 2, 3
 X_NHWC_T, X_NHWC_F32, X_NCHW_F32_MEAN = 0, 1, 2
-O_NHWC_T, O_NHWC_F32, O_PIXSHUF_T, O_NCHW_F32 = 0, 1, 2, 3
+O_NHWC_T, O_NHWC_F32, O_PIXSHUF_T, O_NCHW_F32, O_FOLD2_NCHW_F32 = 0, 1, 2, 3, 4
 METRICS_Y, METRICS_BGR, METRICS_PSNR, METRICS_SSIM = 1, 2, 4, 8
 
 _ERRORS = {-1: "HAT_EINVAL (bad argument)", -2: "HAT_ELDS (tile does not fit in 160 KiB LDS)",
@@ -191,6 +191,10 @@
                                     C.c_void_p]),
     "hat_conv3x3_to_yuv": (C.c_int, [C.c_void_p, C.c_void_p, C.c_void_p, C.POINTER(HatYuvSurface)] + [C.c_int32] * 7 + [C.c_float, C.c_void_p,
                                                                                                         C.c_void_p, C.c_int32, C.c_void_p]),
+    "hat_upfold_to_planes": (C.c_int, [C.c_void_p] * 4 + [C.c_int32] * 4 + [C.c_float] * 4 + [C.c_int32, C.c_void_p]),
+    "hat_upfold_to_u8": (C.c_int, [C.c_void_p] * 4 + [C.c_int64, C.c_int64] + [C.c_int32] * 6 + [C.c_float] * 4 + [C.c_int32, C.c_int32, C.c_void_p]),
+    "hat_upfold_to_yuv": (C.c_int, [C.c_void_p, C.c_void_p, C.c_void_p, C.POINTER(HatYuvSurface)] + [C.c_int32] * 6 + [C.c_float] * 4
+                          + [C.c_void_p, C.c_int32, C.c_void_p]),
     "hat_plan_forward_yuv": (C.c_int, [C.c_void_p, C.POINTER(HatYuvSurface), C.POINTER(HatYuvSurface), C.c_int32, C.c_int32, C.c_void_p,
                                        C.c_void_p, C.c_void_p]),
     "hat_yuv_to_planes_sited": (C.c_int, [C.POINTER(HatYuvSurface), C.c_int32, C.c_void_p] + [C.c_int32] * 5 + [C.c_void_p, C.c_void_p]),
diff --git a/super_resolution_amd/build.py b/super_resolution_amd/build.py
--- a/super_resolution_amd/build.py
+++ b/super_resolution_amd/build.py
@@ -8,7 +8,7 @@
 HERE = os.path.dirname(os.path.abspath(__file__))
 CSRC = os.path.join(HERE, "csrc")
 LIB = os.path.join(HERE, "libhat_mi355x.so")
-SOURCES = ["hat_conv.hip", "hat_conv64r.hip", "hat_attn.hip", "hat_misc.hip", "hat_ffn.hip", "hat_ffn2.hip", "hat_tail3.hip", "hat_tail3l.hip", "hat_pw.hip", "hat_mlp.hip", "hat_cabsq.hip", "hat_esc13.hip", "hat_u8.hip", "hat_yuv.hip", "hat_resize.hip", "hat_pil_resize.hip", "hat_metrics.hip", "hat_dihedral.hip", "hat_niqe.hip", "hat_naf.hip", "hat_esc.hip", "hat_escreal.hip", "hat_escrealm.hip", "hat_escfp.hip", "hat_lte.hip", "hat_esc_sink.hip", "hat_plan.cpp"]
+SOURCES = ["hat_conv.hip", "hat_conv64r.hip", "hat_attn.hip", "hat_misc.hip", "hat_ffn.hip", "hat_ffn2.hip", "hat_tail3.hip", "hat_tail3l.hip", "hat_pw.hip", "hat_mlp.hip", "hat_cabsq.hip", "hat_esc13.hip", "hat_upfold.hip", "hat_u8.hip", "hat_yuv.hip", "hat_resize.hip", "hat_pil_resize.hip", "hat_metrics.hip", "hat_dihedral.hip", "hat_niqe.hip", "hat_naf.hip", "hat_esc.hip", "hat_escreal.hip", "hat_escrealm.hip", "hat_escfp.hip", "hat_lte.hip", "hat_esc_sink.hip", "hat_plan.cpp"]
 HEADERS = [os.path.join(CSRC, "hat_common.h"), os.path.join(CSRC, "hat_yuv_check.h"), os.path.join(CSRC, "hat_yuv_sample.h"), os.path.join(CSRC, "hat_frame_sink.h"), os.path.join(CSRC, "hat_esc_ffn.h"), os.path.join(CSRC, "hat_plan_parse.h"), os.path.join(os.path.dirname(HERE), "include", "hat_mi355x.h")]
 FLAGS = ["-O3", "--offload-arch=gfx950", "-fPIC", "-std=c++17", "-Wall", "-Wno-unused-function"]
 
diff --git a/super_resolution_amd/csrc/hat_conv.hip b/super_resolution_amd/csrc/hat_conv.hip
--- a/super_resolution_amd/csrc/hat_conv.hip
+++ b/super_resolution_amd/csrc/hat_conv.hip
@@ -4,6 +4,7 @@
 
 bool hat_conv64r_can_launch(const HatConvDesc& d);
 int hat_conv64r_launch(const HatConvDesc& d, hipStream_t s);
+int hat_upfold_launch_desc(const HatConvDesc& d, hipStream_t s);
 
 #ifndef HAT_CONV_PIPE
 #define HAT_CONV_PIPE 1
@@ -597,10 +598,11 @@
 extern "C" int hat_conv(const HatConvDesc* dp, void* stream) {
     if (!dp) return HAT_EINVAL;
     const HatConvDesc& d = *dp;
+    hipStream_t s = reinterpret_cast<hipStream_t>(stream);
+    if (d.out_mode == HAT_O_FOLD2_NCHW_F32) return hat_upfold_launch_desc(d, s);
     int rc = conv_validate(d);
     if (rc) return rc;
     TileCfg tc; size_t lds;
-    hipStream_t s = reinterpret_cast<hipStream_t>(stream);
     if (hat_conv64r_can_launch(d)) return hat_conv64r_launch(d, s);
     if (!conv_pick(d, &tc, &lds)) return HAT_ELDS;
     if (d.dtype == HAT_BF16) return dispatch_tile<bf16_t>(d, tc, lds, s);
diff --git a/super_resolution_amd/csrc/hat_plan.cpp b/super_resolution_amd/csrc/hat_plan.cpp
--- a/super_resolution_amd/csrc/hat_plan.cpp
+++ b/super_resolution_amd/csrc/hat_plan.cpp
@@ -1,6 +1,7 @@
 #include <hip/hip_runtime.h>
 #include <stdint.h>
 #include <stdio.h>
+#include <stddef.h>
 #include <string.h>
 
 #include <string>
@@ -175,14 +176,32 @@
     return false;
 }
 
-bool ends_in_planes(const hat_plan* p) {
-    if (p->calls.empty()) return false;
+enum Ending { ENDS_OTHER = 0, ENDS_CONV_LAST, ENDS_FOLDED };
+Ending ending_of(const hat_plan* p) {
+    if (p->calls.empty()) return ENDS_OTHER;
     const Call& c = p->calls.back();
-    if (c.fn != FN_hat_conv3x3_to_planes || c.args.size() != 14 || c.args[3].tag != ARG_PTR || c.args[3].buf >= p->bufs.size()) return false;
-    if (p->bufs[c.args[3].buf].kind != BUF_OUTPUT || c.args[3].off != 0 || c.args[9].i != 3) return false;
+    Ending e = ENDS_OTHER;
+    if (c.fn == FN_hat_conv3x3_to_planes) {
+        if (c.args.size() != 14 || c.args[3].tag != ARG_PTR || c.args[3].buf >= p->bufs.size()) return ENDS_OTHER;
+        if (p->bufs[c.args[3].buf].kind != BUF_OUTPUT || c.args[3].off != 0 || c.args[9].i != 3) return ENDS_OTHER;
+        e = ENDS_CONV_LAST;
+    } else if (c.fn == FN_hat_conv) {
+        if (c.args.size() != 2 || c.args[0].tag != ARG_STRUCT || c.args[0].blob.size() != sizeof(HatConvDesc)) return ENDS_OTHER;
+        HatConvDesc d;
+        memcpy(&d, c.args[0].blob.data(), sizeof(d));
+        if (d.out_mode != HAT_O_FOLD2_NCHW_F32) return ENDS_OTHER;
+        bool out_ok = false;
+        for (const Fix& fx : c.args[0].fix)
+            if (fx.field_off == offsetof(HatConvDesc, out))
+                out_ok = fx.buf != NULL_BUF && fx.buf < p->bufs.size() && p->bufs[fx.buf].kind == BUF_OUTPUT && fx.off == 0;
+        if (!out_ok) return ENDS_OTHER;
+        e = ENDS_FOLDED;
+    } else {
+        return ENDS_OTHER;
+    }
     for (size_t k = 0; k + 1 < p->calls.size(); ++k)
-        if (addresses_output(p, p->calls[k])) return false;
-    return true;
+        if (addresses_output(p, p->calls[k])) return ENDS_OTHER;
+    return e;
 }
 
 template <typename Source, typename Fused, typename Planes>
@@ -190,7 +209,8 @@
     const int32_t B = p->dims[0], H = p->dims[2], W = p->dims[3], s = p->dims[4];
     int dev = -1;
     if (hipGetDevice(&dev) != hipSuccess || dev != p->device) return HAT_EINVAL;
-    const bool fused = may_fuse && ends_in_planes(p);
+    const Ending ending = may_fuse ? ending_of(p) : ENDS_OTHER;
+    const bool fused = ending != ENDS_OTHER;
     if (!p->stage_in) {
         const hipError_t e = hipMalloc((void**)&p->stage_in, (size_t)B * 3 * H * W * sizeof(float));
         if (e != hipSuccess) { p->stage_in = nullptr; return (int)e; }
@@ -209,7 +229,7 @@
     }
     if (!fused) return planes_sink(p->stage_out, s * H, s * W);
     Resolved r{p, &p->calls.back(), p->stage_in, nullptr, stream, {}};
-    return fused_sink(r);
+    return fused_sink(r, ending);
 }
 
 int frame_fits(const hat_plan* p, int32_t h, int32_t w) {
@@ -232,7 +252,12 @@
             if (hat_siting_of(src, src_siting) == HAT_SITING_CENTER) return hat_yuv_to_planes(src, in, B, h, w, H, W, to_rgb12, stream);
             return hat_yuv_to_planes_sited(src, src_siting, in, B, h, w, H, W, to_rgb12, stream);
         },
-        [&](Resolved& r) {
+        [&](Resolved& r, Ending ending) {
+            if (ending == ENDS_FOLDED) {
+                const HatConvDesc* d = (const HatConvDesc*)r.P(0);
+                return hat_upfold_to_yuv(d->x, d->w, d->bias, dst, d->B, d->H, d->W, d->ldx, ho, wo, d->out_scale, d->mean[0], d->mean[1], d->mean[2],
+                                         from_rgb12, d->dtype, stream);
+            }
             return hat_conv3x3_to_yuv(r.P(0), r.P(1), (const float*)r.P(2), dst, r.I(4), r.I(5), r.I(6), r.I(7), r.I(8), ho, wo, r.F(10),
                                       (const float*)r.P(11), from_rgb12, r.I(12), stream);
         },
@@ -259,7 +284,12 @@
     const int bgr = flags & 1, ho = s * h, wo = s * w;
     return forward_frames(
         p, stream, [&](float* in) { return hat_u8_to_planes(src, src_pitch, src_pitch * h, in, B, h, w, H, W, bgr, stream); },
-        [&](Resolved& r) {
+        [&](Resolved& r, Ending ending) {
+            if (ending == ENDS_FOLDED) {
+                const HatConvDesc* d = (const HatConvDesc*)r.P(0);
+                return hat_upfold_to_u8(d->x, d->w, d->bias, dst, dst_pitch, dst_pitch * ho, d->B, d->H, d->W, d->ldx, ho, wo, d->out_scale, d->mean[0],
+                                        d->mean[1], d->mean[2], bgr, d->dtype, stream);
+            }
             return hat_conv3x3_to_u8(r.P(0), r.P(1), (const float*)r.P(2), dst, dst_pitch, dst_pitch * ho, r.I(4), r.I(5), r.I(6), r.I(7), r.I(8),
                                      ho, wo, r.F(10), (const float*)r.P(11), bgr, r.I(12), stream);
         },
diff --git a/super_resolution_amd/csrc/hat_upfold.hip b/super_resolution_amd/csrc/hat_upfold.hip
--- /dev/null
+++ b/super_resolution_amd/csrc/hat_upfold.hip
@@ -0,0 +1,266 @@
+#include <type_traits>
+
+#include "hat_frame_sink.h"
+
+namespace {
+
+constexpr int F_TR = 16, F_TC = 32, F_HALO = 2;
+constexpr int F_HR = F_TR + 2 * F_HALO, F_HC = F_TC + 2 * F_HALO;
+constexpr int F_NFRAG = 50, F_WAVES = 8, F_THREADS = F_WAVES * 64;
+constexpr int F_X_OFF = F_NFRAG * 1024;
+constexpr int F_LDS = F_X_OFF + F_HR * F_HC * 128;
+constexpr int F_VARIANT = F_NFRAG * 512;
+static_assert(F_LDS <= HAT_LDS_MAX, "weights + haloed tile must fit the LDS");
+
+struct FoldEpi { float out_scale; float mean[3]; };
+struct FoldEpiU8 { float out_scale; float mean[3]; int h_out, w_out, bgr; long long pitch, bstride; };
+template <typename T, int SX, int SY, bool GREY> struct FoldEpiYuv {
+    float out_scale; float mean[3]; int h_out, w_out; HatCsc k; HatSample<T> q; HatYuvDst<T> d;
+};
+template <typename E> struct FoldYuvTraits { static constexpr bool yuv = false, grey = false; static constexpr int sx = 1, sy = 1; };
+template <typename T, int SX, int SY, bool G> struct FoldYuvTraits<FoldEpiYuv<T, SX, SY, G>> {
+    static constexpr bool yuv = true, grey = G; static constexpr int sx = SX, sy = SY;
+};
+
+__device__ __forceinline__ unsigned fold_x_addr(int hy, int hx, int s) {
+    return (unsigned)((hy * F_HC + hx) * 128 + ((s ^ ((hx >> 1) & 7)) << 4));
+}
+
+template <typename Epi>
+__global__ __launch_bounds__(F_THREADS) void upfold_kernel(const bf16_t* __restrict__ x, int ldx, const bf16_t* __restrict__ wpk,
+                                                           const float* __restrict__ bias, void* __restrict__ outv, int H, int W,
+                                                           int tiles_x, int ntiles, Epi epi) {
+    typedef __bf16 bf8 __attribute__((ext_vector_type(8)));
+    constexpr bool U8 = std::is_same<Epi, FoldEpiU8>::value;
+    using YT = FoldYuvTraits<Epi>;
+    constexpr bool YUV = YT::yuv;
+    constexpr bool C420 = YUV && !YT::grey && YT::sx == 1 && YT::sy == 1, C422 = YUV && !YT::grey && YT::sx == 1 && YT::sy == 0;
+    constexpr bool C444 = YUV && !YT::grey && YT::sx == 0;
+    extern __shared__ __attribute__((aligned(16))) char smem[];
+    const int tid = threadIdx.x, lane = tid & 63, g = lane >> 4, c16 = lane & 15;
+    const int wave = __builtin_amdgcn_readfirstlane(tid >> 6);
+    const int b = blockIdx.y;
+    const bf16_t* xb = x + (size_t)b * H * W * ldx;
+    const int Ho = 2 * H, Wo = 2 * W;
+
+    for (int i = tid; i < F_NFRAG * 64; i += F_THREADS)
+        *reinterpret_cast<u32x4*>(smem + i * 16) = *reinterpret_cast<const u32x4*>(wpk + (size_t)i * 8);
+    const f32x4 bias0 = *reinterpret_cast<const f32x4*>(bias + 4 * g);
+
+    auto finish = [&](f32x4 acc, f32x4 bs, int py, int px, bool ok) {
+        const int oy = 2 * py + (g >> 1), ox = 2 * px + (g & 1);
+        float rgb[3];
+#pragma unroll
+        for (int m = 0; m < 3; ++m) rgb[m] = __builtin_fmaf(acc[m] + bs[m], epi.out_scale, epi.mean[m]);
+        if constexpr (YUV) {
+            float Yv, cbv, crv;
+            hat_rgb_to_ycc(epi.k, rgb[0], rgb[1], rgb[2], Yv, cbv, crv);
+            [[maybe_unused]] float cbs = cbv, crs = crv, cbo = 0.f, cro = 0.f;
+            if constexpr (C420 || C422) {
+                cbs = hat_add_rn(cbv, __shfl_xor(cbv, 16));
+                crs = hat_add_rn(crv, __shfl_xor(crv, 16));
+            }
+            if constexpr (C420) {
+                cbo = __shfl_xor(cbs, 32);
+                cro = __shfl_xor(crs, 32);
+            }
+            if (ok && oy < epi.h_out && ox < epi.w_out) {
+                yuv_store_luma(epi.d, epi.q, b, oy, ox, Yv);
+                if constexpr (C420) {
+                    if (g == 0 && oy + 1 < epi.h_out) yuv_store_chroma420(epi.d, epi.q, epi.k, b, py, px, cbs, cbo, crs, cro);
+                } else if constexpr (C422) {
+                    if (!(g & 1)) yuv_store_chroma422(epi.d, epi.q, epi.k, b, oy, px, cbs, crs);
+                } else if constexpr (C444) {
+                    yuv_store_chroma444(epi.d, epi.q, epi.k, b, oy, ox, cbv, crv);
+                }
+            }
+        } else if constexpr (U8) {
+            if (ok && oy < epi.h_out && ox < epi.w_out) {
+                uint8_t* p = reinterpret_cast<uint8_t*>(outv) + (size_t)b * epi.bstride + (size_t)oy * epi.pitch + (size_t)ox * 3;
+#pragma unroll
+                for (int m = 0; m < 3; ++m) p[epi.bgr ? 2 - m : m] = (uint8_t)hat_unit_to_u8(rgb[m]);
+            }
+        } else {
+            if (ok) {
+                float* of = reinterpret_cast<float*>(outv) + (size_t)b * 3 * Ho * Wo + (size_t)oy * Wo + ox;
+#pragma unroll
+                for (int m = 0; m < 3; ++m) of[(size_t)m * Ho * Wo] = rgb[m];
+            }
+        }
+    };
+
+    auto slow_group = [&](int v, int hy, int hx) -> f32x4 {
+        const bf16_t* wv = wpk + (size_t)v * F_VARIANT + lane * 8;
+        f32x4 acc = {0.f, 0.f, 0.f, 0.f};
+#pragma nounroll
+        for (int ty = 0; ty < 5; ++ty) {
+#pragma unroll
+            for (int tx = 0; tx < 5; ++tx)
+#pragma unroll
+                for (int ks = 0; ks < 2; ++ks) {
+                    const bf8 a = __builtin_bit_cast(bf8, *reinterpret_cast<const u32x4*>(wv + ((ty * 5 + tx) * 2 + ks) * 512));
+                    const bf8 bf = __builtin_bit_cast(bf8, *reinterpret_cast<const u32x4*>(smem + F_X_OFF + fold_x_addr(hy + ty - 2, hx + tx - 2, ks * 4 + g)));
+                    acc = __builtin_amdgcn_mfma_f32_16x16x32_bf16(a, bf, acc, 0, 0, 0);
+                }
+        }
+        return acc;
+    };
+
+    constexpr int NPIECE = F_HR * F_HC * 8, NIT = (NPIECE + F_THREADS - 1) / F_THREADS;
+    u32x4 pv[NIT];
+    auto fetch = [&](int t) {
+        const int tc = min(t, ntiles - 1);
+        const int ty0 = (tc / tiles_x) * F_TR, tx0 = (tc - (tc / tiles_x) * tiles_x) * F_TC;
+#pragma unroll
+        for (int it = 0; it < NIT; ++it) {
+            const int i = min(tid + it * F_THREADS, NPIECE - 1);
+            const int hp = i >> 3, s = i & 7;
+            const int hy = hp / F_HC, hx = hp - hy * F_HC;
+            const int y = ty0 - F_HALO + hy, xx = tx0 - F_HALO + hx;
+            const bool in = y >= 0 && y < H && xx >= 0 && xx < W;
+            const u32x4 v = *reinterpret_cast<const u32x4*>(xb + ((size_t)min(max(y, 0), H - 1) * W + min(max(xx, 0), W - 1)) * ldx + s * 8);
+            pv[it] = in ? v : u32x4{0u, 0u, 0u, 0u};
+        }
+    };
+    const int q4 = 4 * (wave >> 1), ch = wave & 1;
+    fetch(blockIdx.x);
+    for (int t = blockIdx.x; t < ntiles; t += gridDim.x) {
+        const int ty0 = (t / tiles_x) * F_TR, tx0 = (t - (t / tiles_x) * tiles_x) * F_TC;
+#pragma unroll
+        for (int it = 0; it < NIT; ++it) {
+            const int i = tid + it * F_THREADS;
+            if (i < NPIECE) {
+                const int hp = i >> 3, hx = hp % F_HC;
+                *reinterpret_cast<u32x4*>(smem + F_X_OFF + hp * 128 + (((i & 7) ^ ((hx >> 1) & 7)) << 4)) = pv[it];
+            }
+        }
+        __syncthreads();
+        fetch(t + gridDim.x);
+
+        const int px = tx0 + 16 * ch + c16;
+        if (tx0 + 16 * ch < W) {
+            f32x4 acc[4];
+#pragma unroll
+            for (int j = 0; j < 4; ++j) acc[j] = f32x4{0.f, 0.f, 0.f, 0.f};
+#pragma unroll
+            for (int tx = 0; tx < 5; ++tx) {
+                const int hx = 16 * ch + c16 + tx;
+#pragma unroll
+                for (int ks = 0; ks < 2; ++ks) {
+                    bf8 rowf[8];
+#pragma unroll
+                    for (int i = 0; i < 8; ++i)
+                        rowf[i] = __builtin_bit_cast(bf8, *reinterpret_cast<const u32x4*>(smem + F_X_OFF + fold_x_addr(q4 + i, hx, ks * 4 + g)));
+#pragma unroll
+                    for (int ty = 0; ty < 5; ++ty) {
+                        const bf8 a = __builtin_bit_cast(bf8, *reinterpret_cast<const u32x4*>(smem + ((ty * 5 + tx) * 2 + ks) * 1024 + lane * 16));
+#pragma unroll
+                        for (int j = 0; j < 4; ++j) acc[j] = __builtin_amdgcn_mfma_f32_16x16x32_bf16(a, rowf[j + ty], acc[j], 0, 0, 0);
+                    }
+                    __builtin_amdgcn_sched_barrier(0);
+                }
+            }
+#pragma unroll
+            for (int j = 0; j < 4; ++j) {
+                const int py = ty0 + q4 + j;
+                finish(acc[j], bias0, py, px, py > 0 && py < H - 1 && px > 0 && px < W - 1);
+            }
+        }
+
+        const int rs_top = 1 + (H == 1 ? 2 : 0);
+        const bool has_top = ty0 == 0, has_bot = H > 1 && ty0 + F_TR >= H;
+        const bool has_left = tx0 == 0, has_right = tx0 + F_TC >= W;
+        if (wave < 4) {
+            const bool top = wave < 2;
+            const int py = top ? 0 : H - 1, half = wave & 1;
+            const int pxr = tx0 + 16 * half + c16;
+            if ((top ? has_top : has_bot) && tx0 + 16 * half < W) {
+                const int v = 3 * (top ? rs_top : 2);
+                const f32x4 acc = slow_group(v, py - ty0 + F_HALO, 16 * half + c16 + F_HALO);
+                finish(acc, *reinterpret_cast<const f32x4*>(bias + v * 16 + 4 * g), py, pxr, pxr > 0 && pxr < W - 1);
+            }
+        } else if (wave < 6) {
+            const bool left = wave == 4;
+            if (left ? has_left : has_right) {
+                const int pxc = left ? 0 : W - 1, cs = left ? 1 : 2;
+                const int py = ty0 + c16, hy = c16 + F_HALO, hx = pxc - tx0 + F_HALO;
+                const int rs = (py == 0 ? 1 : 0) | (py == H - 1 ? 2 : 0);
+                f32x4 acc = slow_group(cs, hy, hx);
+                if (has_top) {
+                    const f32x4 a2 = slow_group(3 * rs_top + cs, hy, hx);
+                    if (py == 0) acc = a2;
+                }
+                if (has_bot) {
+                    const f32x4 a2 = slow_group(3 * 2 + cs, hy, hx);
+                    if (py == H - 1 && py != 0) acc = a2;
+                }
+                const int rsc = py < H ? rs : 0;
+                finish(acc, *reinterpret_cast<const f32x4*>(bias + (3 * rsc + cs) * 16 + 4 * g), py, pxc, py < H);
+            }
+        }
+        __syncthreads();
+    }
+}
+
+int fold_args_ok(const void* x, const void* wpk, const float* bias, int B, int H, int W, int ldx, int dtype) {
+    if (!x || !wpk || !bias || B < 1 || H < 1 || W < 16 || W % 16 || ldx < 64 || ldx % 8) return HAT_EINVAL;
+    if (H > (1 << 14) || W > (1 << 14)) return HAT_EINVAL;
+    if (dtype != HAT_BF16) return HAT_EUNSUPPORTED;
+    return (reinterpret_cast<uintptr_t>(x) | reinterpret_cast<uintptr_t>(wpk) | reinterpret_cast<uintptr_t>(bias)) % 16 ? HAT_EINVAL : 0;
+}
+
+template <typename Epi>
+int launch_fold(const void* x, const void* wpk, const float* bias, void* out, int B, int H, int W, int ldx, const Epi& epi, void* stream) {
+    const int tiles_x = (W + F_TC - 1) / F_TC, tiles_y = (H + F_TR - 1) / F_TR, ntiles = tiles_x * tiles_y;
+    int gx = 256 / B;
+    if (gx < 1) gx = 1;
+    if (gx > ntiles) gx = ntiles;
+    hipError_t e = hipFuncSetAttribute(reinterpret_cast<const void*>(upfold_kernel<Epi>), hipFuncAttributeMaxDynamicSharedMemorySize, F_LDS);
+    if (e != hipSuccess) return (int)e;
+    HAT_LAUNCH(upfold_kernel<Epi>, dim3(gx, B), dim3(F_THREADS), F_LDS, reinterpret_cast<hipStream_t>(stream), reinterpret_cast<const bf16_t*>(x),
+               ldx, reinterpret_cast<const bf16_t*>(wpk), bias, out, H, W, tiles_x, ntiles, epi);
+    return hat_check_launch();
+}
+
+}
+
+extern "C" int hat_upfold_to_planes(const void* x, const void* wpk, const float* bias, float* out, int32_t B, int32_t H, int32_t W,
+                                    int32_t ldx, float out_scale, float mean_r, float mean_g, float mean_b, int32_t dtype, void* stream) {
+    if (!out) return HAT_EINVAL;
+    if (const int rc = fold_args_ok(x, wpk, bias, B, H, W, ldx, dtype)) return rc;
+    return launch_fold(x, wpk, bias, out, B, H, W, ldx, FoldEpi{out_scale, {mean_r, mean_g, mean_b}}, stream);
+}
+
+int hat_upfold_launch_desc(const HatConvDesc& d, hipStream_t s) {
+    if (d.ksize != 5 || d.Cin != 64 || d.x_mode != HAT_X_NHWC_T || d.act != HAT_ACT_NONE || d.w_bstride != 0 || d.reserved0 != 0) return HAT_EINVAL;
+    if (d.x0 || d.r1 || d.r2 || d.r2scale || d.colsum || d.ln_out || d.gap_out || d.n16_out) return HAT_EINVAL;
+    return hat_upfold_to_planes(d.x, d.w, d.bias, reinterpret_cast<float*>(d.out), d.B, d.H, d.W, d.ldx, d.out_scale, d.mean[0], d.mean[1],
+                                d.mean[2], d.dtype, s);
+}
+
+extern "C" int hat_upfold_to_u8(const void* x, const void* wpk, const float* bias, uint8_t* dst, int64_t dst_pitch, int64_t dst_bstride,
+                                int32_t B, int32_t H, int32_t W, int32_t ldx, int32_t h_out, int32_t w_out, float out_scale, float mean_r,
+                                float mean_g, float mean_b, int32_t bgr, int32_t dtype, void* stream) {
+    if (!dst || h_out < 1 || w_out < 1) return HAT_EINVAL;
+    if (const int rc = fold_args_ok(x, wpk, bias, B, H, W, ldx, dtype)) return rc;
+    if (h_out > 2 * H || w_out > 2 * W) return HAT_EINVAL;
+    if (dst_pitch < 3 * (int64_t)w_out || (B > 1 && dst_bstride < dst_pitch * (int64_t)(h_out - 1) + 3 * (int64_t)w_out)) return HAT_EINVAL;
+    return launch_fold(x, wpk, bias, dst, B, H, W, ldx,
+                       FoldEpiU8{out_scale, {mean_r, mean_g, mean_b}, h_out, w_out, bgr ? 1 : 0, (long long)dst_pitch, (long long)dst_bstride}, stream);
+}
+
+extern "C" int hat_upfold_to_yuv(const void* x, const void* wpk, const float* bias, const HatYuvSurface* dst, int32_t B, int32_t H, int32_t W,
+                                 int32_t ldx, int32_t h_out, int32_t w_out, float out_scale, float mean_r, float mean_g, float mean_b,
+                                 const float* from_rgb12, int32_t dtype, void* stream) {
+    if (!from_rgb12) return HAT_EINVAL;
+    if (const int rc = fold_args_ok(x, wpk, bias, B, H, W, ldx, dtype)) return rc;
+    if (h_out > 2 * H || w_out > 2 * W || !hat_yuv_surface_ok(dst, B, h_out, w_out)) return HAT_EINVAL;
+    int rc = 0;
+    yuv_dispatch(*dst, [&](auto L, auto q) {
+        using T = typename decltype(L)::sample_t;
+        using Epi = FoldEpiYuv<T, L.sx, L.sy, L.grey>;
+        rc = launch_fold(x, wpk, bias, dst->y, B, H, W, ldx,
+                         Epi{out_scale, {mean_r, mean_g, mean_b}, h_out, w_out, load_csc(from_rgb12), q, yuv_dst<T>(*dst)}, stream);
+    });
+    return rc;
+}
diff --git a/super_resolution_amd/engine.py b/super_resolution_amd/engine.py
--- a/super_resolution_amd/engine.py
+++ b/super_resolution_amd/engine.py
@@ -41,6 +41,7 @@
     no_ocab_qkv: bool = False
     no_bf16_conv_in: bool = False
     no_conv_ln: bool = False
+    no_upfold: bool = False
 
     @classmethod
     def from_env(cls, env=None) -> "Options":
@@ -205,6 +206,12 @@
         self.conv_last_sweep = None
         if ops.conv3x3_to_planes_supported(wl.shape[0], wl.shape[1], 16, self.dtype) and not self.opt.no_cab_sweep:
             self.conv_last_sweep = ops.pack_cab_squeeze(wl, sd["conv_last.bias"], dev) + (wl.shape[0],)
+        self.upfold = None
+        if self.ups and self.ups[-1][1] == 2 and self.conv_last_sweep is not None and not self.opt.no_upfold:
+            key = f"upsample.{2 * (len(self.ups) - 1)}"
+            wu = sd[key + ".weight"]
+            if ops.upfold_supported(wu.shape[1], wl.shape[0], 2, 16, self.dtype) and wl.shape[1] * 4 == wu.shape[0]:
+                self.upfold = ops.pack_upfold(wu, sd[key + ".bias"], wl, sd["conv_last.bias"], dev)
 
     def _pack_naf(self, sd):
         c, nb = int(self.cfg["naf"]["width"]), int(self.cfg["naf"]["blocks"])
@@ -408,10 +415,17 @@
             w["x_naf"] = z(B, self.cfg["in_chans"], H, W, dtype=f)
         h, wd = H, W
         w["ups"] = []
-        for _, r in self.ups:
+        for i, (_, r) in enumerate(self.ups):
             h, wd = h * r, wd * r
-            w["ups"].append(z(B, h * wd, 64))
+            w["ups"].append(None if i + 1 == len(self.ups) and self._folded(W) else z(B, h * wd, 64))
         return w
+
+    def _folded(self, W: int) -> bool:
+        if self.upfold is None:
+            return False
+        for _, r in self.ups[:-1]:
+            W *= r
+        return ops.upfold_supported(64, 3, 2, W, self.dtype)
 
     def _esc_w(self, esc: _ESC, w, B, H, W, nblk, gap=None):
         ops.esc_weights(w["gap"] if gap is None else gap, nblk, H * W, esc.w1, esc.b1, esc.w2, esc.b2, esc.plk, w["weff"], B=B,
@@ -822,10 +836,22 @@
 
     def _upsample(self, f: _Fwd, y, sink=None):
         src, h, wd, dt = f.w["fb"], f.H, f.W, f.dt
-        for (pw, rr), dst in zip(self.ups, f.w["ups"]):
+        fold = self._folded(f.W)
+        for (pw, rr), dst in list(zip(self.ups, f.w["ups"]))[:len(self.ups) - int(fold)]:
             ops.conv(pw, src, dst, B=f.B, H=h, W=wd, dtype=dt, ldx=64, ldo=64, out_mode=O_PIXSHUF_T, ps_r=rr)
             src, h, wd = dst, h * rr, wd * rr
         r = float(self.cfg.get("img_range", 1.0))
+        if fold:
+            kw = dict(B=f.B, H=h, W=wd, ldx=64, out_scale=1.0 / r, mean=self._mean(), dtype=dt)
+            if sink is not None and sink.fusable:
+                sink.folded(src, self.upfold, **kw)
+                return
+            if sink is not None:
+                y = torch.empty(f.B, 3, 2 * h, 2 * wd, dtype=torch.float32, device=self.dev)
+            ops.upfold_to_planes(src, self.upfold, y, **kw)
+            if sink is not None:
+                sink.from_planes(y)
+            return
         if sink is not None:
             if self.u8_fused and wd % 16 == 0 and sink.fusable:
                 wpk, b8, _ = self.conv_last_sweep
diff --git a/super_resolution_amd/frame_boundary.py b/super_resolution_amd/frame_boundary.py
--- a/super_resolution_amd/frame_boundary.py
+++ b/super_resolution_amd/frame_boundary.py
@@ -28,6 +28,10 @@
 
     def fused(self, src, wpk, b8, **conv):
         ops.conv3x3_to_u8(src, wpk, b8, self.out, h_out=self.size[0], w_out=self.size[1], bgr=self.bgr, **conv)
+        self._count("fused")
+
+    def folded(self, src, pf, **conv):
+        ops.upfold_to_u8(src, pf, self.out, h_out=self.size[0], w_out=self.size[1], bgr=self.bgr, **conv)
         self._count("fused")
 
     def shuffled(self, rows, base, **geo):
@@ -50,6 +54,10 @@
 
     def fused(self, src, wpk, b8, **conv):
         ops.conv3x3_to_yuv(src, wpk, b8, *self.views, from_rgb=self.from_rgb, **self.surface, **conv)
+        self._count("fused")
+
+    def folded(self, src, pf, **conv):
+        ops.upfold_to_yuv(src, pf, *self.views, from_rgb=self.from_rgb, **self.surface, **conv)
         self._count("fused")
 
     def shuffled(self, rows, base, **geo):
diff --git a/super_resolution_amd/ops.py b/super_resolution_amd/ops.py
--- a/super_resolution_amd/ops.py
+++ b/super_resolution_amd/ops.py
@@ -7,7 +7,7 @@
 import torch
 
 from . import _lib
-from ._lib import (ACT_GELU, ACT_LRELU, ACT_LRELU02, ACT_NONE, HAT_BF16, HAT_F32, O_NCHW_F32, O_NHWC_F32, O_NHWC_T, O_PIXSHUF_T,
+from ._lib import (ACT_GELU, ACT_LRELU, ACT_LRELU02, ACT_NONE, HAT_BF16, HAT_F32, O_FOLD2_NCHW_F32, O_NCHW_F32, O_NHWC_F32, O_NHWC_T, O_PIXSHUF_T,
                    X_NCHW_F32_MEAN, X_NHWC_F32, X_NHWC_T, HatAggrCabDesc, HatCabFoldDesc, HatConvDesc, HatFfnDesc, HatHabTailDesc, HatMlpDesc, HatNafFoldDesc,
                    HatNafHalfDesc, HatEscConvFfnDesc)
 from .packing import (ESC_HID_PAD, FP16_SAFE, KC, NAF_WIDTHS, TORCH_DTYPE, PackedConv, PackedEscFfn, PackedFFN, PackedMlp, PackedNafBlock, choose_nt,
@@ -16,7 +16,7 @@
                       LTE_HIDDEN, PackedLte, pack_lte,
                       UNI_UPSAMPLERS, PackedEscRealMSkip, conv_nearest_fold, pack_conv_nearest, pack_escrealm_skip, pack_pixshuf_conv, pixshuf_perm,
                       choose_nt_linear, naf_ffn_fold, naf_frags, pack_naf_block,
-                      ffn_fp16_range_bound, pack_cab_squeeze, pack_cab_w2f, pack_conv_weight, pack_ffn, pack_ffn2, pack_ffn3,
+                      ffn_fp16_range_bound, pack_upfold, pack_cab_squeeze, pack_cab_w2f, pack_conv_weight, pack_ffn, pack_ffn2, pack_ffn3,
                       pack_linear_weight, pack_ocab_mlp, pack_ocab_qkv, pack_pointwise)
 
 DTYPE_CODE = {"f32": HAT_F32, "fp32": HAT_F32, "float32": HAT_F32, "bf16": HAT_BF16, "bfloat16": HAT_BF16}
@@ -538,6 +538,43 @@
     _timed("cab_squeeze_kernel<2, u8>", 2.0 * B * H * W * 9 * C_ * 3, lambda: _lib.check(
         lib.hat_conv3x3_to_u8(_ptr(x), _ptr(wpk), _ptr(bias8), out.data_ptr(), out.stride(1), out.stride(0), B, H, W, C_, ldx, h_out, w_out,
                               out_scale, m4, int(bgr), dtype, _stream()), "hat_conv3x3_to_u8"), tag=f"k3 {C_}->3 {H}x{W} row sweep u8")
+
+
+def upfold_supported(cin: int, nout: int, r: int, W: int, dtype: int) -> bool:
+    return dtype == HAT_BF16 and cin == 64 and nout == 3 and r == 2 and W >= 16 and W % 16 == 0
+
+
+def _upfold_flops(B, H, W):
+    return 2.0 * B * H * W * 25 * 64 * 12
+
+
+def _upfold_bytes(B, H, W, out_bytes):
+    return float(B * H * W * 64 * 2 + out_bytes)
+
+
+def upfold_to_planes(x, pf, out, *, B: int, H: int, W: int, ldx: int, out_scale: float, mean, dtype: int):
+    lib = _lib.load()
+    if out.dtype != torch.float32 or not out.is_cuda or not out.is_contiguous() or tuple(out.shape) != (B, 3, 2 * H, 2 * W):
+        raise RuntimeError(f"upfold_to_planes needs a contiguous (B,3,2H,2W) fp32 device destination, got {tuple(out.shape)} {out.dtype}")
+    d = HatConvDesc()
+    d.x, d.w, d.bias, d.out = _ptr(x), _ptr(pf.w), _ptr(pf.bias), _ptr(out)
+    d.B, d.H, d.W, d.Cin, d.ldx, d.x_mode = B, H, W, 64, ldx, X_NHWC_T
+    d.ksize, d.Kpad, d.nt, d.n_slices, d.n_store = 5, 25 * 64, 1, 1, 12
+    d.out_mode, d.act, d.in_scale, d.out_scale, d.dtype = O_FOLD2_NCHW_F32, ACT_NONE, 1.0, out_scale, dtype
+    for i in range(3):
+        d.mean[i] = float(mean[i])
+    _timed("upfold_kernel<planes>", _upfold_flops(B, H, W), lambda: _lib.check(lib.hat_conv(C.byref(d), _stream()), "hat_conv (folded ending)"),
+        tag=f"k5 64->2x2x3 {H}x{W} folded planes", nbytes=_upfold_bytes(B, H, W, B * 12 * H * W * 4))
+
+
+def upfold_to_u8(x, pf, out, *, B: int, H: int, W: int, ldx: int, h_out: int, w_out: int, out_scale: float, mean, bgr: bool, dtype: int):
+    lib = _lib.load()
+    if out.dtype != torch.uint8 or not out.is_cuda or tuple(out.shape) != (B, h_out, w_out, 3) or out.stride(-1) != 1 or out.stride(-2) != 3:
+        raise RuntimeError("upfold_to_u8 needs a (B,h_out,w_out,3) uint8 device destination with interleaved pixels")
+    _timed("upfold_kernel<u8>", _upfold_flops(B, H, W), lambda: _lib.check(
+        lib.hat_upfold_to_u8(_ptr(x), _ptr(pf.w), _ptr(pf.bias), out.data_ptr(), out.stride(1), out.stride(0), B, H, W, ldx, h_out, w_out,
+                             out_scale, float(mean[0]), float(mean[1]), float(mean[2]), int(bgr), dtype, _stream()), "hat_upfold_to_u8"),
+        tag=f"k5 64->2x2x3 {H}x{W} folded u8", nbytes=_upfold_bytes(B, H, W, B * h_out * w_out * 3))
 
 
 def u8_to_planes(src, dst, *, bgr: bool = False):
@@ -966,6 +1003,19 @@
                                _stream()), "hat_conv3x3_to_yuv"), tag=f"k3 {C_}->3 {H}x{W} row sweep {name}")
 
 
+def upfold_to_yuv(x, pf, y, cb, cr, *, sub, B: int, H: int, W: int, ldx: int, out_scale: float, mean, from_rgb, dtype: int, depth: int = 8,
+                  msb=False):
+    lib = _lib.load()
+    surf = yuv_surface(y, cb, cr, sub=sub, depth=depth, msb=msb, what="upfold_to_yuv")
+    if y.shape[0] != B:
+        raise RuntimeError(f"upfold_to_yuv: destination batch {y.shape[0]} != {B}")
+    m, name = _f12(from_rgb), _sub_name(sub, depth)
+    _timed(f"upfold_kernel<{name}>", _upfold_flops(B, H, W), lambda: _lib.check(
+        lib.hat_upfold_to_yuv(_ptr(x), _ptr(pf.w), _ptr(pf.bias), C.byref(surf), B, H, W, ldx, y.shape[1], y.shape[2], out_scale, float(mean[0]),
+                              float(mean[1]), float(mean[2]), m, dtype, _stream()), "hat_upfold_to_yuv"),
+        tag=f"k5 64->2x2x3 {H}x{W} folded {name}", nbytes=_upfold_bytes(B, H, W, B * y.shape[1] * y.shape[2] * 2))
+
+
 def u8_metrics_flags(*, y_channel: bool, bgr: bool, psnr: bool, ssim: bool) -> int:
     return (_lib.METRICS_Y if y_channel else 0) | (_lib.METRICS_BGR if bgr else 0) | (_lib.METRICS_PSNR if psnr else 0) \
         | (_lib.METRICS_SSIM if ssim else 0)
diff --git a/super_resolution_amd/packing.py b/super_resolution_amd/packing.py
--- a/super_resolution_amd/packing.py
+++ b/super_resolution_amd/packing.py
@@ -529,3 +529,76 @@
     p.w4 = _f32(sd["imnet.layers.6.weight"]).contiguous().to(device)
     p.b4 = _f32(sd["imnet.layers.6.bias"]).contiguous().to(device)
     return p
+
+
+class PackedUpfold:
+    __slots__ = ("w", "bias")
+
+
+def upfold_pieces(wu, bu, wl, bl):
+    wu, bu, wl, bl = (t.detach().to(torch.float64).cpu() for t in (wu, bu, wl, bl))
+    m, k = wl.shape[:2]
+    if wu.shape[0] != 4 * k or tuple(wu.shape[2:]) != (3, 3) or tuple(wl.shape[2:]) != (3, 3):
+        raise ValueError(f"upfold: a {tuple(wu.shape)} conv does not feed PixelShuffle(2) and a {tuple(wl.shape)} conv")
+    c = wu.shape[1]
+    wu4, bu4 = wu.reshape(k, 4, c, 3, 3), bu.reshape(k, 4)
+    G, Bd = torch.zeros(3, 3, m, 2, 2, c, 3, 3, dtype=torch.float64), torch.zeros(3, 3, m, 2, 2, dtype=torch.float64)
+    for a in range(2):
+        for b in range(2):
+            for dy in (-1, 0, 1):
+                for dx in (-1, 0, 1):
+                    iy, ix, sub = (a + dy) // 2 + 1, (b + dx) // 2 + 1, 2 * ((a + dy) % 2) + (b + dx) % 2
+                    G[iy, ix, :, a, b] += torch.einsum("mk,kcef->mcef", wl[:, :, dy + 1, dx + 1], wu4[:, sub])
+                    Bd[iy, ix, :, a, b] += wl[:, :, dy + 1, dx + 1] @ bu4[:, sub]
+    return G, Bd, bl
+
+
+def upfold_variant(G, Bd, bl, rs: int, cs: int):
+    m, c = G.shape[2], G.shape[5]
+    F = torch.zeros(m, 2, 2, c, 5, 5, dtype=torch.float64)
+    bias = bl[:, None, None].expand(m, 2, 2).clone()
+    for iy in range(3):
+        for ix in range(3):
+            if (iy == 0 and rs & 1) or (iy == 2 and rs & 2) or (ix == 0 and cs & 1) or (ix == 2 and cs & 2):
+                continue
+            F[..., iy:iy + 3, ix:ix + 3] += G[iy, ix]
+            bias += Bd[iy, ix]
+    return F, bias
+
+
+def upfold_apply(x, wu, bu, wl, bl):
+    x = x.detach().to(torch.float64).cpu()
+    G, Bd, b0 = upfold_pieces(wu, bu, wl, bl)
+    Bn, _, H, W = x.shape
+    m = G.shape[2]
+    py, px = torch.arange(H)[:, None], torch.arange(W)[None, :]
+    rs, cs = (py == 0) * 1 + (py == H - 1) * 2, (px == 0) * 1 + (px == W - 1) * 2
+    out = torch.zeros(Bn, m * 4, H, W, dtype=torch.float64)
+    for r in range(4):
+        for s in range(4):
+            mask = (rs == r) & (cs == s)
+            if mask.any():
+                F, bias = upfold_variant(G, Bd, b0, r, s)
+                y = torch.nn.functional.conv2d(x, F.reshape(m * 4, -1, 5, 5), bias.reshape(-1), padding=2)
+                out = torch.where(mask, y, out)
+    return torch.nn.functional.pixel_shuffle(out, 2)
+
+
+def pack_upfold(wu, bu, wl, bl, device) -> PackedUpfold:
+    G, Bd, b0 = upfold_pieces(wu, bu, wl, bl)
+    if G.shape[2] != 3 or G.shape[5] != 64:
+        raise ValueError(f"hat_upfold is built for 64 -> 3 channels, got {G.shape[5]} -> {G.shape[2]}")
+    ws, bs = [], []
+    for rs in range(4):
+        for cs in range(3):
+            F, bias = upfold_variant(G, Bd, b0, rs, cs)
+            A = torch.zeros(2, 2, 4, 25, 64, dtype=torch.float64)
+            A[:, :, :3] = F.permute(1, 2, 0, 4, 5, 3).reshape(2, 2, 3, 25, 64)
+            ws.append(frags(A.reshape(16, 25 * 64).to(torch.float32))[0])
+            bb = torch.zeros(2, 2, 4, dtype=torch.float64)
+            bb[:, :, :3] = bias.permute(1, 2, 0)
+            bs.append(bb.reshape(16))
+    p = PackedUpfold()
+    p.w = torch.stack(ws).to(torch.bfloat16).contiguous().to(device)
+    p.bias = torch.stack(bs).to(torch.float32).contiguous().to(device)
+    return p
```

Measured after the change: 351.8 MP/s (median of 6 runs). 3.3% higher.
